# jilljenn/vae

Hardware: AMD Instinct MI355X
Metric: rating-triples/sec (ELBO step) at d=128 (higher is better)
Workload: dtype f32

## Files before the change

### include/vfm_hip.h

```cpp
#ifndef VFM_HIP_H
#define VFM_HIP_H

#include <stdint.h>

#ifdef __cplusplus
extern "C" {
#endif

#define VFM_ABI_VERSION 5
#define VFM_MAX_FIELDS 64
#define VFM_STRUCT_INIT(s) do { memset(&(s), 0, sizeof(s)); (s).struct_size = (uint32_t)sizeof(s); \
                                (s).abi_version = VFM_ABI_VERSION; } while (0)

#define VFM_E_INVALID (-1)
#define VFM_E_UNSUPPORTED (-2)

#define VFM_LIK_NORMAL 0
#define VFM_LIK_BERNOULLI 1

#define VFM_FLAG_NO_PRIOR_TERMS 1
#define VFM_FLAG_SPARSE_ADAM 4
#define VFM_FLAG_SCALED_MOMENTS 32
#define VFM_MOMENT_PERIOD 128
#define VFM_FLAG_ROWS_TOUCHED 128
#define VFM_FLAG_ZREC 1024
#define VFM_FLAG_SHARE_GPU 2048
#define VFM_FLAG_EPS_ZERO 2
#define VFM_FLAG_LINK_SOFTPLUS 16

#define VFM_P_LL 0
#define VFM_P_KL 1
#define VFM_P_G 2
#define VFM_P_ALPHA 3
#define VFM_P_BADID 4
#define VFM_P_GE0 5
#define VFM_P_REDUCED 6
#define VFM_N_PARTIALS 8
#define VFM_SLOT_NTERMS 6
#define VFM_MAX_FWD_BLOCKS 4096
#define VFM_PARTIALS_LEN (VFM_N_PARTIALS * (1 + VFM_MAX_FWD_BLOCKS))

typedef struct vfm_step_consts {
  float step_size, bc2_sqrt;
  float a1, q2, c1, c2, s1, s2;
  int32_t store_true;
  int32_t k;
  int32_t scaled;
  int32_t reserved;
  float lr, beta1, beta2, eps;
} vfm_step_consts_t;
typedef struct vfm_dev_step {
  uint64_t philox_step;
  int64_t adam_step;
  uint64_t philox_step_bwd;
  int64_t adam_step_bwd;
  int64_t tab_first, tab_len;
  const vfm_step_consts_t* tab;
  int64_t error;
} vfm_dev_step_t;
int vfm_step_consts(float lr, float beta1, float beta2, float eps_adam, int64_t step, int32_t scaled,
                    vfm_step_consts_t* out);
int vfm_dev_step_set(vfm_dev_step_t* dev_step, uint64_t philox_step, int64_t adam_step, void* stream);

typedef struct vfm_problem {
  uint32_t struct_size;
  uint32_t abi_version;
  int64_t B;
  int64_t B_global;
  int64_t T;
  int64_t nb_train;
  int32_t F;
  int32_t d;
  int32_t likelihood;
  int32_t id_bits;
  int32_t n_samples;
  int32_t flags;
  int64_t group_hi[VFM_MAX_FIELDS];
  double group_n[VFM_MAX_FIELDS];
  uint64_t seed;
  uint64_t step;
  int64_t e_lo, e_hi;
  vfm_dev_step_t* dev_step;
  float* wrec;
} vfm_problem_t;
int vfm_wrec_build_f32(const float* bias_params, const float* inv_occ, int64_t T, float* wrec, void* stream);

#define VFM_HEAVY_LIST 64
#define VFM_HEAVY_MIN 8
#define VFM_HEAVY_DIRECT 8
typedef struct vfm_index {
  uint32_t struct_size;
  uint32_t abi_version;
  const int32_t* occ_ptr;
  const int32_t* occ_rows;
  const int32_t* heavy_ids;
  const int32_t* heavy_items;
  float* heavy_acc;
  int32_t n_heavy;
  int32_t n_items;
  const int32_t* touched_ids;
  int64_t n_touched;
  const int32_t* occ_other;
  int32_t max_items;
  int32_t heavy_list, heavy_threshold;
  int32_t* status;
} vfm_index_t;

int vfm_abi_version(void);
const char* vfm_last_error(void);

int64_t vfm_index_workspace_bytes(int64_t B, int32_t F, int64_t T);
int vfm_rebuild_heavy(int64_t T, const int32_t* occ_ptr, void* ws, int32_t heavy_list, int32_t threshold, int32_t* heavy_ids,
                      int64_t cap_heavy, int32_t* heavy_items, int64_t cap_items, int32_t* counts , void* stream);
int32_t vfm_heavy_threshold(int32_t heavy_list);
#define VFM_HEAVY_UNITS 8192
int32_t vfm_heavy_list_for(int64_t n_occ, int64_t T);
int vfm_build_index(int64_t B, int32_t F, int64_t T, int32_t id_bits, const void* x, void* ws, int32_t* occ_ptr,
                    int32_t* occ_rows, int32_t heavy_list, int32_t* heavy_ids, int64_t cap_heavy,
                    int32_t* heavy_items, int64_t cap_items, int32_t* touched_ids, int32_t* occ_other,
                    const float* inv_occ, double* W, int32_t* counts, int32_t* counts_host, void* stream);

int vfm_inv_occ_f32(const int64_t* nb_occ, float* inv_occ, int64_t T, void* stream);

int vfm_batch_norms(const vfm_problem_t* p, const void* x, const float* inv_occ, double* W,
                    void* stream);

int vfm_elbo_fwd_f32(const vfm_problem_t* p, const void* x, const float* y,
                     const float* entity_params, const float* bias_params,
                     const float* inv_occ, const float* scalars, const double* W,
                     const float* eps_entity, const float* eps_bias, const float* eps_global,
                     float* pred, double* partials, float* sumz, float* grow, void* stream);

int vfm_elbo_finalize_f32(const vfm_problem_t* p, double* partials, const float* scalars,
                          float* loss, void* stream);

int vfm_elbo_bwd_f32(const vfm_problem_t* p, const vfm_index_t* idx,
                     const float* entity_params, const float* bias_params,
                     const float* inv_occ, const float* scalars, const double* W,
                     const float* eps_entity, const float* eps_bias, const float* eps_global,
                     const float* sumz, const float* grow, const double* partials,
                     const float* grad_out, float* g_entity, float* g_bias, float* g_scalars,
                     void* stream);

int vfm_elbo_bwd_adam_f32(const vfm_problem_t* p, const vfm_index_t* idx,
                          float* entity_params, float* bias_params, float* scalars,
                          const float* inv_occ, const double* W,
                          const float* eps_entity, const float* eps_bias, const float* eps_global,
                          const float* sumz, const float* grow, double* partials,
                          float* m_entity, float* v_entity, float* m_bias, float* v_bias,
                          float* m_scalars, float* v_scalars,
                          float lr, float beta1, float beta2, float eps_adam, int64_t step, float* loss,
                          void* stream);

int vfm_elbo_bwd_acc_f32(const vfm_problem_t* p, const vfm_index_t* idx,
                         const float* sumz, const float* grow, const double* partials, float* acc,
                         float* sums, void* stream);
int vfm_elbo_apply_adam_f32(const vfm_problem_t* p, const float* acc, const float* sums,
                            float* entity_params, float* bias_params, float* scalars, const float* inv_occ,
                            const double* W, const float* eps_entity, const float* eps_bias,
                            const float* eps_global, float* m_entity, float* v_entity, float* m_bias,
                            float* v_bias, float* m_scalars, float* v_scalars, float lr, float beta1,
                            float beta2, float eps_adam, int64_t step, void* stream);
int vfm_elbo_bwd_acc_rows_f32(const vfm_problem_t* p, const vfm_index_t* idx, const int32_t* row_ids, int64_t n_rows,
                              const float* sumz, const float* grow, const double* partials, float* acc,
                              float* sums, void* stream);
int vfm_elbo_apply_adam_rows_f32(const vfm_problem_t* p, const float* acc, const float* sums, const int32_t* row_ids,
                                 int64_t n_rows, int32_t compact_records, float* entity_params, float* bias_params, float* scalars,
                                 const float* inv_occ, const double* W, float* m_entity, float* v_entity, float* m_bias,
                                 float* v_bias, float* m_scalars, float* v_scalars, float lr, float beta1, float beta2,
                                 float eps_adam, int64_t step, void* stream);
int vfm_adam_f32(float* p, const float* g, float* m, float* v, int64_t n, float lr, float beta1,
                 float beta2, float eps, int64_t step, void* stream);

typedef struct vfm_pipe {
  uint32_t struct_size;
  uint32_t abi_version;
  const float* zrec;
  float* zrec_next;
  const int32_t* next_occ_ptr;
  const double* next_W;
  uint64_t next_step;
  int32_t* last_step;
  float* step_tab;
} vfm_pipe_t;
int vfm_sample_records_f32(const vfm_problem_t* p, const int32_t* ids, int64_t n, const float* entity_params,
                           const float* bias_params, const float* inv_occ, const double* W, float* zrec, void* stream);
int vfm_elbo_bwd_adam_pipe_f32(const vfm_problem_t* p, const vfm_index_t* idx, const vfm_pipe_t* pipe,
                               float* entity_params, float* bias_params, float* scalars,
                               const float* inv_occ, const double* W, const float* grow, double* partials,
                               float* m_entity, float* v_entity, float* m_bias, float* v_bias,
                               float* m_scalars, float* v_scalars,
                               float lr, float beta1, float beta2, float eps_adam, int64_t step, float* loss,
                               void* stream);

int vfm_adam_catchup_f32(float* entity_params, float* bias_params, const float* m_entity, const float* v_entity,
                         const float* m_bias, const float* v_bias, int32_t* last_step, const int32_t* ids, int64_t n,
                         int64_t T, int32_t d, const float* lr_of_step, int64_t n_lr, float beta1, float beta2,
                         float eps_adam, int64_t upto, int64_t mark, float* wrec, void* stream);

int64_t vfm_union_workspace_bytes(int64_t T);
int vfm_union_rows(int64_t T, const int32_t* occ_ptr_a, const int32_t* occ_ptr_b, void* ws, int32_t* rows, int32_t* count,
                   int32_t* count_host, void* stream);
int vfm_elbo_bwd_adam_lookahead_f32(const vfm_problem_t* p, const vfm_index_t* idx,
                                    float* entity_params, float* bias_params, float* scalars,
                                    const float* inv_occ, const double* W,
                                    const float* sumz, const float* grow, double* partials,
                                    float* m_entity, float* v_entity, float* m_bias, float* v_bias,
                                    float* m_scalars, float* v_scalars,
                                    float lr, float beta1, float beta2, float eps_adam, int64_t step, float* loss,
                                    int32_t* last_step, const int32_t* next_occ_ptr, float* step_tab, void* stream);

int vfm_moments_rescale_f32(float* m, float* v, int64_t n, float beta1, float beta2, int64_t step, int32_t to_scaled,
                            void* stream);

#define VFM_OBJ_SAMPLED 0
#define VFM_OBJ_CLOSED_FORM 1
int vfm_variant_fwd_f32(const vfm_problem_t* p, int32_t objective, const void* x, const float* values, const float* y,
                        const float* entity_params, const float* bias_params, const float* inv_occ,
                        const float* scalars, const double* W, const float* priors, const float* eps_entity,
                        const float* eps_bias, const float* eps_global, float* pred, double* partials, float* state,
                        float* grow, float* loss, void* stream);
int64_t vfm_variant_workspace_elems(int64_t B, int32_t F, int32_t d);
int vfm_variant_bwd_f32(const vfm_problem_t* p, int32_t objective, const vfm_index_t* idx, int32_t* occ_pos_ws,
                        const void* x, const float* values, const float* entity_params, const float* bias_params,
                        const float* inv_occ, const float* scalars, const double* W, const float* priors,
                        const float* eps_entity, const float* eps_bias, const float* eps_global, const float* state,
                        const float* grow, const double* partials, const float* grad_out, float* g_entity,
                        float* g_bias, float* g_scalars, float* g_priors, void* stream);

int vfm_philox_eps_f32(const vfm_problem_t* p, float* eps_entity, float* eps_bias,
                       float* eps_global, void* stream);

#ifdef __cplusplus
}
#endif
#endif
```

### vae_amd/_abi_gen.py

```python
import ctypes as C

VFM_ABI_VERSION = 5
VFM_E_INVALID = -1
VFM_E_UNSUPPORTED = -2
VFM_FLAG_EPS_ZERO = 2
VFM_FLAG_LINK_SOFTPLUS = 16
VFM_FLAG_NO_PRIOR_TERMS = 1
VFM_FLAG_ROWS_TOUCHED = 128
VFM_FLAG_SCALED_MOMENTS = 32
VFM_FLAG_SHARE_GPU = 2048
VFM_FLAG_SPARSE_ADAM = 4
VFM_FLAG_ZREC = 1024
VFM_HEAVY_DIRECT = 8
VFM_HEAVY_LIST = 64
VFM_HEAVY_MIN = 8
VFM_HEAVY_UNITS = 8192
VFM_LIK_BERNOULLI = 1
VFM_LIK_NORMAL = 0
VFM_MAX_FIELDS = 64
VFM_MAX_FWD_BLOCKS = 4096
VFM_MOMENT_PERIOD = 128
VFM_N_PARTIALS = 8
VFM_OBJ_CLOSED_FORM = 1
VFM_OBJ_SAMPLED = 0
VFM_PARTIALS_LEN = 32776
VFM_P_ALPHA = 3
VFM_P_BADID = 4
VFM_P_G = 2
VFM_P_GE0 = 5
VFM_P_KL = 1
VFM_P_LL = 0
VFM_P_REDUCED = 6
VFM_SLOT_NTERMS = 6


class StepConsts(C.Structure):
    _fields_ = [
        ("step_size", C.c_float),
        ("bc2_sqrt", C.c_float),
        ("a1", C.c_float),
        ("q2", C.c_float),
        ("c1", C.c_float),
        ("c2", C.c_float),
        ("s1", C.c_float),
        ("s2", C.c_float),
        ("store_true", C.c_int32),
        ("k", C.c_int32),
        ("scaled", C.c_int32),
        ("reserved", C.c_int32),
        ("lr", C.c_float),
        ("beta1", C.c_float),
        ("beta2", C.c_float),
        ("eps", C.c_float),
    ]


class DevStep(C.Structure):
    _fields_ = [
        ("philox_step", C.c_uint64),
        ("adam_step", C.c_int64),
        ("philox_step_bwd", C.c_uint64),
        ("adam_step_bwd", C.c_int64),
        ("tab_first", C.c_int64),
        ("tab_len", C.c_int64),
        ("tab", C.c_void_p),
        ("error", C.c_int64),
    ]


class Problem(C.Structure):
    _fields_ = [
        ("struct_size", C.c_uint32),
        ("abi_version", C.c_uint32),
        ("B", C.c_int64),
        ("B_global", C.c_int64),
        ("T", C.c_int64),
        ("nb_train", C.c_int64),
        ("F", C.c_int32),
        ("d", C.c_int32),
        ("likelihood", C.c_int32),
        ("id_bits", C.c_int32),
        ("n_samples", C.c_int32),
        ("flags", C.c_int32),
        ("group_hi", C.c_int64 * VFM_MAX_FIELDS),
        ("group_n", C.c_double * VFM_MAX_FIELDS),
        ("seed", C.c_uint64),
        ("step", C.c_uint64),
        ("e_lo", C.c_int64),
        ("e_hi", C.c_int64),
        ("dev_step", C.c_void_p),
        ("wrec", C.c_void_p),
    ]

    def __init__(self, *a, **k):
        super().__init__(*a, **k)
        self.struct_size, self.abi_version = C.sizeof(type(self)), VFM_ABI_VERSION


class Index(C.Structure):
    _fields_ = [
        ("struct_size", C.c_uint32),
        ("abi_version", C.c_uint32),
        ("occ_ptr", C.c_void_p),
        ("occ_rows", C.c_void_p),
        ("heavy_ids", C.c_void_p),
        ("heavy_items", C.c_void_p),
        ("heavy_acc", C.c_void_p),
        ("n_heavy", C.c_int32),
        ("n_items", C.c_int32),
        ("touched_ids", C.c_void_p),
        ("n_touched", C.c_int64),
        ("occ_other", C.c_void_p),
        ("max_items", C.c_int32),
        ("heavy_list", C.c_int32),
        ("heavy_threshold", C.c_int32),
        ("status", C.c_void_p),
    ]

    def __init__(self, *a, **k):
        super().__init__(*a, **k)
        self.struct_size, self.abi_version = C.sizeof(type(self)), VFM_ABI_VERSION


class Pipe(C.Structure):
    _fields_ = [
        ("struct_size", C.c_uint32),
        ("abi_version", C.c_uint32),
        ("zrec", C.c_void_p),
        ("zrec_next", C.c_void_p),
        ("next_occ_ptr", C.c_void_p),
        ("next_W", C.c_void_p),
        ("next_step", C.c_uint64),
        ("last_step", C.c_void_p),
        ("step_tab", C.c_void_p),
    ]

    def __init__(self, *a, **k):
        super().__init__(*a, **k)
        self.struct_size, self.abi_version = C.sizeof(type(self)), VFM_ABI_VERSION
```

### vae_amd/_lib.py

```python
from __future__ import annotations

import ctypes as C
import os

import torch

HERE = os.path.dirname(os.path.abspath(__file__))
LIB_DIR = os.environ.get("VFM_LIB_DIR") or HERE
LIB_PATH = os.path.join(LIB_DIR, "libvfm_hip.so")
OPS_PATH = os.path.join(LIB_DIR, "libvfm_torch_ops.so")

from . import _abi_gen as _gen

ABI_VERSION = _gen.VFM_ABI_VERSION
MAX_FWD_BLOCKS = _gen.VFM_MAX_FWD_BLOCKS
MAX_FIELDS = _gen.VFM_MAX_FIELDS
N_PARTIALS = _gen.VFM_N_PARTIALS
PARTIALS_LEN = _gen.VFM_PARTIALS_LEN
P_LL, P_KL, P_G, P_ALPHA, P_BADID = _gen.VFM_P_LL, _gen.VFM_P_KL, _gen.VFM_P_G, _gen.VFM_P_ALPHA, _gen.VFM_P_BADID
LIK_NORMAL, LIK_BERNOULLI = _gen.VFM_LIK_NORMAL, _gen.VFM_LIK_BERNOULLI
OBJ_SAMPLED, OBJ_CLOSED_FORM = _gen.VFM_OBJ_SAMPLED, _gen.VFM_OBJ_CLOSED_FORM

EXPORTS = (
    "vfm_abi_version", "vfm_last_error", "vfm_inv_occ_f32", "vfm_batch_norms",
    "vfm_elbo_fwd_f32", "vfm_elbo_finalize_f32", "vfm_elbo_bwd_f32", "vfm_philox_eps_f32",
    "vfm_adam_f32", "vfm_elbo_bwd_adam_f32", "vfm_elbo_bwd_acc_f32", "vfm_elbo_apply_adam_f32",
    "vfm_moments_rescale_f32", "vfm_index_workspace_bytes", "vfm_build_index", "vfm_heavy_list_for",
    "vfm_variant_fwd_f32", "vfm_variant_bwd_f32", "vfm_variant_workspace_elems", "vfm_adam_catchup_f32", "vfm_union_rows", "vfm_union_workspace_bytes",
    "vfm_sample_records_f32", "vfm_elbo_bwd_adam_pipe_f32", "vfm_elbo_bwd_adam_lookahead_f32",
    "vfm_step_consts", "vfm_dev_step_set", "vfm_wrec_build_f32", "vfm_elbo_apply_adam_rows_f32",
    "vfm_elbo_bwd_acc_rows_f32", "vfm_heavy_threshold", "vfm_rebuild_heavy",
)


class _Strict:

    def __setattr__(self, name, value):
        if name not in type(self)._names:
            raise AttributeError(f"{type(self).__name__} has no field {name!r}")
        super().__setattr__(name, value)


class Problem(_Strict, _gen.Problem):
    """`vfm_problem_t` (struct_size / abi_version are set by the generated __init__)."""


class Index(_Strict, _gen.Index):
    """`vfm_index_t`."""


class Pipe(_Strict, _gen.Pipe):
    """`vfm_pipe_t`."""


StepConsts, DevStep = _gen.StepConsts, _gen.DevStep

ELICIT_MAX_ROUNDS = 4096
ELICIT_SOLVE_EXPORTS = ("vfm_elicit_solve_f32", "vfm_elicit_solve_workspace_bytes")
ELICIT_EXPORTS = ("vfm_elicit_f32", "vfm_elicit_workspace_bytes", "vfm_elicit_field_f32",
                  "vfm_elicit_field_workspace_bytes") + ELICIT_SOLVE_EXPORTS


RANK_POST_EXPORTS = ("vfm_field_moments_post_f32", "vfm_rank_field_post_f32", "vfm_rank_heldout_field_post_f32")


VARIANT_STEP_EXPORTS = ("vfm_variant_step_f32", "vfm_variant_step_workspace_bytes")


def _fields(ctype, *names):
    return tuple((n, ctype) for n in names)


FOLDIN_SOLVE_EXPORTS = ("vfm_foldin_solve_f32", "vfm_foldin_solve_workspace_bytes")
FOLDIN_SOLVE_LDS_DIM = 135
FOLDIN_SOLVE_SLABS = 256
SWEEP_EXPORTS = ("vfm_foldin_solve_split_f32", "vfm_foldin_split_workspace_bytes")
PRIOR_EXPORTS = ("vfm_foldin_solve_prior_f32", "vfm_foldin_solve_prior_workspace_bytes",
                 "vfm_foldin_solve_split_prior_f32", "vfm_foldin_split_prior_workspace_bytes")
BOUND_EXPORTS = ("vfm_foldin_bound_f32", "vfm_foldin_bound_workspace_bytes")
BOUND_SWEEP_EXPORTS = ("vfm_foldin_bound_split_f32", "vfm_foldin_bound_split_workspace_bytes")
BOUND_PRIOR_EXPORTS = ("vfm_foldin_bound_prior_f32", "vfm_foldin_bound_prior_workspace_bytes",
                       "vfm_foldin_bound_split_prior_f32", "vfm_foldin_bound_split_prior_workspace_bytes")

_FOLD_COUNTS = _fields(C.c_int64, "E", "R", "T", "n_ops")
_FOLD_DIMS = _fields(C.c_int32, "F", "d", "col")
_FOLD_OPTIONS = _fields(C.c_int32, "flags", "lds_dim") + (("kl_weight", C.c_float),)
_FOLD_IDS = (("entities", C.c_void_p),)
_FOLD_TAIL = (_fields(C.c_void_p, "y", "op_x", "row_op", "entity_params", "bias_params", "scalars", "out_loss", "workspace")
              + (("workspace_bytes", C.c_int64),))
_FOLD_LIST_HEAD = _FOLD_COUNTS + _FOLD_DIMS + _fields(C.c_int32, "objective", "likelihood") + _FOLD_OPTIONS
_FOLD_CHUNK_HEAD = _FOLD_COUNTS + (("n_chunks", C.c_int64),) + _FOLD_DIMS + _FOLD_OPTIONS
_FOLD_LIST_ROWS = _FOLD_IDS + (("row_ptr", C.c_void_p),) + _FOLD_TAIL
_FOLD_CHUNK_ROWS = _FOLD_IDS + _fields(C.c_void_p, "chunk_ptr", "chunks") + _FOLD_TAIL


class FoldinSolve(_Strict, C.Structure):
    _fields_ = list(_FOLD_LIST_HEAD + _FOLD_LIST_ROWS)


class FoldinSplit(_Strict, C.Structure):
    _fields_ = list(_FOLD_CHUNK_HEAD + _FOLD_CHUNK_ROWS)


class FoldinBound(_Strict, C.Structure):
    _fields_ = list(_FOLD_LIST_HEAD + _fields(C.c_int32, "n_iters", "reset", "mode", "pad0") + _FOLD_LIST_ROWS)


class FoldinBoundSplit(_Strict, C.Structure):
    _fields_ = list(_FOLD_CHUNK_HEAD + _fields(C.c_int32, "n_iters", "reset") + _FOLD_CHUNK_ROWS)


_I64, _I32 = C.c_int64, C.c_int32
_SOLVE_SIZES, _SPLIT_SIZES = [_I64, _I64, _I32, _I32], [_I64, _I64, _I64, _I32, _I32]
_FOLD_PROTOTYPES = (
    ("vfm_foldin_solve_f32", FoldinSolve, [], "vfm_foldin_solve_workspace_bytes", _SOLVE_SIZES),
    ("vfm_foldin_solve_split_f32", FoldinSplit, [], "vfm_foldin_split_workspace_bytes", _SPLIT_SIZES),
    ("vfm_foldin_solve_prior_f32", FoldinSolve, [C.c_void_p], "vfm_foldin_solve_prior_workspace_bytes", _SOLVE_SIZES),
    ("vfm_foldin_solve_split_prior_f32", FoldinSplit, [C.c_void_p], "vfm_foldin_split_prior_workspace_bytes", _SPLIT_SIZES),
    ("vfm_foldin_bound_f32", FoldinBound, [], "vfm_foldin_bound_workspace_bytes", [_I64] + _SOLVE_SIZES),
    ("vfm_foldin_bound_split_f32", FoldinBoundSplit, [], "vfm_foldin_bound_split_workspace_bytes", [_I64] + _SPLIT_SIZES),
    ("vfm_foldin_bound_prior_f32", FoldinBound, [C.c_void_p], "vfm_foldin_bound_prior_workspace_bytes", [_I64] + _SOLVE_SIZES),
    ("vfm_foldin_bound_split_prior_f32", FoldinBoundSplit, [C.c_void_p], "vfm_foldin_bound_split_prior_workspace_bytes",
     [_I64] + _SPLIT_SIZES),
)


ELICIT_BOUND_EXPORTS = ("vfm_elicit_bound_f32", "vfm_elicit_bound_workspace_bytes")


_STAMP = _fields(C.c_uint32, "struct_size", "abi_version")
_COUNTS = _fields(C.c_int64, "U", "P", "H", "T", "n_ops")
_FIELD_ROWS = _fields(C.c_void_p, "entities", "pool_ptr", "pool_x", "pool_y", "hist_ptr", "hist_x", "hist_y")
_OPERANDS = _fields(C.c_void_p, "op_x", "pool_op", "hist_op")
_TABLES_OUTPUTS = _fields(C.c_void_p, "entity_params", "bias_params", "scalars", "out_row", "out_score", "out_loss",
                          "out_theta", "out_mean", "out_var")
_WORKSPACE = (("workspace", C.c_void_p), ("workspace_bytes", C.c_int64))
_ADAM_TAIL = (_fields(C.c_int32, "objective", "likelihood", "flags", "n_steps", "n_samples", "reset", "write", "lds_rows")
              + _fields(C.c_float, "lr", "kl_weight") + (("seed", C.c_uint64), ("t0", C.c_int64)))
_SOLVE_HEAD = (_fields(C.c_int32, "F", "d", "field", "key_col", "n_rounds", "strategy", "flags", "reset", "write", "lds_dim")
               + (("kl_weight", C.c_float),))
_SEED = (("seed", C.c_uint64),)


class _Session(_Strict, C.Structure):

    def __init__(self, *a, **k):
        super().__init__(*a, **k)
        self.struct_size, self.abi_version = C.sizeof(type(self)), ABI_VERSION


class Elicit(_Session):
    _fields_ = list(_STAMP + _COUNTS + _fields(C.c_int32, "F", "d", "n_rounds", "strategy") + _ADAM_TAIL
                    + _fields(C.c_void_p, "users", "pool_ptr", "pool_items", "pool_y", "hist_ptr", "hist_items", "hist_y")
                    + _OPERANDS + _TABLES_OUTPUTS + _WORKSPACE)


class ElicitField(_Session):
    _fields_ = list(_STAMP + _COUNTS + _fields(C.c_int32, "F", "d", "field", "key_col", "n_rounds", "strategy")
                    + _ADAM_TAIL + _FIELD_ROWS + _OPERANDS + _TABLES_OUTPUTS + _WORKSPACE)


class ElicitSolve(_Session):
    _fields_ = list(_STAMP + _COUNTS + _SOLVE_HEAD + _SEED + _FIELD_ROWS + _OPERANDS + _TABLES_OUTPUTS + _WORKSPACE)


class ElicitBound(_Session):
    _fields_ = list(_STAMP + _COUNTS + _SOLVE_HEAD + (("n_iters", C.c_int32),) + _SEED + _FIELD_ROWS + _OPERANDS
                    + _TABLES_OUTPUTS + _WORKSPACE)


DESIGN_EXPORTS = ("vfm_design_workspace_bytes", "vfm_design_scores_f32", "vfm_design_elicit_f32")


class ElicitDesign(_Session):
    _fields_ = list(_STAMP + _COUNTS + (("n_targets", C.c_int64),)
                    + _fields(C.c_int32, "F", "d", "field", "n_rounds", "flags", "reset", "write", "lds_dim")
                    + (("kl_weight", C.c_float),) + _FIELD_ROWS + _fields(C.c_void_p, "tgt_ptr", "tgt_op") + _OPERANDS
                    + _TABLES_OUTPUTS + (("out_pool_score", C.c_void_p),) + _WORKSPACE)


ELICIT_PRIOR_EXPORTS = ("vfm_elicit_solve_prior_f32", "vfm_elicit_solve_prior_workspace_bytes",
                        "vfm_elicit_bound_prior_f32", "vfm_elicit_bound_prior_workspace_bytes",
                        "vfm_design_scores_prior_f32", "vfm_design_elicit_prior_f32", "vfm_design_prior_workspace_bytes")
_ELICIT_PRIOR_PROTOTYPES = (
    ("vfm_elicit_solve_prior_f32", ElicitSolve, "vfm_elicit_solve_prior_workspace_bytes", [_I64, _I64, _I64, _I32, _I32]),
    ("vfm_elicit_bound_prior_f32", ElicitBound, "vfm_elicit_bound_prior_workspace_bytes",
     [_I64, _I64, _I64, _I64, _I32, _I32, _I32]),
    ("vfm_design_scores_prior_f32", ElicitDesign, "vfm_design_prior_workspace_bytes", [_I64, _I64, _I64, _I32, _I32]),
    ("vfm_design_elicit_prior_f32", ElicitDesign, "vfm_design_prior_workspace_bytes", [_I64, _I64, _I64, _I32, _I32]),
)


for _c in (Problem, Index, Pipe, Elicit, ElicitField, ElicitSolve, ElicitBound, ElicitDesign, FoldinSolve, FoldinSplit,
           FoldinBound, FoldinBoundSplit):
    _c._names = frozenset(n for n, _ in _c._fields_)


def heavy_list_for(n_occ: int, T: int) -> int:
    return int(load().vfm_heavy_list_for(int(n_occ), int(T)))


class VfmLibraryError(RuntimeError):
    pass


_lib = None


def load():
    global _lib
    if _lib is not None:
        return _lib
    if not os.path.exists(LIB_PATH):
        raise VfmLibraryError(
            f"{LIB_PATH} not found: build it with `python -c 'import __graft_entry__ as g; g.build()'` "
            "(hipcc --offload-arch=gfx950).  vae_amd has no CPU / PyTorch fallback.")
    lib = C.CDLL(LIB_PATH)
    vp, i64, i32 = C.c_void_p, C.c_int64, C.c_int32
    PP = C.POINTER(Problem)
    lib.vfm_abi_version.restype = C.c_int
    lib.vfm_abi_version.argtypes = []
    lib.vfm_last_error.restype = C.c_char_p
    lib.vfm_last_error.argtypes = []
    lib.vfm_inv_occ_f32.argtypes = [vp, vp, i64, vp]
    lib.vfm_batch_norms.argtypes = [PP, vp, vp, vp, vp]
    lib.vfm_elbo_fwd_f32.argtypes = [PP] + [vp] * 15
    lib.vfm_elbo_finalize_f32.argtypes = [PP, vp, vp, vp, vp]
    lib.vfm_elbo_bwd_f32.argtypes = [PP] + [vp] * 17
    lib.vfm_philox_eps_f32.argtypes = [PP, vp, vp, vp, vp]
    lib.vfm_elbo_bwd_adam_f32.argtypes = ([PP] + [vp] * 18 +
                                          [C.c_float, C.c_float, C.c_float, C.c_float, i64, vp, vp])
    lib.vfm_adam_f32.argtypes = [vp, vp, vp, vp, i64, C.c_float, C.c_float, C.c_float, C.c_float,
                                 i64, vp]
    lib.vfm_elbo_bwd_acc_f32.argtypes = [PP] + [vp] * 7
    lib.vfm_elbo_apply_adam_f32.argtypes = ([PP] + [vp] * 16 +
                                            [C.c_float, C.c_float, C.c_float, C.c_float, i64, vp])
    lib.vfm_elbo_bwd_acc_rows_f32.argtypes = [PP, C.POINTER(Index), vp, i64] + [vp] * 6
    lib.vfm_elbo_apply_adam_rows_f32.argtypes = ([PP, vp, vp, vp, i64, i32] + [vp] * 11 +
                                                 [C.c_float, C.c_float, C.c_float, C.c_float, i64, vp])
    lib.vfm_moments_rescale_f32.argtypes = [vp, vp, i64, C.c_float, C.c_float, i64, i32, vp]
    lib.vfm_index_workspace_bytes.argtypes = [i64, i32, i64]
    lib.vfm_heavy_list_for.argtypes = [i64, i64]
    lib.vfm_build_index.argtypes = [i64, i32, i64, i32, vp, vp, vp, vp, i32, vp, i64, vp, i64, vp, vp, vp, vp, vp, vp, vp]
    lib.vfm_rebuild_heavy.argtypes = [i64, vp, vp, i32, i32, vp, i64, vp, i64, vp, vp]
    lib.vfm_adam_catchup_f32.argtypes = [vp] * 8 + [i64, i64, i32, C.POINTER(C.c_float), i64, C.c_float, C.c_float, C.c_float,
                                         i64, i64, vp, vp]
    lib.vfm_step_consts.argtypes = [C.c_float, C.c_float, C.c_float, C.c_float, i64, i32, C.POINTER(StepConsts)]
    lib.vfm_dev_step_set.argtypes = [vp, C.c_uint64, i64, vp]
    lib.vfm_wrec_build_f32.argtypes = [vp, vp, i64, vp, vp]
    lib.vfm_sample_records_f32.argtypes = [PP, vp, i64, vp, vp, vp, vp, vp, vp]
    lib.vfm_elbo_bwd_adam_pipe_f32.argtypes = ([PP, C.POINTER(Index), C.POINTER(Pipe)] + [vp] * 13 +
                                               [C.c_float, C.c_float, C.c_float, C.c_float, i64, vp, vp])
    lib.vfm_elbo_bwd_adam_lookahead_f32.argtypes = ([PP, C.POINTER(Index)] + [vp] * 14 +
                                                    [C.c_float, C.c_float, C.c_float, C.c_float, i64, vp, vp, vp, vp, vp])
    lib.vfm_variant_fwd_f32.argtypes = [PP, i32] + [vp] * 18
    lib.vfm_variant_bwd_f32.argtypes = [PP, i32, C.POINTER(Index)] + [vp] * 21
    lib.vfm_union_workspace_bytes.argtypes = [i64]
    lib.vfm_union_workspace_bytes.restype = i64
    lib.vfm_union_rows.argtypes = [i64] + [vp] * 7
    lib.vfm_variant_workspace_elems.argtypes = [i64, i32, i32]
    lib.vfm_variant_workspace_elems.restype = i64
    lib.vfm_elicit_f32.argtypes = [C.POINTER(Elicit), vp]
    lib.vfm_elicit_f32.restype = C.c_int
    lib.vfm_elicit_workspace_bytes.argtypes = [i64, i64, i32, i32]
    lib.vfm_elicit_workspace_bytes.restype = i64
    lib.vfm_elicit_field_f32.argtypes = [C.POINTER(ElicitField), vp]
    lib.vfm_elicit_field_f32.restype = C.c_int
    lib.vfm_elicit_field_workspace_bytes.argtypes = [i64, i64, i32, i32]
    lib.vfm_elicit_field_workspace_bytes.restype = i64
    lib.vfm_elicit_solve_f32.argtypes = [C.POINTER(ElicitSolve), vp]
    lib.vfm_elicit_solve_f32.restype = C.c_int
    lib.vfm_elicit_solve_workspace_bytes.argtypes = [i64, i64, i64, i32, i32]
    lib.vfm_elicit_solve_workspace_bytes.restype = i64
    lib.vfm_design_workspace_bytes.argtypes = [i64, i64, i64, i32, i32]
    lib.vfm_design_workspace_bytes.restype = i64
    for name in ("vfm_design_scores_f32", "vfm_design_elicit_f32"):
        getattr(lib, name).argtypes = [C.POINTER(ElicitDesign), vp]
        getattr(lib, name).restype = C.c_int
    for entry, struct, extra, size, size_args in _FOLD_PROTOTYPES:
        getattr(lib, entry).argtypes = [C.POINTER(struct)] + extra + [vp]
        getattr(lib, entry).restype = C.c_int
        getattr(lib, size).argtypes = size_args
        getattr(lib, size).restype = i64
    lib.vfm_elicit_bound_f32.argtypes = [C.POINTER(ElicitBound), vp]
    lib.vfm_elicit_bound_f32.restype = C.c_int
    lib.vfm_elicit_bound_workspace_bytes.argtypes = [i64, i64, i64, i64, i32, i32, i32]
    lib.vfm_elicit_bound_workspace_bytes.restype = i64
    for entry, struct, size, size_args in _ELICIT_PRIOR_PROTOTYPES:
        getattr(lib, entry).argtypes = [C.POINTER(struct), vp, vp]
        getattr(lib, entry).restype = C.c_int
        getattr(lib, size).argtypes = size_args
        getattr(lib, size).restype = i64
    u64 = C.c_uint64
    lib.vfm_field_moments_post_f32.argtypes = [i64, i32, i32, i64, i32, i32, vp, i32, i32, vp, vp, vp, vp, i32, u64,
                                               vp, vp, vp, vp, vp]
    lib.vfm_rank_field_post_f32.argtypes = ([i64, vp, i32, i32, vp, vp, i64, vp, i64, i64, i32, i32, i32, i32, i32, u64,
                                             i32, vp, vp, i64, vp, vp, vp, vp, i64] + [vp] * 5)
    lib.vfm_rank_heldout_field_post_f32.argtypes = ([i64, vp, i32, i32, vp, vp, i64, vp, i64, i64, i32, i32, i32, i32, u64,
                                                     i32, vp, vp, i64, vp, vp, i64, vp, vp, vp, vp, i64] + [vp] * 5)
    for name in RANK_POST_EXPORTS:
        getattr(lib, name).restype = C.c_int
    lib.vfm_variant_step_f32.argtypes = ([PP, i32, C.POINTER(Index)] + [vp] * 24 +
                                         [C.c_float, C.c_float, C.c_float, C.c_float, i64, vp])
    lib.vfm_variant_step_f32.restype = C.c_int
    lib.vfm_variant_step_workspace_bytes.argtypes = [i64, i32, i32]
    lib.vfm_variant_step_workspace_bytes.restype = i64
    for name in EXPORTS:
        fn = getattr(lib, name)
        if name != "vfm_last_error":
            fn.restype = C.c_int
    for name in ("vfm_index_workspace_bytes", "vfm_union_workspace_bytes", "vfm_variant_workspace_elems"):
        getattr(lib, name).restype = i64
    if lib.vfm_abi_version() != ABI_VERSION:
        raise VfmLibraryError(f"ABI mismatch: library {lib.vfm_abi_version()}, package {ABI_VERSION}")
    _lib = lib
    return lib


_ops = None


def ops():
    global _ops
    if _ops is not None:
        return _ops
    load()
    if not os.path.exists(OPS_PATH):
        raise VfmLibraryError(f"{OPS_PATH} not found: run __graft_entry__.build()")
    torch.ops.load_library(OPS_PATH)
    if torch.ops.vfm_hip.abi_version() != ABI_VERSION:
        raise VfmLibraryError("ABI mismatch between libvfm_torch_ops.so and the package")
    _ops = torch.ops.vfm_hip
    return _ops


def check(rc, what):
    if rc != 0:
        msg = load().vfm_last_error().decode(errors="replace")
        raise VfmLibraryError(f"{what} failed (code {rc}): {msg}")


def ptr(t):
    return None if t is None else C.c_void_p(t.data_ptr())


def raw_stream(device) -> int:
    idx = device.index if getattr(device, "index", None) is not None else torch.cuda.current_device()
    return torch._C._cuda_getCurrentRawStream(idx)


def current_stream_ptr(device):
    return C.c_void_p(raw_stream(device))
```

### vae_amd/csrc/vfm_abi.hip

```cpp
#include <stdio.h>
#include <string.h>
#include <math.h>
#include <stdlib.h>
#include <mutex>

#include "vfm_args.hpp"

namespace vfm {

namespace {
thread_local char g_err[512] = "";
}

int fail(int code, const char* msg) {
  snprintf(g_err, sizeof(g_err), "%s", msg);
  return code;
}
int fail_hip(hipError_t e, const char* where) {
  snprintf(g_err, sizeof(g_err), "%s: %s", where, hipGetErrorString(e));
  return (int)e;
}
int env_int(const char* name, int dflt) {
  const char* v = getenv(name);
  return (v && *v) ? atoi(v) : dflt;
}

namespace {

#include "vfm_rng.hpp"
#include "vfm_common.hpp"
#include "vfm_reduce.hpp"
#include "vfm_small_kernels.hpp"
#include "vfm_heavy.hpp"
#include "vfm_adam.hpp"

bool pick_shape(int d, Shape* s) {
  auto pow2ceil = [](int v) { int p = 1; while (p < v) p <<= 1; return p; };
  if (d % 4 == 0) {
    const int C = d / 4;
    s->vec = 4;
    s->lpe = pow2ceil(C) < 64 ? (pow2ceil(C) < 4 ? 4 : pow2ceil(C)) : 64;
    const int cpl = (C + s->lpe - 1) / s->lpe;
    s->cpl = cpl <= 1 ? 1 : (cpl <= 2 ? 2 : 4);
    return cpl <= 4;
  }
  s->vec = 1;
  if (d <= 8) { s->lpe = 8; s->cpl = 1; return true; }
  if (d <= 64) { s->lpe = 64; s->cpl = 1; return true; }
  s->lpe = 64; s->cpl = 4;
  return d <= 256;
}

int check_struct(uint32_t size, uint32_t abi, size_t want, const char* name) {
  if (size == (uint32_t)want && abi == (uint32_t)VFM_ABI_VERSION) return 0;
  snprintf(g_err, sizeof(g_err), "%s: struct_size %u / abi_version %u, this library expects %zu / %d (set them with "
           "VFM_STRUCT_INIT; a binding generated from another version of include/vfm_hip.h must be regenerated)",
           name, size, abi, want, VFM_ABI_VERSION);
  return VFM_E_INVALID;
}

int check_problem(const vfm_problem_t* p, bool dev_ok = false) {
  if (!p) return fail(VFM_E_INVALID, "problem is NULL");
  if (int rc = check_struct(p->struct_size, p->abi_version, sizeof(vfm_problem_t), "vfm_problem_t")) return rc;
  if (p->dev_step && !dev_ok)
    return fail(VFM_E_UNSUPPORTED, "vfm_problem_t.dev_step: only the training forward and the fused backward+Adam entry points read the step from device memory");
  if (p->dev_step && p->n_samples != 1) return fail(VFM_E_UNSUPPORTED, "vfm_problem_t.dev_step: one variational sample");
  if (p->dev_step && (((uintptr_t)p->dev_step) & 15) != 0) return fail(VFM_E_INVALID, "vfm_problem_t.dev_step must be 16-byte aligned");
  if (p->wrec && (((uintptr_t)p->wrec) & 15) != 0) return fail(VFM_E_INVALID, "vfm_problem_t.wrec must be 16-byte aligned");
  if (p->B < 0 || p->T <= 0 || p->T > 0xFFFFFFFELL) return fail(VFM_E_INVALID, "bad B or T");
  if (p->F < 1 || p->F > VFM_MAX_FIELDS) return fail(VFM_E_INVALID, "F out of range [1,64]");
  if (p->d < 1) return fail(VFM_E_INVALID, "d < 1");
  if (p->id_bits != 32 && p->id_bits != 64) return fail(VFM_E_INVALID, "id_bits must be 32 or 64");
  if (p->likelihood != VFM_LIK_NORMAL && p->likelihood != VFM_LIK_BERNOULLI)
    return fail(VFM_E_INVALID, "unknown likelihood");
  if (p->n_samples < 1 || p->n_samples > MAX_SAMPLES) return fail(VFM_E_INVALID, "n_samples out of range [1,64]");
  if (p->n_samples > 1 && (p->step >> 48) != 0) return fail(VFM_E_INVALID, "step must stay below 2^48 when n_samples > 1");
  if (p->B_global < p->B) return fail(VFM_E_INVALID, "B_global < B");
  if (p->B * (int64_t)p->F > 0x7FFFFFFFLL) return fail(VFM_E_INVALID, "B*F exceeds int32 index range");
  if (p->e_lo < 0 || p->e_lo > p->T || (p->e_hi != 0 && p->e_hi < p->e_lo)) return fail(VFM_E_INVALID, "bad entity range");
  if (p->flags & ~(VFM_FLAG_NO_PRIOR_TERMS | VFM_FLAG_EPS_ZERO | VFM_FLAG_SPARSE_ADAM | VFM_FLAG_LINK_SOFTPLUS |
                   VFM_FLAG_SCALED_MOMENTS | VFM_FLAG_ROWS_TOUCHED | VFM_FLAG_ZREC | VFM_FLAG_SHARE_GPU))
    return fail(VFM_E_INVALID, "unknown bit in vfm_problem_t.flags");
  Shape s;
  if (!pick_shape(p->d, &s)) return fail(VFM_E_UNSUPPORTED, "embedding size d not supported (d%4==0: d<=1024, else d<=256)");
  return 0;
}

bool softplus(const vfm_problem_t* p) { return (p->flags & VFM_FLAG_LINK_SOFTPLUS) != 0; }

int single_sample_only(const vfm_problem_t* p, const char* who) {
  if (p->n_samples == 1) return 0;
  snprintf(g_err, sizeof(g_err), "%s: n_samples > 1 is not supported by this entry point", who);
  return VFM_E_UNSUPPORTED;
}


int eps_mode(const vfm_problem_t* p, const float* ee, const float* eb, const float* eg, int* mode) {
  const int neps = (ee != nullptr) + (eb != nullptr) + (eg != nullptr);
  if (neps != 0 && neps != 3) return fail(VFM_E_INVALID, "give all three eps tables or none");
  *mode = (p->flags & VFM_FLAG_EPS_ZERO) ? EPS_ZERO : (neps == 3 ? EPS_TABLE : EPS_PHILOX);
  return 0;
}

KArgs make_args(const vfm_problem_t* p, const void* x, const float* y, const float* entity,
                const float* bias, const float* inv_occ, const float* scalars, const double* W,
                const float* ee, const float* eb, const float* eg, int sample = 0) {
  KArgs a;
  memset(&a, 0, sizeof(a));
  a.S = p->n_samples; a.sample = sample; a.inv_S = 1.0f / (float)p->n_samples;
  if (sample > 0) {
    if (ee) ee += (size_t)sample * (size_t)p->T * (size_t)p->d;
    if (eb) eb += (size_t)sample * (size_t)p->T;
  }
  a.B = p->B; a.T = p->T; a.F = p->F; a.d = p->d; a.lik = p->likelihood;
  a.e_lo = p->e_lo; a.e_hi = (p->e_hi > 0 && p->e_hi < p->T) ? p->e_hi : p->T;
  a.id64 = p->id_bits == 64; a.G = p->F; a.flags = p->flags;
  a.ll_scale_d = (double)p->nb_train / ((double)(p->B_global > 0 ? p->B_global : 1) * (double)p->n_samples);
  a.ll_scale = (float)a.ll_scale_d;
  a.key.seed_lo = (uint32_t)p->seed; a.key.seed_hi = (uint32_t)(p->seed >> 32);
  a.key.step_lo = (uint32_t)p->step; a.key.step_hi = (uint32_t)(p->step >> 32);
  a.key.chunk_off = 0;
  a.x = x; a.y = y; a.entity = entity; a.bias = bias; a.inv_occ = inv_occ; a.scalars = scalars;
  a.W = W; a.eps_entity = ee; a.eps_bias = eb; a.eps_global = eg;
  a.dev = p->dev_step; a.wrec = p->wrec;
  for (int g = 0; g < p->F; ++g) { a.group_hi[g] = p->group_hi[g]; a.group_n[g] = p->group_n[g]; }
  return a;
}

bool use_fwd2(const vfm_problem_t* p, int eps, bool multi = false) {
  if (p->F != 2 || (p->d & 3) != 0 || p->d > 512) return false;
  if (multi ? (p->n_samples < 2 || p->n_samples > 4 || eps == EPS_ZERO) : p->n_samples != 1) return false;
  if (softplus(p)) return false;
  const int forced = env_int("VFM_FWD_KERNEL", 0);
  if (forced == 1) return false;
  return forced == 2 || eps == EPS_ZREC || multi || p->d >= 20;
}

bool use_fwdg(const vfm_problem_t* p, int eps, int mode) {
  if (p->F == 2 || (p->d & 3) != 0 || p->d < 16 || p->d > 512 || p->n_samples != 1) return false;
  if ((p->flags & VFM_FLAG_ZREC) || softplus(p)) return false;
  if (!(eps == EPS_PHILOX || (eps == EPS_ZERO && mode == MODE_PREDICT))) return false;
  return env_int("VFM_FWD_KERNEL", 0) != 1;
}

int dispatch_fwd(const vfm_problem_t* p, const Shape& s, int eps, int mode, int ff, KArgs& a, const FwdOut& o,
                 hipStream_t st) {
  if (use_fwdg(p, eps, mode)) return launch_fwdg_abs(eps, mode, a, o, st);
  if (use_fwd2(p, eps)) {
    if (mode == MODE_TRAIN && eps == EPS_PHILOX && env_int("VFM_FWD_AB_NORNG", 0) == 1) eps = EPS_ZERO;
    return launch_fwd2_abs(eps, mode, a, o, st);
  }
  return softplus(p) ? launch_fwd_softplus(s, eps, mode, ff, a, o, st) : launch_fwd_abs(s, eps, mode, ff, a, o, st);
}
int dispatch_bwd(const vfm_problem_t* p, const Shape& s, int eps, int adam, KArgs& a, const BwdArgs& b,
                 const AdamArgs& ad, hipStream_t st) {
  if (adam == 0 || adam == 10)
    return softplus(p) ? launch_bwd0_softplus(s, eps, adam, a, b, ad, st) : launch_bwd0_abs(s, eps, adam, a, b, ad, st);
  return softplus(p) ? launch_bwd1_softplus(s, eps, adam, a, b, ad, st) : launch_bwd1_abs(s, eps, adam, a, b, ad, st);
}

BwdArgs bwd_args(const vfm_problem_t* p, const vfm_index_t* idx) {
  BwdArgs b;
  memset(&b, 0, sizeof(b));
  if (idx) { b.occ_ptr = idx->occ_ptr; b.occ_rows = idx->occ_rows; b.status = idx->status; }
  b.n_occ = (int32_t)(p->B * (int64_t)p->F);
  return b;
}

template <int LPE, int CPL, int VEC>
int launch_heavy_t(const vfm_problem_t* p, const vfm_index_t* idx, const float* sumz, const float* grow, float* hacc, int d,
                   hipStream_t st, const float* zrec = nullptr) {
  constexpr int GPB = BLOCK / LPE;
  const size_t xs = 4 + (((size_t)d + 3) & ~(size_t)3);
  float* item_acc = hacc + xs * (size_t)idx->n_heavy;
  int64_t nb = ((int64_t)idx->n_items + GPB - 1) / GPB;
  if (nb > 4096) nb = 4096;
  hipLaunchKernelGGL((k_heavy<LPE, CPL, VEC>), dim3((unsigned)nb), dim3(BLOCK), 0, st, idx->heavy_items,
                     (int)idx->n_items, idx->occ_rows, sumz, grow, item_acc, d, zrec ? idx->occ_other : nullptr, zrec, hacc,
                     (int)idx->n_heavy, (int)(p->B * (int64_t)p->F), (int)p->B, p->T, idx->status);
  if (idx->max_items > 0 && idx->max_items <= VFM_HEAVY_DIRECT) return 0;
  nb = idx->n_heavy;
  if (nb > 4096) nb = 4096;
  hipLaunchKernelGGL((k_heavy_sum<LPE, CPL, VEC>), dim3((unsigned)nb), dim3(BLOCK), 0, st, idx->heavy_items,
                     (int)idx->n_items, (int)idx->n_heavy, item_acc, hacc, d);
  return 0;
}

int run_heavy(const vfm_problem_t* p, const vfm_index_t* idx, const float* sumz, const float* grow,
              hipStream_t st, BwdArgs* b, const float* zrec = nullptr) {
  b->heavy_ids = nullptr; b->heavy_acc = nullptr; b->n_heavy = 0; b->heavy_stride = 0;
  if (idx->n_heavy <= 0 || idx->n_items <= 0) return 0;
  if (!idx->heavy_ids || !idx->heavy_items || !idx->heavy_acc)
    return fail(VFM_E_INVALID, "index: heavy_ids / heavy_items / heavy_acc missing");
  if ((int64_t)idx->n_heavy > p->T || (int64_t)idx->n_items > p->B * (int64_t)p->F + idx->n_heavy)
    return fail(VFM_E_INVALID, "index: more heavy entities than table rows, or more work items than occurrences");
  const size_t xs = 4 + (((size_t)p->d + 3) & ~(size_t)3);
  const size_t per_sample = xs * ((size_t)idx->n_heavy + (size_t)idx->n_items);
  Shape s;
  pick_shape(p->d, &s);
  for (int sm = 0; sm < p->n_samples; ++sm) {
    const float* sz = sumz ? sumz + (size_t)sm * (size_t)p->B * (size_t)p->d : nullptr;
    float* hacc = idx->heavy_acc + (size_t)sm * per_sample;
#define X(L_, C_, V_) \
    if (s.lpe == L_ && s.cpl == C_ && s.vec == V_) launch_heavy_t<L_, C_, V_>(p, idx, sz, grow, hacc, p->d, st, zrec);
    VFM_FOR_SHAPES(X)
#undef X
  }
  b->heavy_ids = idx->heavy_ids; b->heavy_acc = idx->heavy_acc; b->n_heavy = idx->n_heavy;
  b->heavy_stride = idx->n_heavy + idx->n_items;
  return 0;
}

struct Side { hipStream_t s = nullptr; hipEvent_t e1 = nullptr, e2 = nullptr; bool ok = false, tried = false; std::mutex mu; };
Side* side_of_device() {
  static Side sides[64];
  static std::mutex mu;
  int dev = 0;
  if (hipGetDevice(&dev) != hipSuccess || dev < 0 || dev >= 64) return nullptr;
  std::lock_guard<std::mutex> lk(mu);
  Side& sd = sides[dev];
  if (!sd.tried) {
    sd.tried = true;
    sd.ok = hipStreamCreateWithFlags(&sd.s, hipStreamNonBlocking) == hipSuccess &&
            hipEventCreateWithFlags(&sd.e1, hipEventDisableTiming) == hipSuccess &&
            hipEventCreateWithFlags(&sd.e2, hipEventDisableTiming) == hipSuccess;
  }
  return sd.ok ? &sd : nullptr;
}
bool heavy_overlap(const vfm_problem_t* p, const vfm_index_t* idx) {
  return idx->n_heavy > 0 && idx->n_items > 0 && (int64_t)idx->n_heavy * 16 < p->T && p->n_samples == 1 &&
         env_int("VFM_HEAVY_OVERLAP", 1) != 0;
}

int bwd_adam_overlapped(const vfm_problem_t* p, const vfm_index_t* idx, const Shape& s, int eps, int adam, KArgs& a, BwdArgs& b,
                        const AdamArgs& ad, const float* sumz, const float* grow, hipStream_t st, Side* sd) {
  std::lock_guard<std::mutex> lk(sd->mu);
  hipError_t e = hipEventRecord(sd->e1, st);
  if (e == hipSuccess) e = hipStreamWaitEvent(sd->s, sd->e1, 0);
  if (e != hipSuccess) return fail_hip(e, "heavy-list overlap: events");
  if (int rc = run_heavy(p, idx, sumz, grow, sd->s, &b)) return rc;
  e = hipEventRecord(sd->e2, sd->s);
  if (e != hipSuccess) return fail_hip(e, "heavy-list overlap: events");
  const int32_t keep = a.row_filter;
  a.row_filter = 4;
  if (int rc = dispatch_bwd(p, s, eps, adam, a, b, ad, st)) return rc;
  e = hipStreamWaitEvent(st, sd->e2, 0);
  if (e != hipSuccess) return fail_hip(e, "heavy-list overlap: events");
  BwdArgs bh = b;
  bh.row_ids = idx->heavy_ids; bh.n_rows = idx->n_heavy;
  a.row_filter = 3;
  const int rc = dispatch_bwd(p, s, eps, adam, a, bh, ad, st);
  a.row_filter = keep;
  return rc;
}

bool small_table_step(const vfm_problem_t* p, const vfm_index_t* idx, int eps, int rows_flags) {
  if (eps != EPS_PHILOX || rows_flags != 0 || p->n_samples != 1 || (p->flags & VFM_FLAG_SPARSE_ADAM)) return false;
  if ((p->d & 3) != 0 || p->d > 256) return false;
  if (idx->heavy_list < VFM_HEAVY_MIN || idx->heavy_threshold < VFM_HEAVY_MIN || idx->heavy_threshold > idx->heavy_list) return false;
  if (p->T * (2 * (int64_t)p->d + 2) * 4 > (2LL << 20)) return false;
  return env_int("VFM_BWD_SMALL", 1) != 0;
}

int check_index(const vfm_problem_t* p, const vfm_index_t* idx, const char* who) {
  if (!idx) { snprintf(g_err, sizeof(g_err), "%s: inverted index missing", who); return VFM_E_INVALID; }
  if (int rc = check_struct(idx->struct_size, idx->abi_version, sizeof(vfm_index_t), "vfm_index_t")) return rc;
  if (!idx->occ_ptr || (p->B > 0 && !idx->occ_rows)) {
    snprintf(g_err, sizeof(g_err), "%s: inverted index missing", who);
    return VFM_E_INVALID;
  }
  if (idx->n_heavy < 0 || idx->n_items < 0 || idx->n_touched < 0 || idx->max_items < 0) {
    snprintf(g_err, sizeof(g_err), "%s: negative count in vfm_index_t", who);
    return VFM_E_INVALID;
  }
  return 0;
}

int after_launch(const char* where) {
  const hipError_t e = hipGetLastError();
  if (e != hipSuccess) return fail_hip(e, where);
  return 0;
}

void adam_consts(float lr, float beta1, float beta2, int64_t step, float* step_size, float* bc2_sqrt) {
  const double bc1 = 1.0 - pow((double)beta1, (double)step);
  const double bc2 = 1.0 - pow((double)beta2, (double)step);
  *step_size = (float)((double)lr / bc1);
  *bc2_sqrt = (float)sqrt(bc2);
}

void scaled_step_consts(float step_size, float bc2_sqrt, double s1, double s2, float* a1, float* q2) {
  *a1 = (float)((double)step_size * s1);
  *q2 = (float)(sqrt(s2) / (double)bc2_sqrt);
}

int scaled_moment_consts(const vfm_problem_t* p, float beta1, float beta2, int64_t step, AdamArgs* ad) {
  ad->scaled = 0; ad->store_true = 0; ad->s1 = ad->s2 = 1.f; ad->c1 = 1.f - beta1; ad->c2 = 1.f - beta2;
  ad->inv_bc2_sqrt = 1.0f / ad->bc2_sqrt;
  ad->a1 = ad->step_size; ad->q2 = ad->inv_bc2_sqrt;
  if (!(p->flags & VFM_FLAG_SCALED_MOMENTS)) return 0;
  if (p->flags & VFM_FLAG_SPARSE_ADAM)
    return fail(VFM_E_INVALID, "VFM_FLAG_SCALED_MOMENTS and VFM_FLAG_SPARSE_ADAM exclude each other");
  const int64_t k = (step - 1) % VFM_MOMENT_PERIOD + 1;
  const double s1 = pow((double)beta1, (double)k), s2 = pow((double)beta2, (double)k);
  if (!(s1 > 1e-30) || !(s2 > 1e-30))
    return fail(VFM_E_UNSUPPORTED, "VFM_FLAG_SCALED_MOMENTS: beta^128 underflows (use the plain moments for such betas)");
  ad->scaled = 1; ad->store_true = (k == VFM_MOMENT_PERIOD);
  ad->s1 = (float)s1; ad->s2 = (float)s2;
  ad->c1 = (float)((1.0 - (double)beta1) / s1); ad->c2 = (float)((1.0 - (double)beta2) / s2);
  scaled_step_consts(ad->step_size, ad->bc2_sqrt, s1, s2, &ad->a1, &ad->q2);
  return 0;
}

}
}

using namespace vfm;

int vfm::launch_norms(int64_t B, int F, int64_t T, int id_bits, const void* x, const float* inv_occ, double* W, hipStream_t st) {
  hipLaunchKernelGGL(k_zero_f64, dim3(1), dim3(64), 0, st, W, F);
  if (B == 0) return after_launch("vfm_batch_norms");
  int64_t nbx = (B + BLOCK * 8 - 1) / (BLOCK * 8);
  if (nbx > 1024) nbx = 1024;
  hipLaunchKernelGGL(k_norms, dim3((unsigned)nbx, (unsigned)F), dim3(BLOCK), 0, st, x, (int)(id_bits == 64), inv_occ, B, F, T,
                     reinterpret_cast<unsigned long long*>(W));
  hipLaunchKernelGGL(k_norms_fix, dim3(1), dim3(64), 0, st, W, F);
  return after_launch("vfm_batch_norms");
}

extern "C" {

int vfm_abi_version(void) { return VFM_ABI_VERSION; }
const char* vfm_last_error(void) { return g_err; }

int vfm_step_consts(float lr, float beta1, float beta2, float eps_adam, int64_t step, int32_t scaled,
                    vfm_step_consts_t* out) {
  if (!out || step < 1) return fail(VFM_E_INVALID, "vfm_step_consts: bad argument");
  vfm_problem_t p;
  memset(&p, 0, sizeof(p));
  p.flags = scaled ? VFM_FLAG_SCALED_MOMENTS : 0;
  AdamArgs ad;
  memset(&ad, 0, sizeof(ad));
  ad.b1 = beta1; ad.b2 = beta2; ad.eps = eps_adam;
  adam_consts(lr, beta1, beta2, step, &ad.step_size, &ad.bc2_sqrt);
  if (int rc = scaled_moment_consts(&p, beta1, beta2, step, &ad)) return rc;
  memset(out, 0, sizeof(*out));
  out->step_size = ad.step_size; out->bc2_sqrt = ad.bc2_sqrt; out->a1 = ad.a1; out->q2 = ad.q2;
  out->c1 = ad.c1; out->c2 = ad.c2; out->s1 = ad.s1; out->s2 = ad.s2;
  out->store_true = ad.store_true; out->k = (int32_t)((step - 1) % VFM_MOMENT_PERIOD + 1); out->scaled = ad.scaled;
  out->lr = lr; out->beta1 = beta1; out->beta2 = beta2; out->eps = eps_adam;
  return 0;
}

int vfm_dev_step_set(vfm_dev_step_t* dev_step, uint64_t philox_step, int64_t adam_step, void* stream) {
  if (!dev_step || adam_step < 1) return fail(VFM_E_INVALID, "vfm_dev_step_set: bad argument");
  hipLaunchKernelGGL(k_dev_step_set, dim3(1), dim3(64), 0, (hipStream_t)stream, dev_step, philox_step, adam_step);
  return after_launch("vfm_dev_step_set");
}

int vfm_wrec_build_f32(const float* bias_params, const float* inv_occ, int64_t T, float* wrec, void* stream) {
  if (!bias_params || !inv_occ || !wrec || T <= 0 || (((uintptr_t)wrec) & 15) != 0)
    return fail(VFM_E_INVALID, "vfm_wrec_build_f32: bad argument");
  const int grid = (int)((T + 255) / 256 < 2048 ? (T + 255) / 256 : 2048);
  hipLaunchKernelGGL(k_wrec_build, dim3(grid), dim3(256), 0, (hipStream_t)stream, bias_params, inv_occ, T, wrec);
  return after_launch("vfm_wrec_build_f32");
}

int vfm_inv_occ_f32(const int64_t* nb_occ, float* inv_occ, int64_t T, void* stream) {
  if (!nb_occ || !inv_occ || T <= 0) return fail(VFM_E_INVALID, "vfm_inv_occ_f32: bad argument");
  const int grid = (int)((T + 255) / 256 < 2048 ? (T + 255) / 256 : 2048);
  hipLaunchKernelGGL(k_inv_occ, dim3(grid), dim3(256), 0, (hipStream_t)stream, nb_occ, inv_occ, T);
  return after_launch("vfm_inv_occ_f32");
}

int vfm_batch_norms(const vfm_problem_t* p, const void* x, const float* inv_occ, double* W,
                    void* stream) {
  if (int rc = check_problem(p)) return rc;
  if (!W || (p->B > 0 && (!x || !inv_occ))) return fail(VFM_E_INVALID, "vfm_batch_norms: NULL pointer");
  return launch_norms(p->B, p->F, p->T, p->id_bits, x, inv_occ, W, (hipStream_t)stream);
}

int vfm_elbo_fwd_f32(const vfm_problem_t* p, const void* x, const float* y,
                     const float* entity_params, const float* bias_params,
                     const float* inv_occ, const float* scalars, const double* W,
                     const float* eps_entity, const float* eps_bias, const float* eps_global,
                     float* pred, double* partials, float* sumz, float* grow, void* stream) {
  if (int rc = check_problem(p, true)) return rc;
  if (!partials) return fail(VFM_E_INVALID, "vfm_elbo_fwd_f32: partials is NULL");
  if (p->dev_step && (eps_entity || eps_bias || eps_global || (p->flags & VFM_FLAG_EPS_ZERO)))
    return fail(VFM_E_UNSUPPORTED, "vfm_elbo_fwd_f32: dev_step goes with the in-kernel Philox eps stream only");
  hipStream_t st0 = (hipStream_t)stream;
  if (p->B == 0) {
    hipLaunchKernelGGL(k_zero_f64, dim3(1), dim3(64), 0, st0, partials, (int)VFM_N_PARTIALS);
    return after_launch("vfm_elbo_fwd_f32");
  }
  const bool zrec = (p->flags & VFM_FLAG_ZREC) != 0;
  if (zrec) {
    if (!use_fwd2(p, EPS_ZREC)) return fail(VFM_E_UNSUPPORTED, "VFM_FLAG_ZREC: two fields, one sample, d % 4 == 0, d <= 512, |.| link");
    if (!x || !y || !entity_params || !scalars || !pred || !grow || eps_entity || eps_bias || eps_global)
      return fail(VFM_E_INVALID, "vfm_elbo_fwd_f32 (VFM_FLAG_ZREC): x, y, the record table, scalars, pred, grow; no eps tables");
    KArgs a = make_args(p, x, y, entity_params, nullptr, nullptr, scalars, nullptr, nullptr, nullptr, nullptr, 0);
    FwdOut o{pred, partials, nullptr, grow};
    if (int rc = launch_fwd2_abs(EPS_ZREC, MODE_TRAIN, a, o, (hipStream_t)stream)) return rc;
    return after_launch("vfm_elbo_fwd_f32");
  }
  if (!x || !entity_params || !bias_params || !scalars || !pred)
    return fail(VFM_E_INVALID, "vfm_elbo_fwd_f32: NULL pointer");
  const bool train = y != nullptr;
  if (train && (!inv_occ || !W || !sumz || !grow))
    return fail(VFM_E_INVALID, "vfm_elbo_fwd_f32: y given, so inv_occ, W, sumz and grow are required");
  if (!train && (sumz || grow)) return fail(VFM_E_INVALID, "vfm_elbo_fwd_f32: sumz / grow need y");
  int eps;
  if (int rc = eps_mode(p, eps_entity, eps_bias, eps_global, &eps)) return rc;
  if (train && eps == EPS_ZERO) return fail(VFM_E_UNSUPPORTED, "vfm_elbo_fwd_f32: VFM_FLAG_EPS_ZERO is prediction-only");
  hipStream_t st = (hipStream_t)stream;
  FwdOut o{pred, partials, sumz, grow};
  Shape s;
  pick_shape(p->d, &s);
  if (use_fwd2(p, eps, true)) {
    KArgs a = make_args(p, x, y, entity_params, bias_params, inv_occ, scalars, W, eps_entity, eps_bias, eps_global, 0);
    const int md = train ? MODE_TRAIN : MODE_PREDICT;
    if (int rc = launch_fwd2m_abs(eps, md, a, o, st)) return rc;
    return after_launch("vfm_elbo_fwd_f32");
  }
  for (int sm = 0; sm < p->n_samples; ++sm) {
    KArgs a = make_args(p, x, y, entity_params, bias_params, inv_occ, scalars, W, eps_entity, eps_bias,
                        eps_global, sm);
// ... 416 lines not shown
```

### vae_amd/csrc/vfm_args.hpp

```cpp
#pragma once
#include <hip/hip_runtime.h>
#include <stdint.h>

#include "vfm_hip.h"

#define VFM_INTERNAL __attribute__((visibility("hidden")))

namespace vfm {

constexpr int BLOCK = 256;
constexpr float LOG_SQRT_2PI = 0.918938533204672742f;
constexpr float LN2 = 0.693147180559945309f;
constexpr float LOG2E = 1.4426950408889634f;

struct RngKey {
  uint32_t seed_lo, seed_hi, step_lo, step_hi;
  uint32_t chunk_off;
};

struct KArgs {
  int64_t B, T;
  int64_t e_lo, e_hi;
  int32_t F, d, lik, id64, G, flags;
  int32_t S, sample;
  int32_t row_filter;
  float inv_S;
  float ll_scale;
  double ll_scale_d;
  RngKey key;
  const void* x;
  const float* y;
  const float* entity;
  const float* bias;
  const float* inv_occ;
  const float* scalars;
  const double* W;
  const float* eps_entity;
  const float* eps_bias;
  const float* eps_global;
  vfm_dev_step_t* dev;
  float* wrec;
  int64_t group_hi[VFM_MAX_FIELDS];
  double group_n[VFM_MAX_FIELDS];
};

struct FwdOut {
  float* pred;
  double* partials;
  float* sumz;
  float* grow;
};

struct BwdArgs {
  const int32_t* occ_ptr;
  const int32_t* occ_rows;
  const float* sumz;
  const float* grow;
  double* partials;
  const float* grad_out;
  float* g_entity;
  float* g_bias;
  float* g_scalars;
  float* loss;
  float* acc;
  float* sums;
  const int32_t* heavy_ids;
  const float* heavy_acc;
  int32_t n_heavy;
  int32_t heavy_stride;
  const int32_t* row_ids;
  int64_t n_rows;
  const float* zrec;
  const int32_t* occ_other;
  float* zrec_next;
  const int32_t* next_occ_ptr;
  const double* next_W;
  RngKey next_key;
  int32_t* last_step;
  float2* step_tab;
  int32_t la_step, la_k;
  int32_t rec_by_slot;
  int32_t n_occ;
  int32_t* status;
};

struct AdamArgs {
  float* m_entity; float* v_entity; float* m_bias; float* v_bias; float* m_scal; float* v_scal;
  float b1, b2, eps, step_size, bc2_sqrt;
  int32_t scaled, store_true;
  float s1, s2, c1, c2, inv_bc2_sqrt;
  float a1, q2;
};

__device__ __forceinline__ RngKey key_of_step(const KArgs& a, bool writer) {
  RngKey key = a.key;
  if (a.dev) {
    const uint64_t s = a.dev->philox_step;
    key.step_lo = (uint32_t)s; key.step_hi = (uint32_t)(s >> 32);
    if (writer) { a.dev->philox_step_bwd = s; a.dev->adam_step_bwd = a.dev->adam_step; }
  }
  return key;
}
__device__ __forceinline__ void load_dev_step(const KArgs& a, RngKey& key, AdamArgs& ad, int32_t& la_step, int32_t& la_k,
                                              RngKey& next_key, bool bump) {
  if (!a.dev) return;
  const uint64_t s = a.dev->philox_step_bwd;
  const int64_t t = a.dev->adam_step_bwd;
  key.step_lo = (uint32_t)s; key.step_hi = (uint32_t)(s >> 32);
  next_key.step_lo = (uint32_t)(s + 1); next_key.step_hi = (uint32_t)((s + 1) >> 32);
  int64_t i = t - a.dev->tab_first;
  const bool miss = i < 0 || i >= a.dev->tab_len;
  if (miss) i = i < 0 ? 0 : a.dev->tab_len - 1;
  const vfm_step_consts_t c = a.dev->tab[i];
  ad.step_size = c.step_size; ad.bc2_sqrt = c.bc2_sqrt; ad.inv_bc2_sqrt = 1.0f / c.bc2_sqrt;
  ad.a1 = c.a1; ad.q2 = c.q2; ad.c1 = c.c1; ad.c2 = c.c2; ad.s1 = c.s1; ad.s2 = c.s2;
  ad.store_true = c.store_true; ad.scaled = c.scaled;
  ad.b1 = c.beta1; ad.b2 = c.beta2; ad.eps = c.eps;
  la_step = (int32_t)t; la_k = c.k;
  if (bump) {
    a.dev->philox_step = s + 1; a.dev->adam_step = t + 1;
    if (miss) a.dev->error = 1;
  }
}

struct Shape {
  int lpe, cpl, vec;
};

enum { EPS_PHILOX = 0, EPS_TABLE = 1, EPS_ZERO = 2, EPS_ZREC = 4 };
enum { MODE_PREDICT = 0, MODE_TRAIN = 1 };
enum { STAGE_FULL = 0, STAGE_ACC = 1, STAGE_APPLY = 2 };
enum { LINK_ABS = 0, LINK_SOFTPLUS = 1 };
constexpr int MAX_SAMPLES = 64;

VFM_INTERNAL int fail(int code, const char* msg);
VFM_INTERNAL int fail_hip(hipError_t e, const char* where);
VFM_INTERNAL int env_int(const char* name, int dflt);
VFM_INTERNAL int launch_norms(int64_t B, int F, int64_t T, int id_bits, const void* x, const float* inv_occ, double* W,
                              hipStream_t st);

#define VFM_DECLARE_LAUNCHERS(SUFFIX)                                                                          \
  VFM_INTERNAL int launch_fwd_##SUFFIX(const Shape& s, int eps, int mode, int ff, KArgs& a, const FwdOut& o,   \
                                       hipStream_t st);                                                        \
  VFM_INTERNAL int launch_bwd0_##SUFFIX(const Shape& s, int eps, int adam, KArgs& a, const BwdArgs& b,         \
                                        const AdamArgs& ad, hipStream_t st);                                   \
  VFM_INTERNAL int launch_bwd1_##SUFFIX(const Shape& s, int eps, int adam, KArgs& a, const BwdArgs& b,         \
                                        const AdamArgs& ad, hipStream_t st);
VFM_DECLARE_LAUNCHERS(abs)
VFM_DECLARE_LAUNCHERS(softplus)
VFM_INTERNAL int launch_bwd_small_abs(const Shape& s, KArgs& a, const BwdArgs& b, const AdamArgs& ad, int L, int THR, hipStream_t st);
VFM_INTERNAL int launch_bwd_small_softplus(const Shape& s, KArgs& a, const BwdArgs& b, const AdamArgs& ad, int L, int THR, hipStream_t st);
VFM_INTERNAL int launch_fwd2_abs(int eps, int mode, KArgs& a, const FwdOut& o, hipStream_t st);
VFM_INTERNAL int launch_fwd2m_abs(int eps, int mode, KArgs& a, const FwdOut& o, hipStream_t st);
VFM_INTERNAL int launch_fwdg_abs(int eps, int mode, KArgs& a, const FwdOut& o, hipStream_t st);
VFM_INTERNAL int launch_sample_rec_abs(const Shape& s, KArgs& a, const int32_t* ids, int n, float* zrec, hipStream_t st);

#define VFM_FOR_SHAPES(X)                                                                      \
  X(4, 1, 4) X(8, 1, 4) X(16, 1, 4) X(32, 1, 4) X(64, 1, 4) X(64, 2, 4) \
  X(64, 4, 4) X(8, 1, 1) X(64, 1, 1) X(64, 4, 1)

}
```

### vae_amd/csrc/vfm_fwd2.hip

```cpp
#include <math.h>

#include "vfm_args.hpp"

#ifndef VFM_LINK
#error "compile with -DVFM_LINK=0 (abs) or -DVFM_LINK=1 (softplus)"
#endif

namespace vfm {
namespace {

#include "vfm_rng.hpp"
#include "vfm_common.hpp"
typedef float v2f __attribute__((ext_vector_type(2)));
#include "vfm_fwd2.hpp"

constexpr int LINK = VFM_LINK;

template <int LPE, bool FULL, int EPS, int MODE>
int launch_fwd2_t(KArgs& a, const FwdOut& o, hipStream_t st) {
  constexpr int GPB = BLOCK / LPE;
  const int per_cu = env_int("VFM_FWD2_BLOCKS_PER_CU", 4);
  int64_t nb = (a.B + GPB - 1) / GPB;
  int64_t cap = 256LL * per_cu;
  if (cap > VFM_MAX_FWD_BLOCKS) cap = VFM_MAX_FWD_BLOCKS;
  if (nb > cap) nb = cap;
  { const int share = env_int("VFM_SHARE_CAP", 960); if ((a.flags & VFM_FLAG_SHARE_GPU) && share > 0 && nb > share) nb = share; }
  { const int forced = env_int("VFM_FWD2_GRID", 0); if (forced > 0 && nb > forced) nb = forced; }
  if (nb < 1) nb = 1;
  if constexpr (EPS == EPS_PHILOX && MODE == MODE_TRAIN) {
    if (a.wrec) {
      if (a.id64)
        hipLaunchKernelGGL((k_fwd2<LPE, FULL, EPS, MODE, true, LINK, true>), dim3((unsigned)nb), dim3(BLOCK), 0, st, a, o);
      else
        hipLaunchKernelGGL((k_fwd2<LPE, FULL, EPS, MODE, false, LINK, true>), dim3((unsigned)nb), dim3(BLOCK), 0, st, a, o);
      return 0;
    }
  }
  if (a.id64)
    hipLaunchKernelGGL((k_fwd2<LPE, FULL, EPS, MODE, true, LINK>), dim3((unsigned)nb), dim3(BLOCK), 0, st, a, o);
  else
    hipLaunchKernelGGL((k_fwd2<LPE, FULL, EPS, MODE, false, LINK>), dim3((unsigned)nb), dim3(BLOCK), 0, st, a, o);
  return 0;
}

template <int LPE, bool FULL>
int launch_fwd2_s(int eps, int mode, KArgs& a, const FwdOut& o, hipStream_t st) {
#define FWD2(E_, M_) \
  if (eps == E_ && mode == M_) return launch_fwd2_t<LPE, FULL, E_, M_>(a, o, st);
  FWD2(EPS_PHILOX, MODE_TRAIN) FWD2(EPS_TABLE, MODE_TRAIN) FWD2(EPS_ZERO, MODE_TRAIN) FWD2(EPS_ZREC, MODE_TRAIN)
  FWD2(EPS_PHILOX, MODE_PREDICT) FWD2(EPS_TABLE, MODE_PREDICT) FWD2(EPS_ZERO, MODE_PREDICT)
#undef FWD2
  return fail(VFM_E_UNSUPPORTED, "forward (task stream): unsupported eps source / mode combination");
}

int dispatch_fwd2(int eps, int mode, KArgs& a, const FwdOut& o, hipStream_t st) {
  const int C = a.d / 4, P = (C + 1) / 2;
  int lpe = 1;
  while (lpe < P) lpe <<= 1;
  const bool full = a.d == 8 * lpe;
#define X(L_)                                                                       \
  if (lpe == L_) return full ? launch_fwd2_s<L_, true>(eps, mode, a, o, st)         \
                             : launch_fwd2_s<L_, false>(eps, mode, a, o, st);
  X(1) X(2) X(4) X(8) X(16) X(32) X(64)
#undef X
  return fail(VFM_E_UNSUPPORTED, "forward (task stream): embedding size above 512");
}

}

#if VFM_LINK == 0
int launch_fwd2_abs(int eps, int mode, KArgs& a, const FwdOut& o, hipStream_t st) {
  return dispatch_fwd2(eps, mode, a, o, st);
}
#else
int launch_fwd2_softplus(int eps, int mode, KArgs& a, const FwdOut& o, hipStream_t st) {
  return dispatch_fwd2(eps, mode, a, o, st);
}
#endif

}
```

### vae_amd/csrc/vfm_fwd2.hpp

```cpp
#pragma once


template <int EPS>
struct EntRegs {
  uint32_t e;
  Chunk<4> mu[2], s[2], ep[2];
  float2 th;
  float io;
  float epw;
};

template <bool ID64>
struct RawIds {
  uint32_t ulo, uhi, ilo, ihi;
};
struct Ids {
  uint32_t u, i;
};
constexpr uint32_t BAD_ID = 0xFFFFFFFFu;

template <bool ID64>
__device__ __forceinline__ RawIds<ID64> load_row_ids(const KArgs& a, int r) {
  RawIds<ID64> v;
  if constexpr (ID64) {
    const uint4 t = reinterpret_cast<const uint4*>(a.x)[r];
    v.ulo = t.x; v.uhi = t.y; v.ilo = t.z; v.ihi = t.w;
  } else {
    const uint2 t = reinterpret_cast<const uint2*>(a.x)[r];
    v.ulo = t.x; v.uhi = 0u; v.ilo = t.y; v.ihi = 0u;
  }
  return v;
}

template <bool ID64>
__device__ __forceinline__ Ids fold_ids(const RawIds<ID64>& v, uint32_t T32) {
  Ids o;
  o.u = ((!ID64 || v.uhi == 0u) && v.ulo < T32) ? v.ulo : BAD_ID;
  o.i = ((!ID64 || v.ihi == 0u) && v.ilo < T32) ? v.ilo : BAD_ID;
  return o;
}

__device__ __forceinline__ uint32_t entity_of(uint32_t id, bool live, float& bad) {
  const bool ok = id != BAD_ID;
  bad += (live && !ok) ? 1.f : 0.f;
  return ok ? id : 0u;
}

template <int EPS, int MODE, bool WREC = false>
__device__ __forceinline__ void load_ent(const KArgs& a, uint32_t e, int off0, int off1, EntRegs<EPS>& R) {
  const size_t d = (size_t)a.d;
  R.e = e;
  if constexpr (EPS == EPS_ZREC) {
    const float* rec = a.entity + (size_t)e * (4 + d);
    R.mu[0] = ld_chunk<4>(rec + 4 + off0);
    R.mu[1] = ld_chunk<4>(rec + 4 + off1);
    const float4 h = *reinterpret_cast<const float4*>(rec);
    R.th = make_float2(h.x, 0.f);
    R.io = h.y;
    return;
  }
  const float* row = a.entity + (size_t)e * (2 * d);
  R.mu[0] = ld_chunk<4>(row + off0);
  R.mu[1] = ld_chunk<4>(row + off1);
  R.s[0] = ld_chunk<4>(row + d + off0);
  R.s[1] = ld_chunk<4>(row + d + off1);
  if constexpr (EPS == EPS_TABLE) {
    const float* er = a.eps_entity + (size_t)e * d;
    R.ep[0] = ld_chunk<4>(er + off0);
    R.ep[1] = ld_chunk<4>(er + off1);
    R.epw = a.eps_bias[e];
  }
  if constexpr (WREC) {
    const float4 h = *reinterpret_cast<const float4*>(a.wrec + 4 * (size_t)e);
    R.th = make_float2(h.x, h.y);
    R.io = h.z;
  } else {
    R.th = *reinterpret_cast<const float2*>(a.bias + 2 * (size_t)e);
    if constexpr (MODE == MODE_TRAIN) R.io = a.inv_occ[e];
  }
}

template <bool FULL, int EPS, int MODE, int LINK>
__device__ __forceinline__ void sample_ent(const RngKey& key, const EntRegs<EPS>& R, uint32_t pg, bool v0, bool v1,
                                           bool owns_bias, float cs, float (&z)[8], float& w, float& klw) {
  if constexpr (EPS == EPS_ZREC) {
#pragma unroll
    for (int t = 0; t < 4; ++t) {
      z[t] = (FULL || v0) ? R.mu[0].v[t] : 0.f;
      z[4 + t] = (FULL || v1) ? R.mu[1].v[t] : 0.f;
    }
    w = owns_bias ? R.th.x : 0.f;
    klw = (MODE == MODE_TRAIN && owns_bias) ? R.io : 0.f;
    return;
  }
  float ep[8], epw = 0.f;
  if constexpr (EPS == EPS_TABLE) {
#pragma unroll
    for (int t = 0; t < 4; ++t) { ep[t] = R.ep[0].v[t]; ep[4 + t] = R.ep[1].v[t]; }
    epw = R.epw;
  } else if constexpr (EPS == EPS_PHILOX) {
    normal8b(key, R.e, pg, ep, epw);
  } else {
#pragma unroll
    for (int t = 0; t < 8; ++t) ep[t] = 0.f;
  }
  float klv = 0.f;
#pragma unroll
  for (int c = 0; c < 2; ++c) {
    const bool valid = FULL || (c == 0 ? v0 : v1);
    v2f kq = {0.f, 0.f};
    float lg = 0.f;
#pragma unroll
    for (int h = 0; h < 2; ++h) {
      const v2f m2 = {R.mu[c].v[2 * h], R.mu[c].v[2 * h + 1]};
      const v2f g2 = {link_f<LINK>(R.s[c].v[2 * h]), link_f<LINK>(R.s[c].v[2 * h + 1])};
      const v2f e2 = {ep[4 * c + 2 * h], ep[4 * c + 2 * h + 1]};
      const v2f z2 = g2 * e2 + m2;
      z[4 * c + 2 * h] = valid ? z2.x : 0.f;
      z[4 * c + 2 * h + 1] = valid ? z2.y : 0.f;
      if constexpr (MODE == MODE_TRAIN) {
        kq = g2 * g2 + kq;
        kq = m2 * m2 + kq;
        lg += __builtin_amdgcn_logf(fmaxf(g2.x, SIGMA_MIN) * fmaxf(g2.y, SIGMA_MIN));
      }
    }
    if constexpr (MODE == MODE_TRAIN) klv += valid ? fmaf(0.5f, kq.x + kq.y, fmaf(-LN2, lg, -2.0f)) : 0.f;
  }
  const float sgw = link_f<LINK>(R.th.y);
  w = owns_bias ? fmaf(sgw, epw, R.th.x) : 0.f;
  klw = 0.f;
  if constexpr (MODE == MODE_TRAIN) {
    klv += owns_bias ? kl_std_normal(R.th.x, sgw) : 0.f;
    klw = klv * (cs * R.io);
  }
}

template <int LPE, bool FULL, int EPS, int MODE, bool ID64, int LINK, bool WREC = false>
__global__ __launch_bounds__(BLOCK, 4) void k_fwd2(const KArgs a, const FwdOut out) {
  constexpr int GPB = BLOCK / LPE;
  __shared__ float sh_cs[2];
  __shared__ int64_t sh_hi[2];
  __shared__ float sh_red[6 * 4];
  __shared__ float sh_e0;

  const int tid = threadIdx.x;
  const int lig = tid % LPE;
  const int C = a.d >> 2;
  const int NG = (int)gridDim.x * GPB;
  const int gid = (int)blockIdx.x * GPB + tid / LPE;
  const int q = (int)(a.B / NG), rem = (int)(a.B % NG);
  const int gbeg = gid * q + (gid < rem ? gid : rem);
  const int gend = gbeg + q + (gid < rem ? 1 : 0);
  const int glast = gend - 1;
  RawIds<ID64> raw0, raw1, raw2;
  float y_first = 0.f;
  if (gbeg < gend) {
    raw0 = load_row_ids<ID64>(a, gbeg);
    raw1 = load_row_ids<ID64>(a, gbeg + 1 < gend ? gbeg + 1 : glast);
    raw2 = load_row_ids<ID64>(a, gbeg + 2 < gend ? gbeg + 2 : glast);
    if constexpr (MODE == MODE_TRAIN) y_first = a.y[gbeg];
  }
  const RngKey key = key_of_step(a, blockIdx.x == 0 && tid == 0);

  if (MODE == MODE_TRAIN && EPS != EPS_ZREC && tid < 2) {
    sh_cs[tid] = (float)(a.group_n[tid] / a.W[tid]);
    sh_hi[tid] = a.group_hi[tid];
  }
  if constexpr (EPS == EPS_PHILOX || EPS == EPS_ZREC) {
    if (tid < 64) {
      float n[8], nb;
      normal8b(key, 0xFFFFFFFFu, 0u, n, nb);
      if (tid == 0) sh_e0 = n[0];
    }
  } else if (tid == 0) {
    sh_e0 = (EPS == EPS_TABLE) ? a.eps_global[0] : 0.f;
  }
  __syncthreads();
  const float alpha = a.scalars[0], m0 = a.scalars[1], s0 = a.scalars[2];
  const float aabs = link_f<LINK>(alpha);
  const float w0 = fmaf(link_f<LINK>(s0), sh_e0, m0);
  const float half_log_a = 0.5f * LN2 * __builtin_amdgcn_logf(aabs);
  const bool owns_bias = lig == 0;
  float cs0 = 0.f, cs1 = 0.f;
  uint32_t hi0 = 0u;
  if constexpr (MODE == MODE_TRAIN && EPS != EPS_ZREC) {
    cs0 = sh_cs[0]; cs1 = sh_cs[1];
    hi0 = sh_hi[0] > 0xFFFFFFFFLL ? 0xFFFFFFFFu : (uint32_t)sh_hi[0];
  }
  const uint32_t T32 = (uint32_t)a.T;

  const int j0 = 2 * lig, j1 = 2 * lig + 1;
  const bool v0 = j0 < C, v1 = j1 < C;
  const int off0 = 4 * (v0 ? j0 : C - 1), off1 = 4 * (v1 ? j1 : C - 1);
  const uint32_t pg = (uint32_t)lig + (key.chunk_off >> 1);

  float tot[6] = {0.f, 0.f, 0.f, 0.f, 0.f, 0.f};
  if (gbeg < gend) {
    int r0 = gbeg;
    Ids id0 = fold_ids<ID64>(raw0, T32);
    Ids id1 = fold_ids<ID64>(raw1, T32);
    RawIds<ID64> id2 = raw2;
    bool cur_item = true;
    EntRegs<EPS> A, Bq;
    load_ent<EPS, MODE, WREC>(a, entity_of(id0.i, true, tot[4]), off0, off1, A);
    float ycur = y_first;
    float zi[8], wi = 0.f, klwi = 0.f;
#pragma unroll
    for (int t = 0; t < 8; ++t) zi[t] = 0.f;

    auto step = [&](const EntRegs<EPS>& cu, EntRegs<EPS>& nx) -> bool {
      const bool item_now = cur_item;
      const int r_now = r0;
      const float y_now = ycur;
      const bool adv = !item_now;
      const uint32_t n_u = adv ? id1.u : id0.u, n_i = adv ? id1.i : id0.i;
      const int r_next = r0 + (adv ? 1 : 0);
      const bool live_next = r_next < gend;
      const bool item_next = adv && (n_i != id0.i);
      const uint32_t e_next = entity_of(item_next ? n_i : n_u, live_next, tot[4]);
      const Ids f2 = fold_ids<ID64>(id2, T32);
      id2 = load_row_ids<ID64>(a, r_next + 2 < gend ? r_next + 2 : glast);
      load_ent<EPS, MODE, WREC>(a, e_next, off0, off1, nx);
      if constexpr (MODE == MODE_TRAIN) ycur = a.y[live_next ? r_next : glast];
      id0.u = n_u; id0.i = n_i;
      id1.u = adv ? f2.u : id1.u;
      id1.i = adv ? f2.i : id1.i;
      r0 = r_next;
      cur_item = item_next;
      float z[8], w, klw;
      const float cs = (cu.e < hi0) ? cs0 : cs1;
      sample_ent<FULL, EPS, MODE, LINK>(key, cu, pg, v0, v1, owns_bias, cs, z, w, klw);
      if (item_now) {
#pragma unroll
        for (int t = 0; t < 8; ++t) zi[t] = z[t];
        wi = w; klwi = klw;
      } else {
        v2f qv = {0.f, 0.f};
#pragma unroll
        for (int h = 0; h < 4; ++h) {
          const v2f zu = {z[2 * h], z[2 * h + 1]};
          const v2f zv = {zi[2 * h], zi[2 * h + 1]};
          qv = zu * zv + qv;
        }
        const float val = group_sum<LPE>(qv.x + qv.y + w + wi);
        if constexpr (MODE == MODE_TRAIN) tot[1] += klw + klwi;
        if constexpr (MODE == MODE_TRAIN && EPS != EPS_ZREC) {
          float* srow = out.sumz + (size_t)r_now * a.d;
          Chunk<4> s0c, s1c;
#pragma unroll
          for (int t = 0; t < 4; ++t) { s0c.v[t] = z[t] + zi[t]; s1c.v[t] = z[4 + t] + zi[4 + t]; }
          if (FULL || v0) st_chunk<4>(srow + off0, s0c);
          if (FULL || v1) st_chunk<4>(srow + off1, s1c);
        }
        const float pred = w0 + val;
        if (lig == 0) {
          out.pred[r_now] = pred;
          if constexpr (MODE == MODE_TRAIN) {
            float ll, dll, at;
            lik_terms(a.lik, y_now, pred, aabs, half_log_a, ll, dll, at);
            const float g = -a.ll_scale * dll;
            tot[0] += ll; tot[2] += g; tot[3] += at;
            out.grow[r_now] = g;
          }
        }
      }
      return live_next;
    };

    while (true) {
      if (!step(A, Bq)) break;
      if (!step(Bq, A)) break;
    }
  }
  block_sum<6>(tot, sh_red);
  if (tid == 0) {
    double* slot = out.partials + VFM_N_PARTIALS * (1 + (size_t)blockIdx.x);
#pragma unroll
    for (int i = 0; i < 6; ++i) slot[i] = (double)tot[i];
    slot[VFM_SLOT_NTERMS] = slot_nterms(a, MODE == MODE_TRAIN);
    if (blockIdx.x == 0) {
      out.partials[7] = (double)gridDim.x;
      out.partials[VFM_P_REDUCED] = 0.0;
    }
  }
}
```

### vae_amd/csrc/vfm_index.hip

```cpp
#include <string.h>

#include "vfm_args.hpp"

namespace vfm {
namespace {

constexpr int RS_THREADS = 256;
constexpr int RS_ITEMS = 8;
constexpr int RS_TILE = RS_THREADS * RS_ITEMS;
constexpr int RS_SUB = RS_ITEMS * (RS_THREADS / 64);
constexpr int RS_MAXBITS = 9;
constexpr int RS_MAXD = 1 << RS_MAXBITS;
constexpr int RS_MAXPASS = 4;
constexpr int HV_CHUNK = 256;
constexpr int HV_SELF = 1024;
constexpr int NW_MAXF = 4;

struct Geo {
  int64_t n, n4, NB, G, NS, NBH;
  int passes, rb[RS_MAXPASS], shift[RS_MAXPASS];
  int64_t k0, v0, k1, v1, zero_lo, L1[RS_MAXPASS], L2[RS_MAXPASS], zero_hi, excl, blk, bad, wpart, total;
};

int key_bits(int64_t T) {
// ... 288 lines not shown
      }
    }
  }
}

__device__ __forceinline__ void ent_counts(uint32_t c, int L, int THR, uint32_t& hv, uint32_t& it, uint32_t& any) {
  any = c > 0 ? 1u : 0u;
  hv = c > (uint32_t)THR ? 1u : 0u;
  it = hv ? (c + (uint32_t)L - 1) / (uint32_t)L : 0u;
}

constexpr int IC_STAGE = 6144;
template <bool SEARCH>
__global__ __launch_bounds__(HV_CHUNK) void k_index_count(const uint32_t* __restrict__ keys, const uint32_t* __restrict__ excl,
                                                          int n, int shift_top, int ND_top, int32_t* __restrict__ occ_ptr,
                                                          int64_t T, int L, int THR, uint32_t* __restrict__ blk, int NBH) {
  __shared__ uint32_t sh[5][HV_CHUNK / 64];
  __shared__ int sh_lo[SEARCH ? HV_CHUNK + 1 : 1];
  __shared__ uint32_t sh_keys[SEARCH ? IC_STAGE : 1];
  const int tid = threadIdx.x;
  const int64_t e0 = blockIdx.x * (int64_t)HV_CHUNK;
  const int64_t e = e0 + tid;
  uint32_t c = 0;
  if constexpr (SEARCH) {
    auto first_of = [&](int64_t ee, bool past) -> int {
      if (n == 0) return 0;
      const int64_t b = (int64_t)((uint64_t)ee >> shift_top) + (past ? 1 : 0);
      return b >= ND_top ? n : (int)excl[b];
    };
    const int64_t e_hi = e0 + HV_CHUNK < T ? e0 + HV_CHUNK : T;
    const int r_lo = first_of(e0, false), r_hi = first_of(e_hi, true);
    const bool staged = r_hi - r_lo <= IC_STAGE;
    if (staged)
      for (int i = tid; i < r_hi - r_lo; i += HV_CHUNK) sh_keys[i] = keys[r_lo + i];
    __syncthreads();
    auto find = [&](int64_t ee) -> int {
      if (ee >= T || n == 0) return ee > 0 ? n : 0;
      if (staged) {
        int lo = 0, hi = r_hi - r_lo;
        while (lo < hi) {
          const int mid = (lo + hi) >> 1;
          if (sh_keys[mid] < (uint32_t)ee) lo = mid + 1; else hi = mid;
        }
        return r_lo + lo;
      }
      const int b = (int)((uint64_t)ee >> shift_top);
      if (b >= ND_top) return n;
      int lo = (int)excl[b], hi = (int)excl[b + 1];
      while (lo < hi) {
        const int mid = (lo + hi) >> 1;
        if (keys[mid] < (uint32_t)ee) lo = mid + 1; else hi = mid;
      }
      return lo;
    };
    sh_lo[tid] = find(e);
    if (tid == 0) sh_lo[HV_CHUNK] = find(e + HV_CHUNK);
    __syncthreads();
    if (e <= T) occ_ptr[e] = sh_lo[tid];
    if (tid == 0 && e + HV_CHUNK == T) occ_ptr[T] = sh_lo[HV_CHUNK];
    if (e < T) c = (uint32_t)(sh_lo[tid + 1] - sh_lo[tid]);
  } else {
    if (e < T) c = (uint32_t)(occ_ptr[e + 1] - occ_ptr[e]);
  }
  uint32_t v[5];
  v[0] = c;
  ent_counts(c, L, THR, v[1], v[2], v[3]);
  v[4] = v[2];
#pragma unroll
  for (int m = 32; m >= 1; m >>= 1) {
#pragma unroll
    for (int r = 0; r < 4; ++r) v[r] += __shfl_xor(v[r], m, 64);
    const uint32_t o = __shfl_xor(v[4], m, 64);
    v[4] = o > v[4] ? o : v[4];
  }
  if ((tid & 63) == 0)
    for (int r = 0; r < 5; ++r) sh[r][tid >> 6] = v[r];
  __syncthreads();
  if (tid < 5) {
    uint32_t t = 0;
    for (int w = 0; w < HV_CHUNK / 64; ++w) t = tid == 4 ? (sh[4][w] > t ? sh[4][w] : t) : t + sh[tid][w];
    blk[(size_t)tid * NBH + blockIdx.x] = t;
  }
}

__global__ __launch_bounds__(320) void k_index_scan(uint32_t* __restrict__ blk, int NBH) {
  const int w = threadIdx.x >> 6, lane = threadIdx.x & 63;
  uint32_t* row = blk + (size_t)w * NBH;
  uint32_t carry = 0;
  for (int i0 = 0; i0 < NBH; i0 += 64) {
    const int i = i0 + lane;
    const uint32_t v = i < NBH ? row[i] : 0u;
    if (w == 4) {
      uint32_t mx = v;
#pragma unroll
      for (int m = 32; m >= 1; m >>= 1) { const uint32_t o = __shfl_xor(mx, m, 64); mx = o > mx ? o : mx; }
      carry = mx > carry ? mx : carry;
      continue;
    }
    uint32_t inc = v;
#pragma unroll
    for (int o = 1; o < 64; o <<= 1) {
      const uint32_t t = __shfl_up(inc, o, 64);
      if (lane >= o) inc += t;
    }
    if (i < NBH) row[i] = carry + inc - v;
    carry += __shfl(inc, 63, 64);
  }
  if (lane == 0) blk[(size_t)5 * NBH + w] = carry;
}

template <bool SCANNED>
__global__ __launch_bounds__(HV_CHUNK) void k_index_write(const int32_t* __restrict__ occ_ptr, int64_t T, int L, int THR,
                                                          const uint32_t* __restrict__ blk, int NBH,
                                                          int32_t* __restrict__ heavy_ids, int32_t* __restrict__ items,
                                                          int cap_h, int cap_i, int32_t* __restrict__ touched_ids,
                                                          int32_t* __restrict__ counts, const uint32_t* __restrict__ badpart,
                                                          int NB, const double* __restrict__ wpart, double* __restrict__ W,
                                                          int F) {
  __shared__ uint32_t sh[3][HV_CHUNK / 64];
  __shared__ uint32_t sh_bt[7][HV_CHUNK / 64];
  __shared__ uint32_t sh_base[7];
  const int tid = threadIdx.x, me = blockIdx.x;
  const bool last = me == (int)gridDim.x - 1;
  if constexpr (SCANNED) {
    if (tid < 3) { sh_base[tid] = blk[(size_t)(1 + tid) * NBH + me]; sh_base[3 + tid] = blk[(size_t)5 * NBH + 1 + tid]; }
    if (tid == 3) sh_base[6] = blk[(size_t)5 * NBH + 4];
  } else {
    uint32_t b[7] = {0u, 0u, 0u, 0u, 0u, 0u, 0u};
    for (int j = tid; j < NBH; j += HV_CHUNK) {
#pragma unroll
      for (int r = 0; r < 3; ++r) {
        const uint32_t v = blk[(size_t)(1 + r) * NBH + j];
        b[r] += j < me ? v : 0u;
        b[3 + r] += v;
      }
      const uint32_t v4 = blk[(size_t)4 * NBH + j];
      b[6] = v4 > b[6] ? v4 : b[6];
    }
#pragma unroll
    for (int m = 32; m >= 1; m >>= 1) {
#pragma unroll
      for (int r = 0; r < 6; ++r) b[r] += __shfl_xor(b[r], m, 64);
      const uint32_t o = __shfl_xor(b[6], m, 64);
      b[6] = o > b[6] ? o : b[6];
    }
    if ((tid & 63) == 0)
      for (int r = 0; r < 7; ++r) sh_bt[r][tid >> 6] = b[r];
    __syncthreads();
    if (tid < 7) {
      uint32_t t = 0;
      for (int w = 0; w < HV_CHUNK / 64; ++w) t = tid == 6 ? (sh_bt[6][w] > t ? sh_bt[6][w] : t) : t + sh_bt[tid][w];
      sh_base[tid] = t;
    }
  }
  const int64_t e = me * (int64_t)HV_CHUNK + tid;
  int beg = 0;
  uint32_t c = 0;
  if (e < T) { beg = occ_ptr[e]; c = (uint32_t)(occ_ptr[e + 1] - beg); }
  uint32_t v[3];
  ent_counts(c, L, THR, v[0], v[1], v[2]);
  uint32_t inc[3] = {v[0], v[1], v[2]};
#pragma unroll
  for (int o = 1; o < 64; o <<= 1) {
#pragma unroll
    for (int r = 0; r < 3; ++r) {
      const uint32_t t = __shfl_up(inc[r], o, 64);
      if ((tid & 63) >= o) inc[r] += t;
    }
  }
  if ((tid & 63) == 63)
    for (int r = 0; r < 3; ++r) sh[r][tid >> 6] = inc[r];
  __syncthreads();
  if (tid < 3) {
    uint32_t r = 0;
    for (int w = 0; w < HV_CHUNK / 64; ++w) { const uint32_t t = sh[tid][w]; sh[tid][w] = r; r += t; }
  }
  __syncthreads();
  uint32_t ex[3];
#pragma unroll
  for (int r = 0; r < 3; ++r) ex[r] = sh_base[r] + sh[r][tid >> 6] + inc[r] - v[r];
  if (v[2] && touched_ids) touched_ids[ex[2]] = (int32_t)e;
  if (v[0]) {
    const uint32_t slot = ex[0];
    uint32_t it = ex[1];
    if (slot < (uint32_t)cap_h) heavy_ids[slot] = (int32_t)e;
    const int end = beg + (int)c;
    for (int o = beg; o < end; o += L, ++it) {
      if (it < (uint32_t)cap_i) {
        const int oe = (o + L < end) ? o + L : end;
        *reinterpret_cast<int4*>(items + 4 * (size_t)it) = make_int4((int)slot, o, oe, 0);
      }
    }
  }
  if (last) {
    if (tid >= 1 && tid < 4) counts[tid] = (int32_t)sh_base[2 + tid];
    if (tid == 4) counts[4] = (int32_t)sh_base[6];
    if (tid >= 5 && tid < 8) counts[tid] = 0;
    if (tid < 64) {
      uint32_t b = 0;
      if (badpart)
        for (int j = tid; j < NB; j += 64) b += badpart[j];
#pragma unroll
      for (int m = 32; m >= 1; m >>= 1) b += __shfl_xor(b, m, 64);
      if (tid == 0) counts[0] = (int32_t)b;
    }
    if (W) {
      const int lane = tid & 63;
      for (int f = tid >> 6; f < F && f < NW_MAXF; f += HV_CHUNK / 64) {
        double t = 0.0;
        if (wpart)
          for (int j = lane; j < NB; j += 64) t += wpart[(size_t)j * NW_MAXF + f];
#pragma unroll
        for (int m = 32; m >= 1; m >>= 1) t += __shfl_xor(t, m, 64);
        if (lane == 0) W[f] = t;
      }
    }
  }
}

__device__ __forceinline__ bool in_either(const int32_t* a, const int32_t* b, int64_t e, int64_t T) {
  return e < T && (a[e + 1] != a[e] || b[e + 1] != b[e]);
}
__global__ __launch_bounds__(HV_CHUNK) void k_union_count(const int32_t* __restrict__ occ_a, const int32_t* __restrict__ occ_b,
                                                          int64_t T, uint32_t* __restrict__ blk) {
  __shared__ uint32_t sh[HV_CHUNK / 64];
  const int64_t e = blockIdx.x * (int64_t)HV_CHUNK + threadIdx.x;
  const unsigned long long m = __ballot(in_either(occ_a, occ_b, e, T));
  if ((threadIdx.x & 63) == 0) sh[threadIdx.x >> 6] = (uint32_t)__popcll(m);
  __syncthreads();
  if (threadIdx.x == 0) {
    uint32_t t = 0;
    for (int w = 0; w < HV_CHUNK / 64; ++w) t += sh[w];
    blk[blockIdx.x] = t;
  }
}
__global__ __launch_bounds__(64) void k_union_scan(uint32_t* __restrict__ blk, int NBH, int32_t* __restrict__ count) {
  const int lane = threadIdx.x;
  uint32_t carry = 0;
  for (int i0 = 0; i0 < NBH; i0 += 64) {
    const int i = i0 + lane;
    const uint32_t v = i < NBH ? blk[i] : 0u;
    uint32_t inc = v;
#pragma unroll
    for (int o = 1; o < 64; o <<= 1) {
      const uint32_t t = __shfl_up(inc, o, 64);
      if (lane >= o) inc += t;
    }
    if (i < NBH) blk[i] = carry + inc - v;
    carry += __shfl(inc, 63, 64);
  }
  if (lane == 0) count[0] = (int32_t)carry;
}
template <bool SCANNED>
__global__ __launch_bounds__(HV_CHUNK) void k_union_write(const int32_t* __restrict__ occ_a, const int32_t* __restrict__ occ_b,
                                                          int64_t T, const uint32_t* __restrict__ blk, int NBH,
                                                          int32_t* __restrict__ rows, int32_t* __restrict__ count) {
  __shared__ uint32_t sh[HV_CHUNK / 64];
  __shared__ uint32_t sh_bt[2][HV_CHUNK / 64];
  __shared__ uint32_t sh_base[2];
  const int tid = threadIdx.x, lane = tid & 63, me = blockIdx.x;
  if constexpr (SCANNED) {
    if (tid == 0) sh_base[0] = blk[me];
  } else {
    uint32_t b0 = 0, b1 = 0;
    for (int j = tid; j < NBH; j += HV_CHUNK) { const uint32_t v = blk[j]; b0 += j < me ? v : 0u; b1 += v; }
#pragma unroll
    for (int m = 32; m >= 1; m >>= 1) { b0 += __shfl_xor(b0, m, 64); b1 += __shfl_xor(b1, m, 64); }
    if (lane == 0) { sh_bt[0][tid >> 6] = b0; sh_bt[1][tid >> 6] = b1; }
    __syncthreads();
    if (tid < 2) {
      uint32_t t = 0;
      for (int w = 0; w < HV_CHUNK / 64; ++w) t += sh_bt[tid][w];
      sh_base[tid] = t;
      if (tid == 1 && me == 0) count[0] = (int32_t)t;
    }
  }
  const int64_t e = me * (int64_t)HV_CHUNK + tid;
  const bool in = in_either(occ_a, occ_b, e, T);
  const unsigned long long m = __ballot(in);
  if (lane == 0) sh[tid >> 6] = (uint32_t)__popcll(m);
  __syncthreads();
  uint32_t wbase = 0;
  for (int w = 0; w < (tid >> 6); ++w) wbase += sh[w];
  const unsigned long long lt = (lane == 0) ? 0ull : (~0ull >> (64 - lane));
  if (in) rows[sh_base[0] + wbase + (uint32_t)__popcll(m & lt)] = (int32_t)e;
}

int compaction_write(int64_t NBH64, const int32_t* occ_ptr, int64_t T, int L, int THR, uint32_t* blk, int32_t* heavy_ids,
                     int32_t* items, int64_t cap_heavy, int64_t cap_items, int32_t* touched_ids, int32_t* counts,
                     const uint32_t* badpart, int NB, const double* wpart, double* W, int F, hipStream_t st) {
  const int NBH = (int)NBH64;
  const int ch = (int)(cap_heavy > 0x7FFFFFFF ? 0x7FFFFFFF : cap_heavy), ci = (int)(cap_items > 0x7FFFFFFF ? 0x7FFFFFFF : cap_items);
  if (NBH > HV_SELF) {
    hipLaunchKernelGGL(k_index_scan, dim3(1), dim3(320), 0, st, blk, NBH);
    hipLaunchKernelGGL(k_index_write<true>, dim3(NBH), dim3(HV_CHUNK), 0, st, occ_ptr, T, L, THR, blk, NBH, heavy_ids, items,
                       ch, ci, touched_ids, counts, badpart, NB, wpart, W, F);
  } else {
    hipLaunchKernelGGL(k_index_write<false>, dim3(NBH), dim3(HV_CHUNK), 0, st, occ_ptr, T, L, THR, blk, NBH, heavy_ids, items,
                       ch, ci, touched_ids, counts, badpart, NB, wpart, W, F);
  }
  return 0;
}

}
}

using namespace vfm;

extern "C" {

int32_t vfm_heavy_list_for(int64_t n_occ, int64_t T) {
  const int forced = env_int("VFM_HEAVY_LIST", 0);
  if (forced > 0) return forced < VFM_HEAVY_MIN ? VFM_HEAVY_MIN : forced;
  if (T >= VFM_HEAVY_UNITS) return VFM_HEAVY_LIST;
  const int64_t l = n_occ / VFM_HEAVY_UNITS;
  return (int32_t)(l < VFM_HEAVY_MIN ? VFM_HEAVY_MIN : (l > VFM_HEAVY_LIST ? VFM_HEAVY_LIST : l));
}

int32_t vfm_heavy_threshold(int32_t heavy_list) {
  int thr = env_int("VFM_HEAVY_THR", heavy_list / 4);
  if (thr > heavy_list) thr = heavy_list;
  return thr < VFM_HEAVY_MIN ? VFM_HEAVY_MIN : thr;
}

int64_t vfm_index_workspace_bytes(int64_t B, int32_t F, int64_t T) {
  if (B < 0 || F < 1 || T < 1 || T > 0xFFFFFFFELL || B * (int64_t)F > 0x7FFFFFFFLL) return -1;
  return geometry(B * F, T).total * 4;
}

int64_t vfm_union_workspace_bytes(int64_t T) { return T < 1 ? -1 : 4 * ((T + HV_CHUNK - 1) / HV_CHUNK + 4); }

int vfm_union_rows(int64_t T, const int32_t* occ_ptr_a, const int32_t* occ_ptr_b, void* ws, int32_t* rows, int32_t* count,
                   int32_t* count_host, void* stream) {
  if (T < 1 || T > 0x7FFFFFFELL || !occ_ptr_a || !occ_ptr_b || !ws || !rows || !count)
    return fail(VFM_E_INVALID, "vfm_union_rows: bad argument");
  hipStream_t st = (hipStream_t)stream;
  const int NBH = (int)((T + HV_CHUNK - 1) / HV_CHUNK);
  uint32_t* blk = reinterpret_cast<uint32_t*>(ws);
  hipLaunchKernelGGL(k_union_count, dim3(NBH), dim3(HV_CHUNK), 0, st, occ_ptr_a, occ_ptr_b, T, blk);
  if (NBH > HV_SELF) {
    hipLaunchKernelGGL(k_union_scan, dim3(1), dim3(64), 0, st, blk, NBH, count);
    hipLaunchKernelGGL(k_union_write<true>, dim3(NBH), dim3(HV_CHUNK), 0, st, occ_ptr_a, occ_ptr_b, T, blk, NBH, rows, count);
  } else {
    hipLaunchKernelGGL(k_union_write<false>, dim3(NBH), dim3(HV_CHUNK), 0, st, occ_ptr_a, occ_ptr_b, T, blk, NBH, rows, count);
  }
  hipError_t e = hipSuccess;
  if (count_host) e = hipMemcpyAsync(count_host, count, sizeof(int32_t), hipMemcpyDeviceToHost, st);
  if (e == hipSuccess) e = hipGetLastError();
  return e == hipSuccess ? 0 : fail_hip(e, "vfm_union_rows");
}

int vfm_build_index(int64_t B, int32_t F, int64_t T, int32_t id_bits, const void* x, void* ws, int32_t* occ_ptr,
                    int32_t* occ_rows, int32_t heavy_list, int32_t* heavy_ids, int64_t cap_heavy,
                    int32_t* heavy_items, int64_t cap_items, int32_t* touched_ids, int32_t* occ_other,
                    const float* inv_occ, double* W, int32_t* counts, int32_t* counts_host, void* stream) {
  if (B < 0 || F < 1 || F > VFM_MAX_FIELDS || T < 1 || T > 0xFFFFFFFELL || B * (int64_t)F > 0x7FFFFFFFLL ||
      (id_bits != 32 && id_bits != 64) || heavy_list < VFM_HEAVY_MIN)
    return fail(VFM_E_INVALID, "vfm_build_index: bad B, F, T, id_bits or heavy_list");
  if (occ_other && F != 2) return fail(VFM_E_INVALID, "vfm_build_index: occ_other is defined for two fields");
  if (!ws || !occ_ptr || !counts || (B > 0 && (!x || !occ_rows)) || cap_heavy < 0 || cap_items < 0 ||
      (cap_heavy > 0 && !heavy_ids) || (cap_items > 0 && !heavy_items))
    return fail(VFM_E_INVALID, "vfm_build_index: NULL pointer");
  if ((inv_occ == nullptr) != (W == nullptr)) return fail(VFM_E_INVALID, "vfm_build_index: give inv_occ and W together, or neither");
  if ((((uintptr_t)ws) & 15) != 0) return fail(VFM_E_INVALID, "vfm_build_index: ws must be 16-byte aligned");
  hipStream_t st = (hipStream_t)stream;
  const Geo g = geometry(B * F, T);
  const int n = (int)g.n, NB = (int)g.NB;
  uint32_t* w32 = reinterpret_cast<uint32_t*>(ws);
  const bool fused_w = W != nullptr && F <= NW_MAXF;
  if (W != nullptr && !fused_w)
    if (int rc = launch_norms(B, F, T, id_bits, x, inv_occ, W, st)) return rc;
  hipError_t e = hipSuccess;
  if (B > 0) e = hipMemsetAsync(w32 + g.zero_lo, 0, (size_t)(g.zero_hi - g.zero_lo) * 4, st);
  if (e != hipSuccess) return fail_hip(e, "vfm_build_index: memset");
  double* wpart = reinterpret_cast<double*>(w32 + g.wpart);
  if (n > 0) {
    hipLaunchKernelGGL(k_index_keys, dim3(NB), dim3(RS_THREADS), 0, st, x, (int)(id_bits == 64), n, (uint32_t)T, (int)F,
                       w32 + g.k0, w32 + g.v0, g.rb[0], w32 + g.L1[0], w32 + g.L2[0], (int)g.G,
                       fused_w ? inv_occ : (const float*)nullptr, wpart, w32 + g.bad);
    uint32_t *kin = w32 + g.k0, *vin = w32 + g.v0, *kout = w32 + g.k1, *vout = w32 + g.v1;
    for (int p = 0; p < g.passes; ++p) {
      if (p > 0)
        hipLaunchKernelGGL(k_radix_hist, dim3(NB), dim3(RS_THREADS), 0, st, kin, n, g.shift[p], g.rb[p], w32 + g.L1[p],
                           w32 + g.L2[p], (int)g.G);
      if (p + 1 == g.passes) {
        hipLaunchKernelGGL(k_radix_scatter<true>, dim3(NB), dim3(RS_THREADS), 0, st, kin, vin, n, g.shift[p], g.rb[p],
                           w32 + g.L1[p], w32 + g.L2[p], (int)g.G, (int)g.NS, kout, vout, w32 + g.excl, occ_rows, occ_other, x,
                           (int)(id_bits == 64), (int)F, T);
      } else {
        hipLaunchKernelGGL(k_radix_scatter<false>, dim3(NB), dim3(RS_THREADS), 0, st, kin, vin, n, g.shift[p], g.rb[p],
                           w32 + g.L1[p], w32 + g.L2[p], (int)g.G, (int)g.NS, kout, vout, (uint32_t*)nullptr, occ_rows, occ_other,
                           x, (int)(id_bits == 64), (int)F, T);
      }
      uint32_t* t = kin; kin = kout; kout = t;
      t = vin; vin = vout; vout = t;
    }
    hipLaunchKernelGGL(k_index_count<true>, dim3((unsigned)g.NBH), dim3(HV_CHUNK), 0, st, kin, w32 + g.excl, n,
                       g.shift[g.passes - 1], 1 << g.rb[g.passes - 1], occ_ptr, T, (int)heavy_list, (int)heavy_list, w32 + g.blk,
                       (int)g.NBH);
  } else {
    e = hipMemsetAsync(occ_ptr, 0, sizeof(int32_t) * (size_t)(T + 1), st);
    if (e != hipSuccess) return fail_hip(e, "vfm_build_index: memset of occ_ptr");
    hipLaunchKernelGGL(k_index_count<false>, dim3((unsigned)g.NBH), dim3(HV_CHUNK), 0, st, (const uint32_t*)nullptr,
                       (const uint32_t*)nullptr, 0, 0, 1, occ_ptr, T, (int)heavy_list, (int)heavy_list, w32 + g.blk, (int)g.NBH);
  }
  compaction_write(g.NBH, occ_ptr, T, (int)heavy_list, (int)heavy_list, w32 + g.blk, heavy_ids, heavy_items, cap_heavy, cap_items,
                   touched_ids, counts, n > 0 ? w32 + g.bad : (const uint32_t*)nullptr, NB, fused_w && n > 0 ? wpart : nullptr,
                   fused_w ? W : nullptr, (int)F, st);
  if (counts_host) {
    e = hipMemcpyAsync(counts_host, counts, 8 * sizeof(int32_t), hipMemcpyDeviceToHost, st);
    if (e != hipSuccess) return fail_hip(e, "vfm_build_index: readback");
  }
  e = hipGetLastError();
  if (e != hipSuccess) return fail_hip(e, "vfm_build_index");
  return 0;
}

int vfm_rebuild_heavy(int64_t T, const int32_t* occ_ptr, void* ws, int32_t heavy_list, int32_t threshold, int32_t* heavy_ids,
                      int64_t cap_heavy, int32_t* heavy_items, int64_t cap_items, int32_t* counts, void* stream) {
  if (T < 1 || T > 0xFFFFFFFELL || !occ_ptr || !ws || !counts || heavy_list < VFM_HEAVY_MIN || threshold < VFM_HEAVY_MIN ||
      threshold > heavy_list || cap_heavy < 0 || cap_items < 0 || (cap_heavy > 0 && !heavy_ids) || (cap_items > 0 && !heavy_items))
    return fail(VFM_E_INVALID, "vfm_rebuild_heavy: bad argument (VFM_HEAVY_MIN <= threshold <= heavy_list)");
  hipStream_t st = (hipStream_t)stream;
  const int64_t NBH = (T + HV_CHUNK - 1) / HV_CHUNK;
  uint32_t* blk = reinterpret_cast<uint32_t*>(ws);
  hipLaunchKernelGGL(k_index_count<false>, dim3((unsigned)NBH), dim3(HV_CHUNK), 0, st, (const uint32_t*)nullptr,
                     (const uint32_t*)nullptr, 0, 0, 1, const_cast<int32_t*>(occ_ptr), T, (int)heavy_list, (int)threshold, blk,
                     (int)NBH);
  compaction_write(NBH, occ_ptr, T, (int)heavy_list, (int)threshold, blk, heavy_ids, heavy_items, cap_heavy, cap_items, nullptr,
                   counts, nullptr, 0, nullptr, nullptr, 0, st);
  const hipError_t e = hipGetLastError();
  if (e != hipSuccess) return fail_hip(e, "vfm_rebuild_heavy");
  return 0;
}

}
```

### vae_amd/csrc/vfm_torch_ops.cpp

```cpp
#include <ATen/ATen.h>
#include <c10/hip/HIPGuard.h>
#include <c10/hip/HIPStream.h>
#include <torch/library.h>

#include <string.h>

#include "vfm_hip.h"

namespace {

using at::Tensor;
using c10::optional;

void check(int rc, const char* what) {
  TORCH_CHECK(rc == 0, what, " failed (code ", rc, "): ", vfm_last_error());
}

const Tensor& dev_tensor(const Tensor& t, at::ScalarType dt, const char* name) {
  TORCH_CHECK(t.is_cuda(), name, " must be on the GPU (vae_amd has no CPU fallback)");
  TORCH_CHECK(t.scalar_type() == dt, name, " has the wrong dtype");
  TORCH_CHECK(t.is_contiguous(), name, " must be contiguous");
  return t;
}
const float* fptr(const optional<Tensor>& t, const char* name) {
  if (!t.has_value() || !t->defined()) return nullptr;
  return dev_tensor(*t, at::kFloat, name).data_ptr<float>();
}
float* fptr_mut(const optional<Tensor>& t, const char* name) { return const_cast<float*>(fptr(t, name)); }

vfm_problem_t problem(const Tensor& x_like, int64_t B, int64_t B_global, int64_t T, int64_t F, int64_t d,
                      int64_t nb_train, int64_t likelihood, int64_t id_bits, int64_t flags,
                      at::IntArrayRef group_hi, at::ArrayRef<double> group_n, int64_t seed, int64_t step,
                      int64_t n_samples = 1) {
  TORCH_CHECK(F >= 1 && F <= VFM_MAX_FIELDS, "F out of range");
  TORCH_CHECK(n_samples >= 1 && n_samples <= 64, "n_samples out of range [1,64]");
  TORCH_CHECK((int64_t)group_hi.size() == F && (int64_t)group_n.size() == F, "group_hi / group_n need F entries");
  vfm_problem_t p;
  VFM_STRUCT_INIT(p);
  p.B = B; p.B_global = B_global; p.T = T; p.nb_train = nb_train;
  p.F = (int32_t)F; p.d = (int32_t)d; p.likelihood = (int32_t)likelihood; p.id_bits = (int32_t)id_bits;
  p.n_samples = (int32_t)n_samples; p.flags = (int32_t)flags;
  for (int64_t g = 0; g < F; ++g) { p.group_hi[g] = group_hi[g]; p.group_n[g] = group_n[g]; }
  p.seed = (uint64_t)seed; p.step = (uint64_t)step;
  return p;
}

void extensions(vfm_problem_t& p, const optional<Tensor>& wrec, const optional<Tensor>& dev_step, int64_t T) {
  if (wrec.has_value() && wrec->defined()) {
    TORCH_CHECK(dev_tensor(*wrec, at::kFloat, "wrec").numel() >= 4 * T, "wrec needs [T,4] floats");
    p.wrec = wrec->data_ptr<float>();
  }
  if (dev_step.has_value() && dev_step->defined()) {
    TORCH_CHECK(dev_tensor(*dev_step, at::kLong, "dev_step").numel() >= 8, "dev_step needs 8 int64 (vfm_dev_step_t)");
    p.dev_step = reinterpret_cast<vfm_dev_step_t*>(dev_step->data_ptr<int64_t>());
  }
}

struct Ids {
  const void* ptr; int64_t B, F; int id_bits;
};
Ids ids_of(const Tensor& x) {
  TORCH_CHECK(x.is_cuda() && x.is_contiguous() && x.dim() == 2, "x must be a contiguous [B,F] GPU tensor");
  TORCH_CHECK(x.scalar_type() == at::kLong || x.scalar_type() == at::kInt, "x must be int64 or int32");
  return {x.data_ptr(), x.size(0), x.size(1), x.scalar_type() == at::kLong ? 64 : 32};
}

void* stream_of(const Tensor& t) { return (void*)c10::hip::getCurrentHIPStream(t.get_device()).stream(); }

void elbo_fwd(const Tensor& x, const optional<Tensor>& y, const Tensor& entity, const Tensor& bias,
              const optional<Tensor>& inv_occ, const Tensor& scalars, const optional<Tensor>& W,
              const optional<Tensor>& eps_entity, const optional<Tensor>& eps_bias,
              const optional<Tensor>& eps_global, Tensor pred, Tensor partials,
              const optional<Tensor>& sumz, const optional<Tensor>& grow, at::IntArrayRef group_hi,
              at::ArrayRef<double> group_n, int64_t nb_train, int64_t B_global, int64_t likelihood,
              int64_t flags, int64_t seed, int64_t step, int64_t n_samples,
              const optional<Tensor>& wrec, const optional<Tensor>& dev_step) {
  const Ids id = ids_of(x);
  dev_tensor(entity, at::kFloat, "entity_params"); dev_tensor(bias, at::kFloat, "bias_params");
  dev_tensor(scalars, at::kFloat, "scalars"); dev_tensor(pred, at::kFloat, "pred");
  dev_tensor(partials, at::kDouble, "partials");
  TORCH_CHECK(entity.dim() == 2 && bias.dim() == 2 && bias.size(1) == 2 && bias.size(0) == entity.size(0) &&
              entity.size(1) % 2 == 0, "table shapes");
  TORCH_CHECK(n_samples >= 1 && pred.numel() >= n_samples * id.B && partials.numel() >= VFM_PARTIALS_LEN &&
              scalars.numel() >= 3, "output sizes");
  const int64_t T = entity.size(0), d = entity.size(1) / 2;
  if (sumz.has_value() && sumz->defined()) TORCH_CHECK(sumz->numel() >= n_samples * id.B * d, "sumz too small");
  if (eps_entity.has_value() && eps_entity->defined())
    TORCH_CHECK(eps_entity->numel() >= n_samples * T * d && eps_bias.has_value() && eps_bias->defined() &&
                eps_bias->numel() >= n_samples * T && eps_global.has_value() && eps_global->defined() &&
                eps_global->numel() >= n_samples, "eps tables too small for n_samples");
  c10::hip::HIPGuard guard(x.get_device());
  vfm_problem_t p = problem(x, id.B, B_global, T, id.F, d, nb_train, likelihood, id.id_bits, flags, group_hi,
                            group_n, seed, step, n_samples);
  extensions(p, wrec, dev_step, T);
  const double* Wp = (W.has_value() && W->defined()) ? dev_tensor(*W, at::kDouble, "W").data_ptr<double>() : nullptr;
  check(vfm_elbo_fwd_f32(&p, id.ptr, fptr(y, "y"), entity.data_ptr<float>(), bias.data_ptr<float>(),
                         fptr(inv_occ, "inv_occ"), scalars.data_ptr<float>(), Wp, fptr(eps_entity, "eps_entity"),
                         fptr(eps_bias, "eps_bias"), fptr(eps_global, "eps_global"), pred.data_ptr<float>(),
                         partials.data_ptr<double>(), fptr_mut(sumz, "sumz"), fptr_mut(grow, "grow"),
                         stream_of(x)),
        "vfm_elbo_fwd_f32");
}

void elbo_finalize(Tensor partials, const Tensor& scalars, Tensor loss, int64_t nb_train, int64_t B_global,
                   int64_t flags, int64_t n_samples) {
  dev_tensor(partials, at::kDouble, "partials"); dev_tensor(scalars, at::kFloat, "scalars");
  dev_tensor(loss, at::kFloat, "loss");
  TORCH_CHECK(loss.numel() >= 3, "loss needs 3 entries");
  c10::hip::HIPGuard guard(partials.get_device());
  vfm_problem_t p;
  VFM_STRUCT_INIT(p);
  p.B = 0; p.B_global = B_global; p.T = 1; p.nb_train = nb_train; p.F = 1; p.d = 4; p.id_bits = 64;
  TORCH_CHECK(n_samples >= 1 && n_samples <= 64, "n_samples out of range [1,64]");
  p.n_samples = (int32_t)n_samples; p.flags = (int32_t)flags; p.group_hi[0] = 1; p.group_n[0] = 1;
  check(vfm_elbo_finalize_f32(&p, partials.data_ptr<double>(), scalars.data_ptr<float>(), loss.data_ptr<float>(),
                              stream_of(partials)),
        "vfm_elbo_finalize_f32");
}

int64_t rec_len(int64_t d) { return 4 + ((d + 3) / 4) * 4; }

vfm_index_t index_of(at::TensorList index_all, int64_t T, int64_t B, int64_t F, int64_t d, int64_t n_samples = 1) {
  int32_t max_items = 0, heavy_list = 0, heavy_threshold = 0;
  if (index_all.size() > 0 && index_all[index_all.size() - 1].is_cpu()) {
    const at::Tensor& meta = index_all[index_all.size() - 1];
    TORCH_CHECK(meta.scalar_type() == at::kInt && meta.numel() >= 3,
                "index: the trailing host tensor holds int32 [max_items, heavy_list, heavy_threshold]");
    max_items = meta.data_ptr<int32_t>()[0];
    heavy_list = meta.data_ptr<int32_t>()[1];
    heavy_threshold = meta.data_ptr<int32_t>()[2];
    index_all = index_all.slice(0, index_all.size() - 1);
  }
  TORCH_CHECK(index_all.size() == 3 || index_all.size() == 4 || index_all.size() == 6 || index_all.size() == 7,
              "index = [occ_ptr, occ_rows, status] (+ [heavy_ids, heavy_items, heavy_acc]) (+ [touched_ids])");
  const bool has_touched = index_all.size() == 4 || index_all.size() == 7;
  const bool has_heavy = index_all.size() >= 6;
  dev_tensor(index_all[0], at::kInt, "occ_ptr"); dev_tensor(index_all[1], at::kInt, "occ_rows");
  dev_tensor(index_all[2], at::kInt, "index status");
  TORCH_CHECK(index_all[0].numel() == T + 1 && index_all[1].numel() == B * F && index_all[2].numel() == 1, "inverted index sizes");
  vfm_index_t ix;
  VFM_STRUCT_INIT(ix);
  ix.occ_ptr = index_all[0].data_ptr<int32_t>(); ix.occ_rows = index_all[1].data_ptr<int32_t>();
  ix.status = index_all[2].data_ptr<int32_t>();
  ix.heavy_list = heavy_list; ix.heavy_threshold = heavy_threshold;
  if (has_heavy && index_all[3].numel() > 0) {
    const at::Tensor &hid = index_all[3], &items = index_all[4], &hacc = index_all[5];
    dev_tensor(hid, at::kInt, "heavy_ids"); dev_tensor(items, at::kInt, "heavy_items"); dev_tensor(hacc, at::kFloat, "heavy_acc");
    TORCH_CHECK(items.numel() % 4 == 0 && hacc.numel() >= n_samples * (hid.numel() + items.numel() / 4) * rec_len(d),
                "heavy index sizes");
    ix.heavy_ids = hid.data_ptr<int32_t>(); ix.heavy_items = items.data_ptr<int32_t>(); ix.heavy_acc = hacc.data_ptr<float>();
    ix.n_heavy = (int32_t)hid.numel(); ix.n_items = (int32_t)(items.numel() / 4);
    ix.max_items = max_items;
  }
  if (has_touched) {
    const at::Tensor& t = index_all[index_all.size() - 1];
    dev_tensor(t, at::kInt, "touched_ids");
    ix.touched_ids = t.numel() > 0 ? t.data_ptr<int32_t>() : nullptr; ix.n_touched = t.numel();
  }
  return ix;
}

struct BwdCommon {
  vfm_problem_t p; vfm_index_t ix;
};

BwdCommon bwd_common(at::TensorList index, const Tensor& entity, const Tensor& bias,
                     int64_t B, int64_t F, int64_t B_global, int64_t nb_train, int64_t likelihood, int64_t flags,
                     at::IntArrayRef group_hi, at::ArrayRef<double> group_n, int64_t seed, int64_t step,
                     int64_t n_samples, const Tensor& sumz, const optional<Tensor>& eps_entity,
                     const optional<Tensor>& eps_bias, const optional<Tensor>& eps_global) {
  dev_tensor(entity, at::kFloat, "entity_params"); dev_tensor(bias, at::kFloat, "bias_params");
  const int64_t T = entity.size(0), d = entity.size(1) / 2;
  TORCH_CHECK(n_samples >= 1 && sumz.numel() >= n_samples * B * d, "sumz too small for n_samples");
  if (eps_entity.has_value() && eps_entity->defined())
    TORCH_CHECK(eps_entity->numel() >= n_samples * T * d && eps_bias.has_value() && eps_bias->defined() &&
                eps_bias->numel() >= n_samples * T && eps_global.has_value() && eps_global->defined() &&
                eps_global->numel() >= n_samples, "eps tables too small for n_samples");
  return {problem(entity, B, B_global, T, F, d, nb_train, likelihood, 64, flags, group_hi, group_n, seed, step,
                  n_samples),
          index_of(index, T, B, F, d, n_samples)};
}

void elbo_bwd(at::TensorList index, const Tensor& entity, const Tensor& bias,
              const Tensor& inv_occ, const Tensor& scalars, const Tensor& W, const optional<Tensor>& eps_entity,
              const optional<Tensor>& eps_bias, const optional<Tensor>& eps_global, const Tensor& sumz,
              const Tensor& grow, const Tensor& partials, const Tensor& grad_out, Tensor g_entity, Tensor g_bias,
              Tensor g_scalars, int64_t F, at::IntArrayRef group_hi, at::ArrayRef<double> group_n,
              int64_t nb_train, int64_t B_global, int64_t likelihood, int64_t flags, int64_t seed, int64_t step,
              int64_t n_samples) {
  const int64_t B = grow.numel();
  BwdCommon c = bwd_common(index, entity, bias, B, F, B_global, nb_train, likelihood, flags, group_hi,
                           group_n, seed, step, n_samples, sumz, eps_entity, eps_bias, eps_global);
  TORCH_CHECK(g_entity.sizes() == entity.sizes() && g_bias.sizes() == bias.sizes() && g_scalars.numel() >= 3,
              "gradient shapes");
  c10::hip::HIPGuard guard(entity.get_device());
  check(vfm_elbo_bwd_f32(&c.p, &c.ix, entity.data_ptr<float>(), bias.data_ptr<float>(),
                         dev_tensor(inv_occ, at::kFloat, "inv_occ").data_ptr<float>(),
                         dev_tensor(scalars, at::kFloat, "scalars").data_ptr<float>(),
                         dev_tensor(W, at::kDouble, "W").data_ptr<double>(), fptr(eps_entity, "eps_entity"),
                         fptr(eps_bias, "eps_bias"), fptr(eps_global, "eps_global"),
                         dev_tensor(sumz, at::kFloat, "sumz").data_ptr<float>(),
                         dev_tensor(grow, at::kFloat, "grow").data_ptr<float>(),
                         dev_tensor(partials, at::kDouble, "partials").data_ptr<double>(),
                         dev_tensor(grad_out, at::kFloat, "grad_out").data_ptr<float>(),
                         dev_tensor(g_entity, at::kFloat, "g_entity").data_ptr<float>(),
                         dev_tensor(g_bias, at::kFloat, "g_bias").data_ptr<float>(),
                         dev_tensor(g_scalars, at::kFloat, "g_scalars").data_ptr<float>(), stream_of(entity)),
        "vfm_elbo_bwd_f32");
}

void elbo_bwd_adam(at::TensorList index, Tensor entity, Tensor bias, Tensor scalars,
                   const Tensor& inv_occ, const Tensor& W, const optional<Tensor>& eps_entity,
                   const optional<Tensor>& eps_bias, const optional<Tensor>& eps_global, const Tensor& sumz,
                   const Tensor& grow, const Tensor& partials, Tensor m_entity, Tensor v_entity, Tensor m_bias,
                   Tensor v_bias, Tensor m_scalars, Tensor v_scalars, int64_t F, at::IntArrayRef group_hi,
                   at::ArrayRef<double> group_n, int64_t nb_train, int64_t B_global, int64_t likelihood,
                   int64_t flags, int64_t seed, int64_t step, double lr, double beta1, double beta2,
                   double eps_adam, int64_t adam_step, const optional<Tensor>& loss, int64_t n_samples,
                   const optional<Tensor>& wrec, const optional<Tensor>& dev_step) {
  const int64_t B = grow.numel();
  BwdCommon c = bwd_common(index, entity, bias, B, F, B_global, nb_train, likelihood, flags, group_hi,
                           group_n, seed, step, n_samples, sumz, eps_entity, eps_bias, eps_global);
  extensions(c.p, wrec, dev_step, entity.size(0));
  TORCH_CHECK(m_entity.numel() == entity.numel() && v_entity.numel() == entity.numel() &&
              m_bias.numel() == bias.numel() && v_bias.numel() == bias.numel() && m_scalars.numel() >= 3 &&
              v_scalars.numel() >= 3, "Adam moment shapes");
  c10::hip::HIPGuard guard(entity.get_device());
  check(vfm_elbo_bwd_adam_f32(
            &c.p, &c.ix, entity.data_ptr<float>(), bias.data_ptr<float>(),
            dev_tensor(scalars, at::kFloat, "scalars").data_ptr<float>(),
            dev_tensor(inv_occ, at::kFloat, "inv_occ").data_ptr<float>(),
            dev_tensor(W, at::kDouble, "W").data_ptr<double>(), fptr(eps_entity, "eps_entity"),
            fptr(eps_bias, "eps_bias"), fptr(eps_global, "eps_global"),
            dev_tensor(sumz, at::kFloat, "sumz").data_ptr<float>(), dev_tensor(grow, at::kFloat, "grow").data_ptr<float>(),
            dev_tensor(partials, at::kDouble, "partials").data_ptr<double>(),
            dev_tensor(m_entity, at::kFloat, "m_entity").data_ptr<float>(),
            dev_tensor(v_entity, at::kFloat, "v_entity").data_ptr<float>(),
            dev_tensor(m_bias, at::kFloat, "m_bias").data_ptr<float>(),
            dev_tensor(v_bias, at::kFloat, "v_bias").data_ptr<float>(),
            dev_tensor(m_scalars, at::kFloat, "m_scalars").data_ptr<float>(),
            dev_tensor(v_scalars, at::kFloat, "v_scalars").data_ptr<float>(), (float)lr, (float)beta1, (float)beta2,
            (float)eps_adam, adam_step, fptr_mut(loss, "loss"), stream_of(entity)),
        "vfm_elbo_bwd_adam_f32");
}

void elbo_bwd_acc(at::TensorList index, const Tensor& sumz, const Tensor& grow,
                  const Tensor& partials, Tensor acc, Tensor sums, int64_t T, int64_t F, int64_t d, int64_t e_lo,
                  int64_t e_hi) {
  dev_tensor(acc, at::kFloat, "acc"); dev_tensor(sums, at::kFloat, "sums");
  const int64_t B = grow.numel();
  TORCH_CHECK(acc.numel() >= T * rec_len(d) && sums.numel() >= 2, "bwd_acc sizes");
  vfm_index_t ix = index_of(index, T, B, F, d);
  c10::hip::HIPGuard guard(acc.get_device());
  vfm_problem_t p;
  VFM_STRUCT_INIT(p);
  p.B = B; p.B_global = B; p.T = T; p.nb_train = 1; p.F = (int32_t)F; p.d = (int32_t)d; p.id_bits = 64;
  p.n_samples = 1; p.e_lo = e_lo; p.e_hi = e_hi;
  for (int64_t g = 0; g < F; ++g) { p.group_hi[g] = T; p.group_n[g] = 1; }
  check(vfm_elbo_bwd_acc_f32(&p, &ix,
                             dev_tensor(sumz, at::kFloat, "sumz").data_ptr<float>(),
                             dev_tensor(grow, at::kFloat, "grow").data_ptr<float>(),
                             dev_tensor(partials, at::kDouble, "partials").data_ptr<double>(),
                             acc.data_ptr<float>(), sums.data_ptr<float>(), stream_of(acc)),
        "vfm_elbo_bwd_acc_f32");
}

void elbo_apply_adam(const Tensor& acc, const Tensor& sums, Tensor entity, Tensor bias,
                     Tensor scalars, const Tensor& inv_occ, const Tensor& W, const optional<Tensor>& eps_entity,
                     const optional<Tensor>& eps_bias, const optional<Tensor>& eps_global, Tensor m_entity,
                     Tensor v_entity, Tensor m_bias, Tensor v_bias, Tensor m_scalars, Tensor v_scalars, int64_t F,
                     at::IntArrayRef group_hi, at::ArrayRef<double> group_n, int64_t nb_train, int64_t B_global,
                     int64_t likelihood, int64_t flags, int64_t seed, int64_t step, double lr, double beta1,
                     double beta2, double eps_adam, int64_t adam_step, int64_t e_lo, int64_t e_hi) {
  dev_tensor(entity, at::kFloat, "entity_params"); dev_tensor(bias, at::kFloat, "bias_params");
  const int64_t T = entity.size(0), d = entity.size(1) / 2;
  TORCH_CHECK(acc.numel() >= T * rec_len(d), "apply_adam sizes");
  TORCH_CHECK(sums.numel() >= 2, "sums size");
  TORCH_CHECK(m_entity.numel() == entity.numel() && v_entity.numel() == entity.numel() &&
              m_bias.numel() == bias.numel() && v_bias.numel() == bias.numel(), "Adam moment shapes");
  c10::hip::HIPGuard guard(entity.get_device());
  vfm_problem_t p = problem(entity, 0, B_global, T, F, d, nb_train, likelihood, 64, flags, group_hi, group_n, seed, step);
  p.e_lo = e_lo; p.e_hi = e_hi;
  check(vfm_elbo_apply_adam_f32(
            &p, dev_tensor(acc, at::kFloat, "acc").data_ptr<float>(), dev_tensor(sums, at::kFloat, "sums").data_ptr<float>(),
            entity.data_ptr<float>(), bias.data_ptr<float>(), dev_tensor(scalars, at::kFloat, "scalars").data_ptr<float>(),
            dev_tensor(inv_occ, at::kFloat, "inv_occ").data_ptr<float>(), dev_tensor(W, at::kDouble, "W").data_ptr<double>(),
            fptr(eps_entity, "eps_entity"), fptr(eps_bias, "eps_bias"), fptr(eps_global, "eps_global"),
            dev_tensor(m_entity, at::kFloat, "m_entity").data_ptr<float>(),
            dev_tensor(v_entity, at::kFloat, "v_entity").data_ptr<float>(),
            dev_tensor(m_bias, at::kFloat, "m_bias").data_ptr<float>(), dev_tensor(v_bias, at::kFloat, "v_bias").data_ptr<float>(),
            dev_tensor(m_scalars, at::kFloat, "m_scalars").data_ptr<float>(),
            dev_tensor(v_scalars, at::kFloat, "v_scalars").data_ptr<float>(), (float)lr, (float)beta1, (float)beta2,
            (float)eps_adam, adam_step, stream_of(entity)),
        "vfm_elbo_apply_adam_f32");
}

void adam(Tensor p, const Tensor& g, Tensor m, Tensor v, double lr, double beta1, double beta2, double eps,
          int64_t step) {
  dev_tensor(p, at::kFloat, "p"); dev_tensor(g, at::kFloat, "g"); dev_tensor(m, at::kFloat, "m");
  dev_tensor(v, at::kFloat, "v");
  TORCH_CHECK(g.numel() >= p.numel() && m.numel() == p.numel() && v.numel() == p.numel(), "adam sizes");
  c10::hip::HIPGuard guard(p.get_device());
  check(vfm_adam_f32(p.data_ptr<float>(), g.data_ptr<float>(), m.data_ptr<float>(), v.data_ptr<float>(), p.numel(),
                     (float)lr, (float)beta1, (float)beta2, (float)eps, step, stream_of(p)),
        "vfm_adam_f32");
}

void moments_rescale(Tensor m, Tensor v, double beta1, double beta2, int64_t step, bool to_scaled) {
  dev_tensor(m, at::kFloat, "m"); dev_tensor(v, at::kFloat, "v");
  TORCH_CHECK(m.numel() == v.numel(), "moment sizes");
  c10::hip::HIPGuard guard(m.get_device());
  check(vfm_moments_rescale_f32(m.data_ptr<float>(), v.data_ptr<float>(), m.numel(), (float)beta1, (float)beta2, step,
                                to_scaled ? 1 : 0, stream_of(m)),
        "vfm_moments_rescale_f32");
}

int64_t abi_version() { return vfm_abi_version(); }

}

TORCH_LIBRARY(vfm_hip, m) {
  m.def("abi_version() -> int", &abi_version);
  m.def("elbo_fwd(Tensor x, Tensor? y, Tensor entity_params, Tensor bias_params, Tensor? inv_occ, Tensor scalars, "
        "Tensor? W, Tensor? eps_entity, Tensor? eps_bias, Tensor? eps_global, Tensor(a!) pred, Tensor(b!) partials, "
        "Tensor(c!)? sumz, Tensor(d!)? grow, int[] group_hi, float[] group_n, int nb_train, int B_global, "
        "int likelihood, int flags, int seed, int step, int n_samples=1, Tensor(e!)? wrec=None, "
        "Tensor(f!)? dev_step=None) -> ()", &elbo_fwd);
  m.def("elbo_finalize(Tensor(a!) partials, Tensor scalars, Tensor(b!) loss, int nb_train, int B_global, int flags, "
        "int n_samples=1) -> ()",
        &elbo_finalize);
  m.def("elbo_bwd(Tensor[] index, Tensor entity_params, Tensor bias_params, Tensor inv_occ, "
        "Tensor scalars, Tensor W, Tensor? eps_entity, Tensor? eps_bias, Tensor? eps_global, Tensor sumz, Tensor grow, "
        "Tensor partials, Tensor grad_out, Tensor(a!) g_entity, Tensor(b!) g_bias, Tensor(c!) g_scalars, int F, "
        "int[] group_hi, float[] group_n, int nb_train, int B_global, int likelihood, int flags, int seed, int step, "
        "int n_samples=1) -> ()",
        &elbo_bwd);
  m.def("elbo_bwd_adam(Tensor[] index, Tensor(a!) entity_params, Tensor(b!) bias_params, "
        "Tensor(c!) scalars, Tensor inv_occ, Tensor W, Tensor? eps_entity, Tensor? eps_bias, Tensor? eps_global, "
        "Tensor sumz, Tensor grow, Tensor partials, Tensor(d!) m_entity, Tensor(e!) v_entity, Tensor(f!) m_bias, "
        "Tensor(g!) v_bias, Tensor(h!) m_scalars, Tensor(i!) v_scalars, int F, int[] group_hi, float[] group_n, "
        "int nb_train, int B_global, int likelihood, int flags, int seed, int step, float lr, float beta1, "
        "float beta2, float eps_adam, int adam_step, Tensor(j!)? loss, int n_samples=1, "
        "Tensor(k!)? wrec=None, Tensor(l!)? dev_step=None) -> ()",
        &elbo_bwd_adam);
  m.def("elbo_bwd_acc(Tensor[] index, Tensor sumz, Tensor grow, Tensor partials, Tensor(a!) acc, "
        "Tensor(c!) sums, int T, int F, int d, int e_lo, int e_hi) -> ()", &elbo_bwd_acc);
  m.def("elbo_apply_adam(Tensor acc, Tensor sums, Tensor(a!) entity_params, Tensor(b!) bias_params, "
        "Tensor(c!) scalars, Tensor inv_occ, Tensor W, Tensor? eps_entity, Tensor? eps_bias, Tensor? eps_global, "
        "Tensor(d!) m_entity, Tensor(e!) v_entity, Tensor(f!) m_bias, Tensor(g!) v_bias, Tensor(h!) m_scalars, "
        "Tensor(i!) v_scalars, int F, int[] group_hi, float[] group_n, int nb_train, int B_global, int likelihood, "
        "int flags, int seed, int step, float lr, float beta1, float beta2, float eps_adam, int adam_step, "
        "int e_lo, int e_hi) -> ()",
        &elbo_apply_adam);
  m.def("moments_rescale(Tensor(a!) m, Tensor(b!) v, float beta1, float beta2, int step, bool to_scaled) -> ()",
        &moments_rescale);
  m.def("adam(Tensor(a!) p, Tensor g, Tensor(b!) m, Tensor(c!) v, float lr, float beta1, float beta2, float eps, "
        "int step) -> ()", &adam);
}
```

### vae_amd/ops.py

```python
from __future__ import annotations

import contextlib
import ctypes as C
from dataclasses import dataclass
from typing import Optional

import torch

from . import _lib
from ._lib import Problem, check, ptr, current_stream_ptr

FLAG_NO_PRIOR_TERMS = 1
FLAG_EPS_ZERO = 2
FLAG_SPARSE_ADAM = 4
FLAG_LINK_SOFTPLUS = 16
FLAG_SCALED_MOMENTS = 32
FLAG_ROWS_TOUCHED = 128
FLAG_SHARE_GPU = 2048
MOMENT_PERIOD = 128
MAX_SAMPLES = 64
_I63 = (1 << 63) - 1


@dataclass
class Spec:
    T: int
    F: int
    d: int
    group_hi: tuple
    group_n: tuple
    likelihood: int
    nb_train: int = 1
    n_samples: int = 1
    link: str = "abs"

    def __post_init__(self):
        if self.link not in ("abs", "softplus"):
            raise ValueError("link must be 'abs' or 'softplus'")
        if not 1 <= int(self.n_samples) <= MAX_SAMPLES:
            raise ValueError(f"n_samples must be in [1,{MAX_SAMPLES}]")

    @property
    def link_flag(self) -> int:
        return FLAG_LINK_SOFTPLUS if self.link == "softplus" else 0


def _problem(spec: Spec, B: int, B_global: int, id_bits: int, seed: int = 0, step: int = 0,
             flags: int = 0, wrec=None, dev_step=None) -> Problem:
    p = Problem()
    if wrec is not None:
        p.wrec = wrec.data_ptr()
    if dev_step is not None:
        p.dev_step = dev_step.data_ptr()
    p.B, p.B_global, p.T, p.nb_train = B, B_global, spec.T, spec.nb_train
    p.F, p.d, p.likelihood, p.id_bits = spec.F, spec.d, spec.likelihood, id_bits
    p.n_samples, p.flags = int(spec.n_samples), flags | spec.link_flag
    for g in range(spec.F):
        p.group_hi[g] = int(spec.group_hi[g])
        p.group_n[g] = float(spec.group_n[g])
    p.seed, p.step = seed & (2 ** 64 - 1), step & (2 ** 62 - 1)
    return p


def _need_cuda(t: torch.Tensor, name: str):
    if not t.is_cuda:
        raise _lib.VfmLibraryError(
            f"{name} is on {t.device}: vae_amd runs on an MI355X only (no CPU fallback)")
    if not t.is_contiguous():
        raise ValueError(f"{name} must be contiguous")


def inv_occ_from_counts(nb_occ: torch.Tensor) -> torch.Tensor:
    _need_cuda(nb_occ, "nb_occ")
    assert nb_occ.dtype == torch.int64
    out = torch.empty(nb_occ.numel(), dtype=torch.float32, device=nb_occ.device)
    lib = _lib.load()
    check(lib.vfm_inv_occ_f32(ptr(nb_occ), ptr(out), nb_occ.numel(), current_stream_ptr(nb_occ.device)),
          "vfm_inv_occ_f32")
    return out


_WS = {}
_ENQUEUE_LOCK = __import__("threading").RLock()


def _index_workspace(n_int32: int, dev, stream: int) -> torch.Tensor:
    key = (dev.index, stream)
    t = _WS.get(key)
    if t is None or t.numel() < n_int32:
        with torch.cuda.stream(_stream_obj(dev, stream)):
            t = _WS[key] = torch.empty(n_int32, dtype=torch.int32, device=dev)
    return t


_ARENAS = {}


def _side_arena(dev, stream, numel: int) -> torch.Tensor:
    key = (dev.index, stream.cuda_stream, numel)
    stash = _ARENAS.get(key)
    if not stash:
        if len(_ARENAS) > 8:
            _ARENAS.clear()
        with torch.cuda.stream(stream):
            stash = _ARENAS[key] = [torch.empty(numel, dtype=torch.int32, device=dev) for _ in range(8)]
    return stash.pop()


_STREAMS = {}


def _stream_obj(dev, raw: int):
    s = _STREAMS.get((dev.index, raw))
    if s is None:
        s = torch.cuda.current_stream(dev)
        if s.cuda_stream != raw:
            s = torch.cuda.ExternalStream(raw, device=dev)
        if len(_STREAMS) > 64:
            _STREAMS.clear()
        _STREAMS[(dev.index, raw)] = s
    return s


_SIZES = {}


def _index_sizes(B: int, F: int, T: int):
    hit = _SIZES.get((B, F, T))
    if hit is None:
        lib = _lib.load()
        hit = (_lib.heavy_list_for(B * F, T), int(lib.vfm_index_workspace_bytes(B, F, T)))
        if len(_SIZES) > 256:
            _SIZES.clear()
        _SIZES[(B, F, T)] = hit
    return hit


_PINNED = {"chunk": None, "used": 0}


def _pinned_ints(n: int) -> torch.Tensor:
    if _PINNED["chunk"] is None or _PINNED["used"] + n > _PINNED["chunk"].numel():
        _PINNED["chunk"] = torch.empty(max(1024, n), dtype=torch.int32, pin_memory=True)
        _PINNED["used"] = 0
    t = _PINNED["chunk"][_PINNED["used"]:_PINNED["used"] + n]
    _PINNED["used"] += n
    return t


def _carve(total_dev, sizes):
    out, off = [], 0
    for n in sizes:
        out.append(total_dev[off:off + n])
        off += (n + 3) & ~3
    return out


class BatchPlan:

    def __init__(self, spec: Spec, x: torch.Tensor, y: Optional[torch.Tensor],
                 inv_occ: Optional[torch.Tensor], B_global: Optional[int] = None,
                 build_index: bool = True, validate: bool = True, process_group=None, defer_readback: bool = False,
                 stream=None):
        _need_cuda(x, "x")
        if x.dim() != 2 or x.shape[1] != spec.F:
            raise ValueError(f"x must be [B,{spec.F}], got {tuple(x.shape)}")
        if x.dtype not in (torch.int64, torch.int32):
            raise TypeError("x must be int64 or int32")
        self.spec = spec
        self.x = x
        self.B = x.shape[0]
        self.B_global = self.B if B_global is None else int(B_global)
        self.id_bits = 64 if x.dtype == torch.int64 else 32
        self.y = None
        if y is not None:
            _need_cuda(y, "y")
            self.y = y.to(torch.float32).contiguous()
            if self.y.shape != (self.B,):
                raise ValueError("y must be [B]")
        self.W = None
        self.occ_ptr = None
        self._occ_rows = self._status = self._occ_other = self._lay = None
        self._ready = None
        self._arena = None
        self._heavy = self._pend = None
        self._U = 0
        self._touched = None
        self._checked = False
        dev = x.device
        lib = _lib.load()
        want_w = inv_occ is not None and y is not None
        if want_w and not (build_index and y is not None):
            self.W = torch.empty(spec.F, dtype=torch.float64, device=dev)
        if build_index and y is not None:
            self.build_index(validate=validate, defer=defer_readback, inv_occ=inv_occ if want_w else None, stream=stream)
        elif want_w:
            p = _problem(spec, self.B, self.B_global, self.id_bits)
            check(lib.vfm_batch_norms(C.byref(p), ptr(x), ptr(inv_occ), ptr(self.W),
                                      current_stream_ptr(dev)), "vfm_batch_norms")
        if want_w and process_group is not None:
            from .dist import sum_normalisers
            sum_normalisers(self.W, process_group)
        if build_index and y is not None:
            pass
        elif validate and self.B > 0:
            if bool(((x < 0) | (x >= spec.T)).any()):
                raise IndexError(f"entity id out of range [0,{spec.T}): min {int(x.min())}, max {int(x.max())}")
            self._checked = True

    def build_index(self, validate: bool = False, defer: bool = False, inv_occ=None, stream=None):
        spec = self.spec
        n = self.B * spec.F
        L, nbytes = _index_sizes(self.B, spec.F, spec.T)
        self.heavy_list = L
        if nbytes < 0:
            raise ValueError("batch too large for a 32-bit index (B * F must stay below 2^31)")
        with _ENQUEUE_LOCK:
            self._build_index_locked(_lib.load(), n, L, nbytes, validate, inv_occ, stream)
        if not defer:
            self._finish()

    def _build_index_locked(self, lib, n, L, nbytes, validate, inv_occ=None, stream=None):
        spec, dev = self.spec, self.x.device
        raw = stream.cuda_stream if stream is not None else _lib.raw_stream(dev)
        ws = _index_workspace(nbytes // 4 + 4, dev, raw)
        cap_h, cap_i = n // L + 1, 2 * n // L + 2
        sizes = (spec.T + 1, max(n, 1), cap_h, 4 * cap_i, 8, max(min(n, spec.T), 1), max(n, 1) if spec.F == 2 else 0,
                 2 * spec.F if inv_occ is not None else 0)
        offs, o = [], 0
        for v in sizes:
            offs.append(o)
            o += (v + 3) & ~3
        arena = self._arena = torch.empty(o, dtype=torch.int32, device=dev) if stream is None else _side_arena(dev, stream, o)
        self._lay = (offs, sizes, cap_i)
        if inv_occ is not None:
            self.W = arena[offs[7]: offs[7] + 2 * spec.F].view(torch.float64)
        base = arena.data_ptr()
        P = [C.c_void_p(base + 4 * q) for q in offs]
        host = _pinned_ints(8)
        check(lib.vfm_build_index(self.B, spec.F, spec.T, self.id_bits, ptr(self.x), ptr(ws), P[0], P[1], L, P[2], cap_h, P[3],
                                  cap_i, P[5], P[6] if spec.F == 2 else None, ptr(inv_occ),
                                  ptr(self.W) if inv_occ is not None else None, P[4], C.c_void_p(host.data_ptr()),
                                  C.c_void_p(raw)), "vfm_build_index")
        self.occ_ptr = arena[: spec.T + 1]
        done = torch.cuda.Event()
        done.record(stream if stream is not None else _stream_obj(dev, raw))
        self._pend = (host, done, validate)

    def _view(self, k):
        offs, sizes, _ = self._lay
        return self._arena[offs[k]: offs[k] + sizes[k]]

    @property
    def occ_rows(self):
        if self._occ_rows is None and self._arena is not None:
            self._occ_rows = self._view(1)[: self.B * self.spec.F]
        return self._occ_rows

    @property
    def status(self):
        if self._status is None and self._arena is not None:
            self._status = self._view(4)[5:6]
        return self._status

    @property
    def occ_other(self):
        if self._occ_other is None and self._arena is not None and self.spec.F == 2:
            self._occ_other = self._view(6)
        return self._occ_other

    def _finish(self):
        if self._pend is None:
            return
        self.use_on_current()
        host, done, validate = self._pend
        self._pend = None
        done.synchronize()
        n_bad, n_heavy, n_items, n_touched, max_items = (int(v) for v in host.tolist()[:5])
        spec, dev = self.spec, self.x.device
        hid, items, touched = self._view(2), self._view(3).view(self._lay[2], 4), self._view(5)
        self._U = n_touched
        self._touched = touched[:n_touched]
        thr = int(_lib.load().vfm_heavy_threshold(self.heavy_list))
        if (n_touched > 0 and self.B >= 4 * n_touched and 4 * n_touched <= spec.T and spec.T >= 8192
                and thr < self.heavy_list and not n_bad):
            n, L = self.B * spec.F, self.heavy_list
            cap_h, cap_i = n // thr + 1, n // L + n // thr + 2
            arena = torch.empty(((cap_h + 3) & ~3) + 4 * cap_i + 8, dtype=torch.int32, device=dev)
            hid, items, counts2 = arena[:cap_h], arena[(cap_h + 3) & ~3:((cap_h + 3) & ~3) + 4 * cap_i].view(cap_i, 4), arena[-8:]
            lib = _lib.load()
            with _ENQUEUE_LOCK:
                ws = _index_workspace(int(lib.vfm_index_workspace_bytes(self.B, spec.F, spec.T)) // 4 + 4, dev, _lib.raw_stream(dev))
                check(lib.vfm_rebuild_heavy(spec.T, ptr(self.occ_ptr), ptr(ws), L, thr, ptr(hid), cap_h, ptr(items), cap_i,
                                            ptr(counts2), current_stream_ptr(dev)), "vfm_rebuild_heavy")
                _, n_heavy, n_items, _, max_items = (int(v) for v in counts2.tolist()[:5])
            self.heavy_threshold = thr
        if validate and n_bad and not self._checked:
            raise IndexError(f"entity id out of range [0,{spec.T}): min {int(self.x.min())}, max {int(self.x.max())}")
        self._checked = True
        self._heavy = None
        self.heavy_max_items = max_items if n_heavy > 0 else 0
        self._heavy_meta = torch.tensor([self.heavy_max_items, self.heavy_list, getattr(self, "heavy_threshold", self.heavy_list)],
                                        dtype=torch.int32)
        if n_heavy > 0:
            rec = 4 + (spec.d + 3) // 4 * 4
            self._heavy = (hid[:n_heavy], items[:n_items],
                           torch.zeros(spec.n_samples * (n_heavy + n_items) * rec, dtype=torch.float32, device=dev))

    @property
    def U(self) -> int:
        if self.occ_ptr is None:
            self.build_index()
        self._finish()
        return self._U

    @property
    def heavy(self):
        self._finish()
        return self._heavy

    def touched_ids(self) -> torch.Tensor:
        if self.occ_ptr is None:
            self.build_index()
        self._finish()
        return self._touched

    def lookahead_rows(self, next_plan: "BatchPlan") -> torch.Tensor:
        pairs = self.__dict__.setdefault("_pairs", {})
        hit = pairs.get(id(next_plan))
        if hit is not None and hit[0]() is next_plan:
            if hit[2] is not None:
                host, done, src = hit[2]
                done.synchronize()
                cur = _stream_obj(self.x.device, _lib.raw_stream(self.x.device))
                if src.cuda_stream != cur.cuda_stream:
                    hit[1].record_stream(cur)
                pairs[id(next_plan)] = (hit[0], hit[1][:int(host.item())], None)
            return pairs[id(next_plan)][1]
        self.prepare_lookahead(next_plan)
        return self.lookahead_rows(next_plan)

    def prepare_lookahead(self, next_plan: "BatchPlan", stream=None) -> None:
        import weakref
        pairs = self.__dict__.setdefault("_pairs", {})
        hit = pairs.get(id(next_plan))
        if hit is not None and hit[0]() is next_plan:
            return
        dev, T = self.x.device, self.spec.T
        for q in (self, next_plan):
            if q.occ_ptr is None:
                q.build_index(defer=True, stream=stream)
        lib = _lib.load()
        raw = stream.cuda_stream if stream is not None else _lib.raw_stream(dev)
        with (torch.cuda.stream(stream) if stream is not None else contextlib.nullcontext()):
            buf = torch.empty((min(T, (self.B + next_plan.B) * self.spec.F) or 1) + 4, dtype=torch.int32, device=dev)
        rows, count = buf[:-4], buf[-4:]
        with _ENQUEUE_LOCK:
            ws = _index_workspace(int(lib.vfm_union_workspace_bytes(T)) // 4 + 4, dev, raw)
            host = _pinned_ints(1)
            check(lib.vfm_union_rows(T, ptr(self.occ_ptr), ptr(next_plan.occ_ptr), ptr(ws), ptr(rows), ptr(count),
                                     C.c_void_p(host.data_ptr()), C.c_void_p(raw)), "vfm_union_rows")
            done = torch.cuda.Event()
            src = stream if stream is not None else _stream_obj(dev, raw)
            done.record(src)
        pairs[id(next_plan)] = (weakref.ref(next_plan), rows, (host, done, src))
        if len(pairs) > 4:
            pairs.pop(next(iter(pairs)))

    def use_on_current(self):
        if self._ready is None:
            return
        ev, src = self._ready
        dev = self.x.device
        raw = _lib.raw_stream(dev)
        if raw != src.cuda_stream:
            cur = _stream_obj(dev, raw)
            cur.wait_event(ev)
            if self._arena is not None:
                self._arena.record_stream(cur)
        self._ready = None

    def check_status(self):
        if self.occ_ptr is not None and int(self.status.item()) != 0:
            raise _lib.VfmLibraryError("corrupted inverted index: a backward kernel clamped entries of this plan's index "
                                       "(vfm_index_t.status != 0); the step's results are not to be trusted")

    def index_tensors(self, with_touched: bool = False):
        if self.occ_ptr is None:
            self.build_index()
        self._finish()
        base = [self.occ_ptr, self.occ_rows, self.status]
        if self.heavy is not None:
            base = base + list(self.heavy)
        if with_touched:
            base = base + [self._touched]
        return base + [self._heavy_meta]


def _index_struct(plan: BatchPlan) -> "_lib.Index":
    if plan.occ_ptr is None:
        plan.build_index()
    plan._finish()
    ix = _lib.Index()
    ix.occ_ptr, ix.occ_rows, ix.status = plan.occ_ptr.data_ptr(), plan.occ_rows.data_ptr(), plan.status.data_ptr()
    ix.heavy_list, ix.heavy_threshold = plan.heavy_list, getattr(plan, "heavy_threshold", plan.heavy_list)
    if plan.heavy is not None:
        hid, items, acc = plan.heavy
        ix.heavy_ids, ix.heavy_items, ix.heavy_acc = hid.data_ptr(), items.data_ptr(), acc.data_ptr()
        ix.n_heavy, ix.n_items = hid.numel(), items.numel() // 4
        ix.max_items = plan.heavy_max_items
    return ix


class PlanStream:

    def __init__(self, device, n_streams: Optional[int] = None):
        import os
        self.device = torch.device(device)
        n = int(os.environ.get("VFM_PLAN_STREAMS", "2")) if n_streams is None else int(n_streams)
        prio = int(os.environ.get("VFM_PLAN_PRIORITY", "-1"))
        self.streams = [torch.cuda.Stream(self.device, priority=prio) for _ in range(max(1, n))]
        self._turn = 0

    @property
    def stream(self):
        return self.streams[self._turn % len(self.streams)]

    def wait_current(self):
        ev = torch.cuda.Event()
        ev.record(_stream_obj(self.device, _lib.raw_stream(self.device)))
        for st in self.streams:
            st.wait_event(ev)

    def build(self, make, pair_with: Optional[BatchPlan] = None, fork: bool = True) -> BatchPlan:
        self._turn += 1
        st = self.stream
        if fork:
            main = _stream_obj(self.device, _lib.raw_stream(self.device))
            ev0 = torch.cuda.Event()
            ev0.record(main)
            st.wait_event(ev0)
        plan = make(st)
        if pair_with is not None:
            if pair_with._ready is not None and pair_with._ready[1] is not st:
                st.wait_event(pair_with._ready[0])
            pair_with.prepare_lookahead(plan, stream=st)
        ev = torch.cuda.Event()
        ev.record(st)
        plan._ready = (ev, st)
        return plan


@dataclass
class FwdState:
    pred: torch.Tensor
    partials: torch.Tensor
    sumz: Optional[torch.Tensor]
    grow: Optional[torch.Tensor]
    problem: Problem
    eps: Optional[tuple]


def elbo_forward(plan: BatchPlan, entity_params, bias_params, scalars, inv_occ, *, eps=None,
                 seed=0, step=0, train=True, flags=0, out_pred=None, out_sumz=None,
                 out_grow=None, out_partials=None, wrec=None, dev_step=None) -> FwdState:
    spec = plan.spec
    dev = plan.x.device
    for t, n in ((entity_params, "entity_params"), (bias_params, "bias_params"), (scalars, "scalars")):
        _need_cuda(t, n)
    if entity_params.shape != (spec.T, 2 * spec.d) or bias_params.shape != (spec.T, 2):
        raise ValueError("table shapes do not match the spec")
    have_y = plan.y is not None
    train = train and have_y
    B, S = plan.B, int(spec.n_samples)
    pshape = (B,) if S == 1 else (S, B)
    pred = out_pred if out_pred is not None else torch.empty(pshape, dtype=torch.float32, device=dev)
    partials = out_partials if out_partials is not None else torch.empty(
        _lib.PARTIALS_LEN, dtype=torch.float64, device=dev)
    sumz = grow = None
    if train:
        sumz = out_sumz if out_sumz is not None else torch.empty(S * B, spec.d, dtype=torch.float32, device=dev)
        grow = out_grow if out_grow is not None else torch.empty(B, dtype=torch.float32, device=dev)
    p = _problem(spec, B, plan.B_global, plan.id_bits, seed, step, flags)
    e = eps if eps is not None else (None, None, None)
    _lib.ops().elbo_fwd(plan.x, plan.y, entity_params, bias_params, inv_occ if have_y else None, scalars,
                        plan.W if have_y else None, e[0], e[1], e[2], pred, partials, sumz, grow,
                        list(spec.group_hi), list(spec.group_n), spec.nb_train, plan.B_global,
                        spec.likelihood, p.flags, p.seed & _I63, p.step, S,
                        wrec if (train and eps is None) else None, dev_step)
    return FwdState(pred, partials, sumz, grow, p, eps)


def elbo_finalize(st: FwdState, scalars, out=None) -> torch.Tensor:
    loss = out if out is not None else torch.empty(3, dtype=torch.float32, device=scalars.device)
    p = st.problem
    _lib.ops().elbo_finalize(st.partials, scalars, loss, p.nb_train, p.B_global, p.flags, p.n_samples)
    return loss


def elbo_backward(plan: BatchPlan, st: FwdState, entity_params, bias_params, scalars, inv_occ,
                  grad_out, g_entity=None, g_bias=None, g_scalars=None):
    dev = plan.x.device
    if plan.occ_ptr is None:
        plan.build_index()
    if g_entity is None:
        g_entity = torch.empty_like(entity_params)
    if g_bias is None:
        g_bias = torch.empty_like(bias_params)
    if g_scalars is None:
        g_scalars = torch.empty(3, dtype=torch.float32, device=dev)
    e = st.eps if st.eps is not None else (None, None, None)
    p, spec = st.problem, plan.spec
    _lib.ops().elbo_bwd(plan.index_tensors(), entity_params, bias_params, inv_occ, scalars, plan.W,
                        e[0], e[1], e[2], st.sumz, st.grow, st.partials, grad_out, g_entity, g_bias, g_scalars,
                        spec.F, list(spec.group_hi), list(spec.group_n), p.nb_train, p.B_global, p.likelihood,
                        p.flags, p.seed & _I63, p.step, p.n_samples)
    return g_entity, g_bias, g_scalars


def elbo_backward_adam(plan: BatchPlan, st: FwdState, entity_params, bias_params, scalars, inv_occ,
                       m_views, v_views, lr, step, beta1=0.9, beta2=0.999, eps_adam=1e-8, loss_out=None,
                       sparse=False, scaled_moments=False, rows=None, wrec=None, dev_step=None):
    rows_flag = {None: 0, "touched": FLAG_ROWS_TOUCHED}[rows]
    if plan.occ_ptr is None:
        plan.build_index()
    e = st.eps if st.eps is not None else (None, None, None)
    p, spec = st.problem, plan.spec
    _lib.ops().elbo_bwd_adam(plan.index_tensors(with_touched=rows == "touched"), entity_params, bias_params, scalars,
                             inv_occ, plan.W,
                             e[0], e[1], e[2], st.sumz, st.grow, st.partials, m_views[0], v_views[0],
                             m_views[1], v_views[1], m_views[2], v_views[2], spec.F, list(spec.group_hi),
                             list(spec.group_n), p.nb_train, p.B_global, p.likelihood,
                             p.flags | (FLAG_SPARSE_ADAM if sparse else 0) |
                             (FLAG_SCALED_MOMENTS if scaled_moments else 0) | rows_flag,
                             p.seed & _I63, p.step, lr, beta1, beta2, eps_adam, int(step), loss_out, p.n_samples,
                             wrec, dev_step)


FLAG_ZREC = 1024


def record_len(d: int) -> int:
    return 4 + d


def pipeline_supported(spec: Spec) -> bool:
    return spec.F == 2 and int(spec.n_samples) == 1 and spec.d % 4 == 0 and spec.d <= 512 and spec.link == "abs"


def sample_records(plan: BatchPlan, entity_params, bias_params, inv_occ, zrec, seed, step):
    p = _problem(plan.spec, plan.B, plan.B_global, plan.id_bits, seed, step, 0)
    ids = plan.touched_ids()
    check(_lib.load().vfm_sample_records_f32(C.byref(p), ptr(ids), ids.numel(), ptr(entity_params), ptr(bias_params),
                                             ptr(inv_occ), ptr(plan.W), ptr(zrec), current_stream_ptr(zrec.device)),
          "vfm_sample_records_f32")


def elbo_forward_records(plan: BatchPlan, zrec, scalars, seed, step, out_pred, out_grow, out_partials, dev_step=None, flags=0) -> FwdState:
    spec = plan.spec
    p = _problem(spec, plan.B, plan.B_global, plan.id_bits, seed, step, FLAG_ZREC | flags, dev_step=dev_step)
    check(_lib.load().vfm_elbo_fwd_f32(C.byref(p), ptr(plan.x), ptr(plan.y), ptr(zrec), None, None, ptr(scalars), None,
                                       None, None, None, ptr(out_pred), ptr(out_partials), None, ptr(out_grow),
                                       current_stream_ptr(zrec.device)), "vfm_elbo_fwd_f32 (records)")
    p.flags = spec.link_flag | (flags & FLAG_SHARE_GPU)
    return FwdState(out_pred, out_partials, None, out_grow, p, None)


def elbo_backward_adam_pipe(plan: BatchPlan, st: FwdState, zrec, zrec_next, next_plan, next_step, entity_params,
                            bias_params, scalars, inv_occ, m_views, v_views, lr, step, loss_out, beta1=0.9, beta2=0.999,
                            eps_adam=1e-8, scaled_moments=True, wrec=None, dev_step=None, last_step=None, step_tab=None,
                            listed=True, la_next=None):
    ix = _index_struct(plan)
    ix.occ_other = plan.occ_other.data_ptr()
    pipe = _lib.Pipe()
    pipe.zrec = zrec.data_ptr()
    if next_plan is not None:
        if next_plan.occ_ptr is None:
            next_plan.build_index()
        pipe.zrec_next, pipe.next_occ_ptr, pipe.next_W = zrec_next.data_ptr(), next_plan.occ_ptr.data_ptr(), next_plan.W.data_ptr()
        pipe.next_step = int(next_step)
    if last_step is not None:
        if la_next.occ_ptr is None:
            la_next.build_index()
        pipe.last_step, pipe.step_tab = last_step.data_ptr(), step_tab.data_ptr()
        pipe.next_occ_ptr = la_next.occ_ptr.data_ptr()
        if next_plan is not None and next_plan is not la_next:
            raise ValueError("pipelined look-ahead step: the records are prepared for the batch the look-ahead names")
        if listed:
            rows = plan.lookahead_rows(la_next)
            if rows.numel() > 0:
                ix.touched_ids, ix.n_touched = rows.data_ptr(), rows.numel()
    p = st.problem
    p.flags = plan.spec.link_flag | (FLAG_SCALED_MOMENTS if scaled_moments else 0) | (p.flags & FLAG_SHARE_GPU)
    p.wrec = wrec.data_ptr() if wrec is not None else None
    p.dev_step = dev_step.data_ptr() if dev_step is not None else None
    check(_lib.load().vfm_elbo_bwd_adam_pipe_f32(
        C.byref(p), C.byref(ix), C.byref(pipe), ptr(entity_params), ptr(bias_params), ptr(scalars), ptr(inv_occ),
        ptr(plan.W), ptr(st.grow), ptr(st.partials), ptr(m_views[0]), ptr(v_views[0]), ptr(m_views[1]), ptr(v_views[1]),
        ptr(m_views[2]), ptr(v_views[2]), lr, beta1, beta2, eps_adam, int(step), ptr(loss_out),
        current_stream_ptr(zrec.device)), "vfm_elbo_bwd_adam_pipe_f32")


def elbo_backward_adam_lookahead(plan: BatchPlan, st: FwdState, next_plan: BatchPlan, entity_params, bias_params,
                                 scalars, inv_occ, m_views, v_views, lr, step, loss_out, last_step, step_tab,
                                 beta1=0.9, beta2=0.999, eps_adam=1e-8, listed=True, wrec=None, dev_step=None):
    ix = _index_struct(plan)
    if listed:
        rows = plan.lookahead_rows(next_plan)
        if rows.numel() > 0:
            ix.touched_ids, ix.n_touched = rows.data_ptr(), rows.numel()
    if next_plan.occ_ptr is None:
        next_plan.build_index()
    p = st.problem
    share = p.flags & FLAG_SHARE_GPU
    p.flags = plan.spec.link_flag | FLAG_SCALED_MOMENTS | share
    p.wrec = wrec.data_ptr() if wrec is not None else None
    p.dev_step = dev_step.data_ptr() if dev_step is not None else None
    check(_lib.load().vfm_elbo_bwd_adam_lookahead_f32(
        C.byref(p), C.byref(ix), ptr(entity_params), ptr(bias_params), ptr(scalars), ptr(inv_occ), ptr(plan.W),
        ptr(st.sumz), ptr(st.grow), ptr(st.partials), ptr(m_views[0]), ptr(v_views[0]), ptr(m_views[1]), ptr(v_views[1]),
        ptr(m_views[2]), ptr(v_views[2]), lr, beta1, beta2, eps_adam, int(step), ptr(loss_out), ptr(last_step),
        ptr(next_plan.occ_ptr), ptr(step_tab), current_stream_ptr(entity_params.device)),
        "vfm_elbo_bwd_adam_lookahead_f32")
    p.flags = plan.spec.link_flag | share


def adam_catchup(entity_params, bias_params, m_views, v_views, last_step, ids, lr_of_step, upto, mark,
                 beta1=0.9, beta2=0.999, eps_adam=1e-8, wrec=None):
    T, d = entity_params.shape[0], entity_params.shape[1] // 2
    n = T if ids is None else ids.numel()
    need = (int(upto) - 1) % MOMENT_PERIOD + 1 if upto > 0 else 0
    vals = [float(v) for v in lr_of_step] + [0.0] * max(0, need - len(lr_of_step))
    lrs = (C.c_float * max(len(vals), 1))(*vals)
    check(_lib.load().vfm_adam_catchup_f32(ptr(entity_params), ptr(bias_params), ptr(m_views[0]), ptr(v_views[0]),
                                           ptr(m_views[1]), ptr(v_views[1]), ptr(last_step), ptr(ids), n, T, d, lrs,
                                           len(vals), beta1, beta2, eps_adam, int(upto), int(mark), ptr(wrec),
                                           current_stream_ptr(entity_params.device)), "vfm_adam_catchup_f32")


def wrec_build(bias_params, inv_occ, wrec):
    check(_lib.load().vfm_wrec_build_f32(ptr(bias_params), ptr(inv_occ), bias_params.shape[0], ptr(wrec),
                                         current_stream_ptr(wrec.device)), "vfm_wrec_build_f32")


class StepState:
    WINDOW = 4096

    def __init__(self, device):
        self.dev = torch.zeros(8, dtype=torch.int64, device=device)
        self.tab = torch.zeros(self.WINDOW, 16, dtype=torch.float32, device=device)
        self.first, self.length, self.key = 0, 0, None
        self.counters = None

    def cover(self, adam_step: int, lr: float, beta1: float, beta2: float, eps: float, scaled: bool):
        key = (float(lr), float(beta1), float(beta2), float(eps), bool(scaled))
        if key == self.key and self.first <= adam_step < self.first + self.length:
            return
        lib = _lib.load()
        host = (_lib.StepConsts * self.WINDOW)()
        for i in range(self.WINDOW):
            check(lib.vfm_step_consts(key[0], key[1], key[2], key[3], adam_step + i, int(scaled), C.byref(host[i])),
                  "vfm_step_consts")
        raw = torch.frombuffer(bytearray(bytes(host)), dtype=torch.float32).view(self.WINDOW, 16)
        self.tab.copy_(raw)
        hdr = _lib.DevStep()
        hdr.tab_first, hdr.tab_len, hdr.tab = adam_step, self.WINDOW, self.tab.data_ptr()
        hdr.error = int(self.dev[7].item())
        self.dev.copy_(torch.frombuffer(bytearray(bytes(hdr)), dtype=torch.int64))
        self.first, self.length, self.key, self.counters = adam_step, self.WINDOW, key, None

    def set(self, philox_step: int, adam_step: int):
        if self.counters != (philox_step, adam_step):
            check(_lib.load().vfm_dev_step_set(ptr(self.dev), int(philox_step), int(adam_step),
                                               current_stream_ptr(self.dev.device)), "vfm_dev_step_set")
            self.counters = (philox_step, adam_step)

    def advanced(self):
        self.counters = (self.counters[0] + 1, self.counters[1] + 1)

    def error(self) -> bool:
        return bool(int(self.dev[7].item()))


def exchange_record_len(d: int) -> int:
    return 4 + (d + 3) // 4 * 4


def elbo_backward_acc(plan: BatchPlan, st: FwdState, acc, sums, e_lo=0, e_hi=0):
    if plan.occ_ptr is None:
        plan.build_index()
    spec = plan.spec
    _lib.ops().elbo_bwd_acc(plan.index_tensors(), st.sumz, st.grow, st.partials, acc, sums,
                            spec.T, spec.F, spec.d, e_lo, e_hi)


def elbo_apply_adam(plan: BatchPlan, st: FwdState, acc, sums, entity_params, bias_params, scalars,
                    inv_occ, m_views, v_views, lr, step, beta1=0.9, beta2=0.999, eps_adam=1e-8, e_lo=0, e_hi=0,
                    scaled_moments=False):
    e = st.eps if st.eps is not None else (None, None, None)
    p, spec = st.problem, plan.spec
    _lib.ops().elbo_apply_adam(acc, sums, entity_params, bias_params, scalars, inv_occ, plan.W,
                               e[0], e[1], e[2], m_views[0], v_views[0], m_views[1], v_views[1], m_views[2],
                               v_views[2], spec.F, list(spec.group_hi), list(spec.group_n), p.nb_train,
                               p.B_global, p.likelihood,
                               (p.flags & ~FLAG_NO_PRIOR_TERMS) | (FLAG_SCALED_MOMENTS if scaled_moments else 0),
                               p.seed & _I63, p.step,
                               lr, beta1, beta2, eps_adam, int(step), e_lo, e_hi)


def elbo_backward_acc_rows(plan: BatchPlan, st: FwdState, row_ids, acc, sums):
    ix = _index_struct(plan)
    spec = plan.spec
    p = _problem(spec, plan.B, plan.B, 64)
    check(_lib.load().vfm_elbo_bwd_acc_rows_f32(C.byref(p), C.byref(ix), ptr(row_ids), row_ids.numel(), ptr(st.sumz),
                                                ptr(st.grow), ptr(st.partials), ptr(acc), ptr(sums),
                                                current_stream_ptr(acc.device)), "vfm_elbo_bwd_acc_rows_f32")


def elbo_apply_adam_rows(plan: BatchPlan, st: FwdState, acc, sums, row_ids, entity_params, bias_params, scalars, inv_occ,
                         m_views, v_views, lr, step, move_scalars: bool, compact: bool = False, beta1=0.9, beta2=0.999,
                         eps_adam=1e-8, wrec=None):
    p0, spec = st.problem, plan.spec
    p = _problem(spec, 0, p0.B_global, 64, p0.seed, p0.step, (p0.flags & ~FLAG_NO_PRIOR_TERMS) | FLAG_SCALED_MOMENTS, wrec=wrec)
    p.e_lo, p.e_hi = 0, (0 if move_scalars else 1)
    check(_lib.load().vfm_elbo_apply_adam_rows_f32(
        C.byref(p), ptr(acc), ptr(sums), ptr(row_ids), row_ids.numel(), int(bool(compact)), ptr(entity_params), ptr(bias_params),
        ptr(scalars),
        ptr(inv_occ), ptr(plan.W), ptr(m_views[0]), ptr(v_views[0]), ptr(m_views[1]), ptr(v_views[1]), ptr(m_views[2]),
        ptr(v_views[2]), lr, beta1, beta2, eps_adam, int(step), current_stream_ptr(entity_params.device)),
        "vfm_elbo_apply_adam_rows_f32")


def moments_rescale(m, v, step, to_scaled, beta1=0.9, beta2=0.999):
    _lib.ops().moments_rescale(m, v, beta1, beta2, int(step), bool(to_scaled))


def adam_step(p, g, m, v, lr, step, beta1=0.9, beta2=0.999, eps=1e-8):
    for t in (p, g, m, v):
        _need_cuda(t, "adam tensor")
    _lib.ops().adam(p, g, m, v, lr, beta1, beta2, eps, int(step))


def philox_eps(spec: Spec, seed: int, step: int, device):
    S = int(spec.n_samples)
    lead = () if S == 1 else (S,)
    ee = torch.empty(*lead, spec.T, spec.d, dtype=torch.float32, device=device)
    eb = torch.empty(*lead, spec.T, dtype=torch.float32, device=device)
    eg = torch.empty(S, dtype=torch.float32, device=device)
    p = _problem(spec, 0, 0, 64, seed, step)
    lib = _lib.load()
    check(lib.vfm_philox_eps_f32(C.byref(p), ptr(ee), ptr(eb), ptr(eg), current_stream_ptr(ee.device)),
          "vfm_philox_eps_f32")
    return ee, eb, eg


class ElboFunction(torch.autograd.Function):

    @staticmethod
    def forward(ctx, entity_params, bias_params, alpha, global_bias_mean, global_bias_scale,
                plan, inv_occ, eps, seed, step):
        scalars = torch.cat([alpha.detach().reshape(1), global_bias_mean.detach().reshape(1),
                             global_bias_scale.detach().reshape(1)]).contiguous()
        ent, bia = entity_params.detach(), bias_params.detach()
        st = elbo_forward(plan, ent, bia, scalars, inv_occ, eps=eps, seed=seed, step=step, train=True)
        loss3 = elbo_finalize(st, scalars)
        ctx.plan, ctx.st, ctx.inv_occ, ctx.scalars = plan, st, inv_occ, scalars
        ctx.save_for_backward(ent, bia)
        ctx.mark_non_differentiable(st.pred, loss3)
        ctx.set_materialize_grads(True)
        return loss3[0:1].clone(), st.pred, loss3

    @staticmethod
    def backward(ctx, g_loss, _g_pred, _g_loss3):
        ent, bia = ctx.saved_tensors
        gout = g_loss.to(torch.float32).reshape(1).contiguous()
        g_ent, g_bias, g_sc = elbo_backward(ctx.plan, ctx.st, ent, bia, ctx.scalars, ctx.inv_occ, gout)
        return (g_ent, g_bias, g_sc[0:1], g_sc[1:2], g_sc[2:3], None, None, None, None, None)
```

Before: 555.7 million.

## Balance forward work groups by row-plus-segment cost via precomputed bounds

Adds a small scan pipeline at index-build time that gives each row a cost (2 if it starts a new user segment, else 1), prefix-sums those costs and binary-searches per-group start/end bounds for the forward kernel. The forward kernel then reads these bounds instead of splitting rows evenly, so groups holding many segment boundaries no longer straggle. The cost is three extra small kernels per batch index build, a larger workspace and arena, plus ABI struct fields with a compatibility path for the old struct size.

```diff
diff --git a/include/vfm_hip.h b/include/vfm_hip.h
--- a/include/vfm_hip.h
+++ b/include/vfm_hip.h
@@ -1,6 +1,7 @@
 #ifndef VFM_HIP_H
 #define VFM_HIP_H
 
+#include <stddef.h>
 #include <stdint.h>
 
 #ifdef __cplusplus
@@ -82,7 +83,14 @@
   int64_t e_lo, e_hi;
   vfm_dev_step_t* dev_step;
   float* wrec;
+  uint64_t fwd_bounds, fwd_bounds_share;
+  int32_t fwd_bounds_ng, fwd_bounds_share_ng;
 } vfm_problem_t;
+#define VFM_PROBLEM_SIZE_MIN ((uint32_t)offsetof(vfm_problem_t, fwd_bounds))
+int32_t vfm_fwd_groups(int64_t B, int32_t d, int32_t flags);
+int64_t vfm_fwd_bounds_workspace_bytes(int64_t B);
+int vfm_fwd_bounds_build(int64_t B, int32_t id_bits, const void* x, void* ws, int32_t ng0, int32_t* bounds0,
+                         int32_t ng1, int32_t* bounds1, void* stream);
 int vfm_wrec_build_f32(const float* bias_params, const float* inv_occ, int64_t T, float* wrec, void* stream);
 
 #define VFM_HEAVY_LIST 64
diff --git a/vae_amd/_abi_gen.py b/vae_amd/_abi_gen.py
--- a/vae_amd/_abi_gen.py
+++ b/vae_amd/_abi_gen.py
@@ -90,6 +90,10 @@
         ("e_hi", C.c_int64),
         ("dev_step", C.c_void_p),
         ("wrec", C.c_void_p),
+        ("fwd_bounds", C.c_uint64),
+        ("fwd_bounds_share", C.c_uint64),
+        ("fwd_bounds_ng", C.c_int32),
+        ("fwd_bounds_share_ng", C.c_int32),
     ]
 
     def __init__(self, *a, **k):
diff --git a/vae_amd/_lib.py b/vae_amd/_lib.py
--- a/vae_amd/_lib.py
+++ b/vae_amd/_lib.py
@@ -30,6 +30,7 @@
     "vfm_sample_records_f32", "vfm_elbo_bwd_adam_pipe_f32", "vfm_elbo_bwd_adam_lookahead_f32",
     "vfm_step_consts", "vfm_dev_step_set", "vfm_wrec_build_f32", "vfm_elbo_apply_adam_rows_f32",
     "vfm_elbo_bwd_acc_rows_f32", "vfm_heavy_threshold", "vfm_rebuild_heavy",
+    "vfm_fwd_groups", "vfm_fwd_bounds_workspace_bytes", "vfm_fwd_bounds_build",
 )
 
 
@@ -248,6 +249,11 @@
     lib.vfm_step_consts.argtypes = [C.c_float, C.c_float, C.c_float, C.c_float, i64, i32, C.POINTER(StepConsts)]
     lib.vfm_dev_step_set.argtypes = [vp, C.c_uint64, i64, vp]
     lib.vfm_wrec_build_f32.argtypes = [vp, vp, i64, vp, vp]
+    lib.vfm_fwd_groups.argtypes = [i64, i32, i32]
+    lib.vfm_fwd_groups.restype = i32
+    lib.vfm_fwd_bounds_workspace_bytes.argtypes = [i64]
+    lib.vfm_fwd_bounds_workspace_bytes.restype = i64
+    lib.vfm_fwd_bounds_build.argtypes = [i64, i32, vp, vp, i32, vp, i32, vp, vp]
     lib.vfm_sample_records_f32.argtypes = [PP, vp, i64, vp, vp, vp, vp, vp, vp]
     lib.vfm_elbo_bwd_adam_pipe_f32.argtypes = ([PP, C.POINTER(Index), C.POINTER(Pipe)] + [vp] * 13 +
                                                [C.c_float, C.c_float, C.c_float, C.c_float, i64, vp, vp])
diff --git a/vae_amd/csrc/vfm_abi.hip b/vae_amd/csrc/vfm_abi.hip
--- a/vae_amd/csrc/vfm_abi.hip
+++ b/vae_amd/csrc/vfm_abi.hip
@@ -61,7 +61,8 @@
 
 int check_problem(const vfm_problem_t* p, bool dev_ok = false) {
   if (!p) return fail(VFM_E_INVALID, "problem is NULL");
-  if (int rc = check_struct(p->struct_size, p->abi_version, sizeof(vfm_problem_t), "vfm_problem_t")) return rc;
+  if (!(p->struct_size == VFM_PROBLEM_SIZE_MIN && p->abi_version == (uint32_t)VFM_ABI_VERSION))
+    if (int rc = check_struct(p->struct_size, p->abi_version, sizeof(vfm_problem_t), "vfm_problem_t")) return rc;
   if (p->dev_step && !dev_ok)
     return fail(VFM_E_UNSUPPORTED, "vfm_problem_t.dev_step: only the training forward and the fused backward+Adam entry points read the step from device memory");
   if (p->dev_step && p->n_samples != 1) return fail(VFM_E_UNSUPPORTED, "vfm_problem_t.dev_step: one variational sample");
@@ -123,6 +124,10 @@
   a.x = x; a.y = y; a.entity = entity; a.bias = bias; a.inv_occ = inv_occ; a.scalars = scalars;
   a.W = W; a.eps_entity = ee; a.eps_bias = eb; a.eps_global = eg;
   a.dev = p->dev_step; a.wrec = p->wrec;
+  if (p->struct_size >= (uint32_t)sizeof(vfm_problem_t)) {
+    a.fwd_bounds = reinterpret_cast<const int32_t*>((uintptr_t)p->fwd_bounds); a.fwd_bounds_ng = p->fwd_bounds_ng;
+    a.fwd_bounds_share = reinterpret_cast<const int32_t*>((uintptr_t)p->fwd_bounds_share); a.fwd_bounds_share_ng = p->fwd_bounds_share_ng;
+  }
   for (int g = 0; g < p->F; ++g) { a.group_hi[g] = p->group_hi[g]; a.group_n[g] = p->group_n[g]; }
   return a;
 }
diff --git a/vae_amd/csrc/vfm_args.hpp b/vae_amd/csrc/vfm_args.hpp
--- a/vae_amd/csrc/vfm_args.hpp
+++ b/vae_amd/csrc/vfm_args.hpp
@@ -40,6 +40,9 @@
   const float* eps_global;
   vfm_dev_step_t* dev;
   float* wrec;
+  const int32_t* fwd_bounds;
+  const int32_t* fwd_bounds_share;
+  int32_t fwd_bounds_ng, fwd_bounds_share_ng;
   int64_t group_hi[VFM_MAX_FIELDS];
   double group_n[VFM_MAX_FIELDS];
 };
@@ -136,6 +139,23 @@
 VFM_INTERNAL int fail(int code, const char* msg);
 VFM_INTERNAL int fail_hip(hipError_t e, const char* where);
 VFM_INTERNAL int env_int(const char* name, int dflt);
+inline int fwd2_lpe(int d) {
+  const int C = d / 4, P = (C + 1) / 2;
+  int lpe = 1;
+  while (lpe < P) lpe <<= 1;
+  return lpe;
+}
+inline int64_t fwd2_blocks(int64_t B, int lpe, int flags, bool env) {
+  const int GPB = BLOCK / lpe;
+  const int per_cu = env ? env_int("VFM_FWD2_BLOCKS_PER_CU", 4) : 4;
+  int64_t nb = (B + GPB - 1) / GPB;
+  int64_t cap = 256LL * per_cu;
+  if (cap > VFM_MAX_FWD_BLOCKS) cap = VFM_MAX_FWD_BLOCKS;
+  if (nb > cap) nb = cap;
+  { const int share = env ? env_int("VFM_SHARE_CAP", 960) : 960; if ((flags & VFM_FLAG_SHARE_GPU) && share > 0 && nb > share) nb = share; }
+  if (env) { const int forced = env_int("VFM_FWD2_GRID", 0); if (forced > 0 && nb > forced) nb = forced; }
+  return nb < 1 ? 1 : nb;
+}
 VFM_INTERNAL int launch_norms(int64_t B, int F, int64_t T, int id_bits, const void* x, const float* inv_occ, double* W,
                               hipStream_t st);
 
diff --git a/vae_amd/csrc/vfm_fwd2.hip b/vae_amd/csrc/vfm_fwd2.hip
--- a/vae_amd/csrc/vfm_fwd2.hip
+++ b/vae_amd/csrc/vfm_fwd2.hip
@@ -19,14 +19,10 @@
 template <int LPE, bool FULL, int EPS, int MODE>
 int launch_fwd2_t(KArgs& a, const FwdOut& o, hipStream_t st) {
   constexpr int GPB = BLOCK / LPE;
-  const int per_cu = env_int("VFM_FWD2_BLOCKS_PER_CU", 4);
-  int64_t nb = (a.B + GPB - 1) / GPB;
-  int64_t cap = 256LL * per_cu;
-  if (cap > VFM_MAX_FWD_BLOCKS) cap = VFM_MAX_FWD_BLOCKS;
-  if (nb > cap) nb = cap;
-  { const int share = env_int("VFM_SHARE_CAP", 960); if ((a.flags & VFM_FLAG_SHARE_GPU) && share > 0 && nb > share) nb = share; }
-  { const int forced = env_int("VFM_FWD2_GRID", 0); if (forced > 0 && nb > forced) nb = forced; }
-  if (nb < 1) nb = 1;
+  const int64_t nb = fwd2_blocks(a.B, LPE, a.flags, true);
+  const int64_t NG = nb * GPB;
+  if (!(a.fwd_bounds && a.fwd_bounds_ng == NG))
+    a.fwd_bounds = (a.fwd_bounds_share && a.fwd_bounds_share_ng == NG) ? a.fwd_bounds_share : nullptr;
   if constexpr (EPS == EPS_PHILOX && MODE == MODE_TRAIN) {
     if (a.wrec) {
       if (a.id64)
diff --git a/vae_amd/csrc/vfm_fwd2.hpp b/vae_amd/csrc/vfm_fwd2.hpp
--- a/vae_amd/csrc/vfm_fwd2.hpp
+++ b/vae_amd/csrc/vfm_fwd2.hpp
@@ -148,9 +148,17 @@
   const int C = a.d >> 2;
   const int NG = (int)gridDim.x * GPB;
   const int gid = (int)blockIdx.x * GPB + tid / LPE;
-  const int q = (int)(a.B / NG), rem = (int)(a.B % NG);
-  const int gbeg = gid * q + (gid < rem ? gid : rem);
-  const int gend = gbeg + q + (gid < rem ? 1 : 0);
+  int gbeg, gend;
+  if (a.fwd_bounds) {
+    const int b0 = a.fwd_bounds[gid], b1 = a.fwd_bounds[gid + 1];
+    const int Bi = (int)a.B;
+    gbeg = b0 < 0 ? 0 : (b0 > Bi ? Bi : b0);
+    gend = b1 < gbeg ? gbeg : (b1 > Bi ? Bi : b1);
+  } else {
+    const int q = (int)(a.B / NG), rem = (int)(a.B % NG);
+    gbeg = gid * q + (gid < rem ? gid : rem);
+    gend = gbeg + q + (gid < rem ? 1 : 0);
+  }
   const int glast = gend - 1;
   RawIds<ID64> raw0, raw1, raw2;
   float y_first = 0.f;
diff --git a/vae_amd/csrc/vfm_index.hip b/vae_amd/csrc/vfm_index.hip
--- a/vae_amd/csrc/vfm_index.hip
+++ b/vae_amd/csrc/vfm_index.hip
@@ -614,6 +614,91 @@
   return 0;
 }
 
+constexpr int FB_ROWS = 4;
+constexpr int FB_TILE = HV_CHUNK * FB_ROWS;
+
+__device__ __forceinline__ int2 fb_block_scan(int v, int* sh) {
+  const int tid = threadIdx.x, lane = tid & 63;
+  int inc = v;
+#pragma unroll
+  for (int o = 1; o < 64; o <<= 1) {
+    const int up = __shfl_up(inc, o, 64);
+    if (lane >= o) inc += up;
+  }
+  if (lane == 63) sh[tid >> 6] = inc;
+  __syncthreads();
+  int base = 0, total = 0;
+#pragma unroll
+  for (int w = 0; w < HV_CHUNK / 64; ++w) {
+    const int s = sh[w];
+    base += (w < (tid >> 6)) ? s : 0;
+    total += s;
+  }
+  return make_int2(base + inc, total);
+}
+
+__global__ __launch_bounds__(HV_CHUNK) void k_fb_tiles(const void* __restrict__ x, int id64, int B, int32_t* __restrict__ pl,
+                                                       int32_t* __restrict__ tot) {
+  __shared__ int sh[HV_CHUNK / 64];
+  const int r0 = (int)blockIdx.x * FB_TILE + (int)threadIdx.x * FB_ROWS;
+  int t[FB_ROWS], s = 0;
+#pragma unroll
+  for (int k = 0; k < FB_ROWS; ++k) {
+    const int r = r0 + k;
+    bool starts = r == 0;
+    if (r > 0 && r < B) {
+      if (id64) starts = reinterpret_cast<const int64_t*>(x)[2 * (size_t)r + 1] != reinterpret_cast<const int64_t*>(x)[2 * (size_t)r - 1];
+      else starts = reinterpret_cast<const int32_t*>(x)[2 * (size_t)r + 1] != reinterpret_cast<const int32_t*>(x)[2 * (size_t)r - 1];
+    }
+    t[k] = r < B ? (starts ? 2 : 1) : 0;
+    s += t[k];
+  }
+  const int2 sc = fb_block_scan(s, sh);
+  int e = sc.x - s;
+#pragma unroll
+  for (int k = 0; k < FB_ROWS; ++k) {
+    if (r0 + k < B) pl[r0 + k] = e;
+    e += t[k];
+  }
+  if (threadIdx.x == 0) tot[blockIdx.x] = sc.y;
+}
+
+__global__ __launch_bounds__(HV_CHUNK) void k_fb_scan(int32_t* __restrict__ tot, int NT) {
+  __shared__ int sh[HV_CHUNK / 64];
+  int carry = 0;
+  for (int b0 = 0; b0 < NT; b0 += HV_CHUNK) {
+    const int i = b0 + (int)threadIdx.x;
+    const int v = i < NT ? tot[i] : 0;
+    const int2 sc = fb_block_scan(v, sh);
+    if (i < NT) tot[i] = carry + sc.x - v;
+    carry += sc.y;
+    __syncthreads();
+  }
+  if (threadIdx.x == 0) tot[NT] = carry;
+}
+
+__global__ __launch_bounds__(HV_CHUNK) void k_fb_bounds(const int32_t* __restrict__ pl, const int32_t* __restrict__ offs, int B,
+                                                        int NT, int ng0, int32_t* __restrict__ out0, int ng1,
+                                                        int32_t* __restrict__ out1) {
+  const int j = (int)blockIdx.x * HV_CHUNK + (int)threadIdx.x;
+  int g = j, ng = ng0;
+  int32_t* out = out0;
+  if (j > ng0) {
+    g = j - (ng0 + 1); ng = ng1; out = out1;
+    if (ng1 <= 0 || g > ng1) return;
+  }
+  const int64_t total = offs[NT];
+  const int64_t q = total / ng, rem = total % ng;
+  const int64_t c = (int64_t)g * q + (g < rem ? g : rem);
+  int lo = 0, hi = B;
+  while (lo < hi) {
+    const int mid = lo + (hi - lo + 1) / 2;
+    const int64_t P = mid == B ? total : (int64_t)pl[mid] + offs[mid / FB_TILE];
+    if (P <= c) lo = mid; else hi = mid - 1;
+  }
+  out[g] = lo;
+}
+
 }
 }
 
@@ -638,6 +723,41 @@
 int64_t vfm_index_workspace_bytes(int64_t B, int32_t F, int64_t T) {
   if (B < 0 || F < 1 || T < 1 || T > 0xFFFFFFFELL || B * (int64_t)F > 0x7FFFFFFFLL) return -1;
   return geometry(B * F, T).total * 4;
+}
+
+int32_t vfm_fwd_groups(int64_t B, int32_t d, int32_t flags) {
+  if (B < 0 || d < 4 || (d & 3) != 0 || d > 512) return 0;
+  const int lpe = fwd2_lpe(d);
+  return (int32_t)(fwd2_blocks(B, lpe, flags, false) * (BLOCK / lpe));
+}
+
+int64_t vfm_fwd_bounds_workspace_bytes(int64_t B) {
+  if (B < 0 || 2 * B > 0x7FFFFFFFLL) return -1;
+  return 4 * (B + (B + FB_TILE - 1) / FB_TILE + 4);
+}
+
+int vfm_fwd_bounds_build(int64_t B, int32_t id_bits, const void* x, void* ws, int32_t ng0, int32_t* bounds0, int32_t ng1,
+                         int32_t* bounds1, void* stream) {
+  if (B < 0 || 2 * B > 0x7FFFFFFFLL || (id_bits != 32 && id_bits != 64) || ng0 < 1 || !bounds0 || ng1 < 0 || (ng1 > 0 && !bounds1) ||
+      (B > 0 && (!x || !ws)))
+    return fail(VFM_E_INVALID, "vfm_fwd_bounds_build: bad argument");
+  hipStream_t st = (hipStream_t)stream;
+  hipError_t e = hipSuccess;
+  if (B == 0) {
+    e = hipMemsetAsync(bounds0, 0, sizeof(int32_t) * ((size_t)ng0 + 1), st);
+    if (e == hipSuccess && ng1 > 0) e = hipMemsetAsync(bounds1, 0, sizeof(int32_t) * ((size_t)ng1 + 1), st);
+    return e == hipSuccess ? 0 : fail_hip(e, "vfm_fwd_bounds_build");
+  }
+  const int NT = (int)((B + FB_TILE - 1) / FB_TILE);
+  int32_t* pl = reinterpret_cast<int32_t*>(ws);
+  int32_t* tot = pl + B;
+  hipLaunchKernelGGL(k_fb_tiles, dim3(NT), dim3(HV_CHUNK), 0, st, x, id_bits == 64 ? 1 : 0, (int)B, pl, tot);
+  hipLaunchKernelGGL(k_fb_scan, dim3(1), dim3(HV_CHUNK), 0, st, tot, NT);
+  const int64_t nthr = (int64_t)ng0 + 1 + (ng1 > 0 ? (int64_t)ng1 + 1 : 0);
+  hipLaunchKernelGGL(k_fb_bounds, dim3((unsigned)((nthr + HV_CHUNK - 1) / HV_CHUNK)), dim3(HV_CHUNK), 0, st, pl, tot, (int)B, NT,
+                     ng0, bounds0, ng1, bounds1);
+  e = hipGetLastError();
+  return e == hipSuccess ? 0 : fail_hip(e, "vfm_fwd_bounds_build");
 }
 
 int64_t vfm_union_workspace_bytes(int64_t T) { return T < 1 ? -1 : 4 * ((T + HV_CHUNK - 1) / HV_CHUNK + 4); }
diff --git a/vae_amd/csrc/vfm_torch_ops.cpp b/vae_amd/csrc/vfm_torch_ops.cpp
--- a/vae_amd/csrc/vfm_torch_ops.cpp
+++ b/vae_amd/csrc/vfm_torch_ops.cpp
@@ -45,7 +45,14 @@
   return p;
 }
 
-void extensions(vfm_problem_t& p, const optional<Tensor>& wrec, const optional<Tensor>& dev_step, int64_t T) {
+void extensions(vfm_problem_t& p, const optional<Tensor>& wrec, const optional<Tensor>& dev_step, int64_t T,
+                const optional<Tensor>& fwd_bounds = c10::nullopt, int64_t ng0 = 0, int64_t ng1 = 0) {
+  if (fwd_bounds.has_value() && fwd_bounds->defined() && ng0 > 0) {
+    const int64_t off1 = (ng0 + 1 + 3) & ~(int64_t)3;
+    TORCH_CHECK(dev_tensor(*fwd_bounds, at::kInt, "fwd_bounds").numel() >= (ng1 > 0 ? off1 + ng1 + 1 : ng0 + 1), "fwd_bounds too small");
+    p.fwd_bounds = (uint64_t)(uintptr_t)fwd_bounds->data_ptr<int32_t>(); p.fwd_bounds_ng = (int32_t)ng0;
+    if (ng1 > 0) { p.fwd_bounds_share = p.fwd_bounds + 4 * (uint64_t)off1; p.fwd_bounds_share_ng = (int32_t)ng1; }
+  }
   if (wrec.has_value() && wrec->defined()) {
     TORCH_CHECK(dev_tensor(*wrec, at::kFloat, "wrec").numel() >= 4 * T, "wrec needs [T,4] floats");
     p.wrec = wrec->data_ptr<float>();
@@ -74,7 +81,8 @@
               const optional<Tensor>& sumz, const optional<Tensor>& grow, at::IntArrayRef group_hi,
               at::ArrayRef<double> group_n, int64_t nb_train, int64_t B_global, int64_t likelihood,
               int64_t flags, int64_t seed, int64_t step, int64_t n_samples,
-              const optional<Tensor>& wrec, const optional<Tensor>& dev_step) {
+              const optional<Tensor>& wrec, const optional<Tensor>& dev_step, const optional<Tensor>& fwd_bounds,
+              int64_t fwd_ng0, int64_t fwd_ng1) {
   const Ids id = ids_of(x);
   dev_tensor(entity, at::kFloat, "entity_params"); dev_tensor(bias, at::kFloat, "bias_params");
   dev_tensor(scalars, at::kFloat, "scalars"); dev_tensor(pred, at::kFloat, "pred");
@@ -92,7 +100,7 @@
   c10::hip::HIPGuard guard(x.get_device());
   vfm_problem_t p = problem(x, id.B, B_global, T, id.F, d, nb_train, likelihood, id.id_bits, flags, group_hi,
                             group_n, seed, step, n_samples);
-  extensions(p, wrec, dev_step, T);
+  extensions(p, wrec, dev_step, T, fwd_bounds, fwd_ng0, fwd_ng1);
   const double* Wp = (W.has_value() && W->defined()) ? dev_tensor(*W, at::kDouble, "W").data_ptr<double>() : nullptr;
   check(vfm_elbo_fwd_f32(&p, id.ptr, fptr(y, "y"), entity.data_ptr<float>(), bias.data_ptr<float>(),
                          fptr(inv_occ, "inv_occ"), scalars.data_ptr<float>(), Wp, fptr(eps_entity, "eps_entity"),
@@ -325,7 +333,7 @@
         "Tensor? W, Tensor? eps_entity, Tensor? eps_bias, Tensor? eps_global, Tensor(a!) pred, Tensor(b!) partials, "
         "Tensor(c!)? sumz, Tensor(d!)? grow, int[] group_hi, float[] group_n, int nb_train, int B_global, "
         "int likelihood, int flags, int seed, int step, int n_samples=1, Tensor(e!)? wrec=None, "
-        "Tensor(f!)? dev_step=None) -> ()", &elbo_fwd);
+        "Tensor(f!)? dev_step=None, Tensor? fwd_bounds=None, int fwd_ng0=0, int fwd_ng1=0) -> ()", &elbo_fwd);
   m.def("elbo_finalize(Tensor(a!) partials, Tensor scalars, Tensor(b!) loss, int nb_train, int B_global, int flags, "
         "int n_samples=1) -> ()",
         &elbo_finalize);
diff --git a/vae_amd/ops.py b/vae_amd/ops.py
--- a/vae_amd/ops.py
+++ b/vae_amd/ops.py
@@ -133,6 +133,15 @@
         if len(_SIZES) > 256:
             _SIZES.clear()
         _SIZES[(B, F, T)] = hit
+    return hit
+
+
+def _fwd_bounds_sizes(B: int, d: int):
+    hit = _SIZES.get(("fb", B, d))
+    if hit is None:
+        lib = _lib.load()
+        ng0, ng1 = int(lib.vfm_fwd_groups(B, d, 0)), int(lib.vfm_fwd_groups(B, d, FLAG_SHARE_GPU))
+        hit = _SIZES[("fb", B, d)] = (ng0, ng1 if ng1 != ng0 else 0, int(lib.vfm_fwd_bounds_workspace_bytes(B))) if ng0 > 0 else (0, 0, 0)
     return hit
 
 
@@ -183,6 +192,7 @@
         self._occ_rows = self._status = self._occ_other = self._lay = None
         self._ready = None
         self._arena = None
+        self.fwd_bounds = None
         self._heavy = self._pend = None
         self._U = 0
         self._touched = None
@@ -223,10 +233,14 @@
     def _build_index_locked(self, lib, n, L, nbytes, validate, inv_occ=None, stream=None):
         spec, dev = self.spec, self.x.device
         raw = stream.cuda_stream if stream is not None else _lib.raw_stream(dev)
-        ws = _index_workspace(nbytes // 4 + 4, dev, raw)
+        ng0 = ng1 = fb_bytes = 0
+        if spec.F == 2 and self.B > 0:
+            ng0, ng1, fb_bytes = _fwd_bounds_sizes(self.B, spec.d)
+        ws = _index_workspace(max(nbytes, fb_bytes) // 4 + 4, dev, raw)
         cap_h, cap_i = n // L + 1, 2 * n // L + 2
         sizes = (spec.T + 1, max(n, 1), cap_h, 4 * cap_i, 8, max(min(n, spec.T), 1), max(n, 1) if spec.F == 2 else 0,
-                 2 * spec.F if inv_occ is not None else 0)
+                 2 * spec.F if inv_occ is not None else 0,
+                 (((ng0 + 4) & ~3) + (ng1 + 1 if ng1 else 0)) if ng0 else 0)
         offs, o = [], 0
         for v in sizes:
             offs.append(o)
@@ -242,6 +256,11 @@
                                   cap_i, P[5], P[6] if spec.F == 2 else None, ptr(inv_occ),
                                   ptr(self.W) if inv_occ is not None else None, P[4], C.c_void_p(host.data_ptr()),
                                   C.c_void_p(raw)), "vfm_build_index")
+        if ng0:
+            b1 = C.c_void_p(base + 4 * (offs[8] + ((ng0 + 4) & ~3))) if ng1 else None
+            check(lib.vfm_fwd_bounds_build(self.B, self.id_bits, ptr(self.x), ptr(ws), ng0, P[8], ng1, b1, C.c_void_p(raw)),
+                  "vfm_fwd_bounds_build")
+            self.fwd_bounds = (arena[offs[8]: offs[8] + sizes[8]], ng0, ng1)
         self.occ_ptr = arena[: spec.T + 1]
         done = torch.cuda.Event()
         done.record(stream if stream is not None else _stream_obj(dev, raw))
@@ -487,7 +506,7 @@
                         plan.W if have_y else None, e[0], e[1], e[2], pred, partials, sumz, grow,
                         list(spec.group_hi), list(spec.group_n), spec.nb_train, plan.B_global,
                         spec.likelihood, p.flags, p.seed & _I63, p.step, S,
-                        wrec if (train and eps is None) else None, dev_step)
+                        wrec if (train and eps is None) else None, dev_step, *(plan.fwd_bounds or (None, 0, 0)))
     return FwdState(pred, partials, sumz, grow, p, eps)
 
 
@@ -559,6 +578,11 @@
 def elbo_forward_records(plan: BatchPlan, zrec, scalars, seed, step, out_pred, out_grow, out_partials, dev_step=None, flags=0) -> FwdState:
     spec = plan.spec
     p = _problem(spec, plan.B, plan.B_global, plan.id_bits, seed, step, FLAG_ZREC | flags, dev_step=dev_step)
+    if plan.fwd_bounds is not None:
+        t, ng0, ng1 = plan.fwd_bounds
+        p.fwd_bounds, p.fwd_bounds_ng = t.data_ptr(), ng0
+        if ng1:
+            p.fwd_bounds_share, p.fwd_bounds_share_ng = t.data_ptr() + 4 * ((ng0 + 4) & ~3), ng1
     check(_lib.load().vfm_elbo_fwd_f32(C.byref(p), ptr(plan.x), ptr(plan.y), ptr(zrec), None, None, ptr(scalars), None,
                                        None, None, None, ptr(out_pred), ptr(out_partials), None, ptr(out_grow),
                                        current_stream_ptr(zrec.device)), "vfm_elbo_fwd_f32 (records)")
```

Result: no change. 559.3 million, median of 6 (+0.6%).
